# centreborelli/satnerf

Hardware: AMD Instinct MI355X
Metric: training rays/sec (64 samples/ray) (higher is better)
Workload: dtype bf16; 1 GPU; BASELINE configs[1] sat-nerf 256/tau4, 1024 rays x 64 samples/GPU, mlp_mode=bf16, saved state 8-bit, noise_std=0 sc_lambda=0 n_importance=0, stratified jitter drawn in-kernel (Philox-4x32-10); rays_per_gpu=1024, global_batch=1024, n_samples=64, parallelism=dp1

## Files before the change

include/satrender.h:

```cpp
#ifndef SATRENDER_H
#define SATRENDER_H

#include <stdint.h>

#ifdef __cplusplus
extern "C" {
#endif

#define SR_VERSION 100

#define SR_MODE_BF16 1
#define SR_MODE_BF16X3 3
#define SR_MODE_F16 2

#define SR_FMT16 16
#define SR_FMT8 8

int sr_version(void);
const char* sr_last_error(void);

int64_t sr_fwd_stream_elems(int feat, int tau);
int64_t sr_bwd_stream_elems(int feat, int tau);
int64_t sr_act_elems_per_tile(int feat, int fmt);
int64_t sr_dpre_elems_per_tile(int feat, int fmt);
int64_t sr_workspace_tiles(int64_t n_points);
int64_t sr_dpre_workspace_elems(int64_t n_points, int feat, int fmt);

int sr_pack_stream(const float* src, const int32_t* idx, const float* scale, int64_t n,
                   uint16_t* out_hi, uint16_t* out_lo, int64_t n_f16, void* stream);
int sr_pack_all(const float* src, const int32_t* idx, const float* scale, int64_t n, uint16_t* out_hi, uint16_t* out_lo,
                const int32_t* f32_idx, const float* f32_scale, int64_t n_f32, float* out_f32, float* tick, int64_t n_f16,
                void* stream);

int sr_gather_scale_f32(const float* src, const int32_t* idx, const float* scale, int64_t n, float* out, void* stream);

int sr_unpack_grads(const float* partial, const int32_t* gidx, const float* gscale, int64_t n_params, const int32_t* blocks,
                    float* grad, int accumulate, void* stream);

int sr_ray_sample_fwd(const float* rays, int ray_stride, const float* u, int64_t n_rays, int n_samples,
                      float* z_vals, void* stream);

int sr_sky_fwd(const float* sun, int sun_stride, int64_t n, int hidden, const float* w1, const float* b1,
               const float* w2, const float* b2, float* sky, void* stream);

typedef struct sr_mlp_inputs {
  const float* org;
  int org_stride;
  const float* dir;
  int dir_stride;
  const float* sun;
  int sun_stride;
  const float* z;
  const float* temb;
  const int64_t* ts;
  int64_t n_points;
  int n_samples;
} sr_mlp_inputs;

int sr_satnerf_mlp_fwd(const sr_mlp_inputs* in, int feat, int tau, int mode, const uint16_t* stream_hi,
                       const uint16_t* stream_lo, const float* l0, float* albedo, float* sigma, float* sun_v,
                       float* beta, uint16_t* acts, int act_fmt, void* stream);

typedef struct sr_render_args {
  const float* rays;
  int ray_stride;
  const int64_t* ts;
  const float* temb;
  int64_t n_rays;
  int n_samples;
  const float* z_in;
  const float* u;
  uint64_t seed;
  float* step_counter;
  int tick;
  const float* noise;
  float noise_std;
  int sky_hidden;
  const float* sky_w1;
  const float* sky_b1;
  const float* sky_w2;
  const float* sky_b2;
  int64_t bank_chunks;
} sr_render_args;

typedef struct sr_render_outputs {
  float* z_vals;
  float* albedo;
  float* sigma;
  float* sun_v;
  float* beta;
  float* sky;
  float* weights;
  float* transparency;
  float* depth;
  float* rgb;
} sr_render_outputs;

int sr_satnerf_render_fwd(const sr_render_args* in, int feat, int tau, int mode, const uint16_t* stream_hi, const uint16_t* stream_lo,
                          const float* l0, const sr_render_outputs* out, void* stream);
int sr_render_points_per_block(int feat, int mode);

typedef struct sr_train_args {
  const float* target;
  const float* sched;
  float beta_min;
  float* loss_parts;
  float* rgb;
  float* d_sigma;
  float* d_albedo;
  float* d_sun_v;
  float* g_beta;
  float* d_sky;
  const int64_t* gather_idx;
  float* cursor;
  int64_t batches;
  float* out_rays;
  float* out_rgbs;
  int64_t* out_ts;
} sr_train_args;
int sr_satnerf_render_train(const sr_render_args* in, int feat, int tau, int mode, const uint16_t* stream_hi, const uint16_t* stream_lo,
                            const float* l0, const sr_render_outputs* out, const sr_train_args* train, uint16_t* acts, int act_fmt, void* stream);

int sr_satnerf_mlp_bwd(int feat, int tau, int64_t n_points, const uint16_t* bwd_stream, const uint16_t* acts,
                       const float* albedo, const float* sigma, const float* sun_v, const float* beta, const float* g_albedo,
                       const float* g_sigma, const float* g_sun_v, const float* g_beta, uint16_t* dpre, float* d_t, int fmt,
                       void* stream);
int sr_wgrad_plan(int32_t* blocks, int n_blocks, int64_t n_points, int n_wg, int fmt, int* n_slices);
int sr_satnerf_wgrad(int feat, int tau, int64_t n_points, const uint16_t* dpre, const uint16_t* acts, const int32_t* blocks,
                     int n_blocks, int n_slices, float* partial, void* stream);
int sr_satnerf_wgrad8(int feat, int tau, int64_t n_points, const uint16_t* dpre, int64_t dpre_elems, const uint16_t* acts,
                      const int32_t* blocks, const int32_t* loads, int n_blocks, int n_slices, int plan_span, float* partial, void* stream);
int sr_wgrad8_load_ints(void);

int sr_sky_bwd(const float* sun, int sun_stride, int64_t n, int hidden, const float* w1, const float* b1, const float* w2,
               const float* sky, const float* d_sky, float* g_w1, float* g_b1, float* g_w2, float* g_b2, void* stream);
int sr_embedding_bwd(const float* d_t, const int64_t* ts, int64_t n_rays, int n_samples, int tau, float* g_emb, void* stream);

int sr_sc_loss(const float* z_vals, const float* sigma, const float* noise, float noise_std, const float* sun_v, int64_t n_rays,
               int n_samples, float lambda_sc, float* loss_parts, float* d_sun_v, void* stream);
int sr_depth_loss(const float* depth, const float* depths, int depths_stride, int use_weights, int64_t n_rays, float lambda_ds,
                  float* loss_parts, float* g_depth, void* stream);
int sr_ray_setup(const float* rays, int ray_stride, const float* u, int64_t n_rays, int n_samples, int hidden, const float* w1,
                 const float* b1, const float* w2, const float* b2, float* z_vals, float* sky, void* stream);
int sr_ray_setup_rng(const float* rays, int ray_stride, uint64_t seed, float* step_counter, int tick, int64_t n_rays, int n_samples,
                     int hidden, const float* w1, const float* b1, const float* w2, const float* b2, float* z_vals, float* sky,
                     void* stream);
int sr_render_loss(const float* z_vals, const float* sigma, const float* noise, float noise_std, const float* albedo,
                   const float* sun_v, const float* beta, const float* sky, const float* target, int64_t n_rays, int n_samples,
                   float beta_min, const float* sched, float* loss_parts, float* rgb, float* d_sigma, float* d_albedo, float* d_sun_v,
                   float* g_beta, float* d_sky, void* stream);

int sr_grad_tail(const float* partial, const int32_t* gidx, const float* gscale, int64_t n_params, const int32_t* blocks, int n_blocks,
                 float* grad, int accumulate, const float* sun, int sun_stride, int64_t n_rays, int hidden,
                 const float* w1, const float* b1, const float* w2, const float* sky, const float* d_sky, float* g_w1, float* g_b1,
                 float* g_w2, float* g_b2, const float* d_t, const int64_t* ts, int n_samples, int tau, float* g_emb, void* stream);
typedef struct sr_pack_scatter {
  const int32_t* map;
  uint16_t* hi;
  uint16_t* lo;
  float* l0;
  int64_t n_f16;
  float scales[4];
} sr_pack_scatter;
int sr_grad_tail_adam(const float* partial, const int32_t* gidx, const float* gscale, int64_t n_params, const int32_t* blocks, int n_blocks,
                      float* grad,
                      int accumulate, const float* sun, int sun_stride, int64_t n_rays, int hidden, const float* w1, const float* b1,
                      const float* w2, const float* sky, const float* d_sky, float* g_w1, float* g_b1, float* g_w2, float* g_b2,
                      const float* d_t, const int64_t* ts, int n_samples, int tau, float* g_emb, float* params, float* exp_avg,
                      float* exp_avg_sq, const int32_t* late_idx, int n_late, float* state, float lr, float beta1, float beta2, float eps,
                      float grad_scale, const sr_pack_scatter* pack, void* stream);
int sr_adam_step_graph(float* params, float* grads, float* exp_avg, float* exp_avg_sq, int64_t n, float lr, float beta1,
                       float beta2, float eps, float grad_scale, float* state, int zero_grad, void* stream);
int sr_adam_step_pack(float* params, float* grads, float* exp_avg, float* exp_avg_sq, int64_t n, float lr, float beta1, float beta2,
                      float eps, float grad_scale, float* state, int zero_grad, int64_t n_packed, const sr_pack_scatter* pack,
                      void* stream);

enum { SR_ACT_NONE = 0, SR_ACT_SIN = 1, SR_ACT_RELU = 2 };
enum { SR_OUT_NONE = 0, SR_OUT_SOFTPLUS = 1, SR_OUT_SIGMOID = 2, SR_OUT_SIGMOID_RGB = 3 };
typedef struct sr_linear_src {
  const float* x;
  int ld;
  int k;
  int act;
  float w0;
  int row_div;
} sr_linear_src;
int sr_linear_fwd(const sr_linear_src* src, int n_src, const float* weight, const float* bias, int64_t n_points, int n_out,
                  int out_act, float* y, int ldy, void* stream);
int sr_linear_bwd_input(const float* gy, int ldg, const float* y, int ldy, int out_act, const float* weight, int k_total, int col0,
                        const sr_linear_src* target, int64_t n_points, int n_out, float* d_src, int ldd, void* stream);
int sr_linear_bwd_weight(const float* gy, int ldg, const float* y, int ldy, int out_act, const sr_linear_src* src, int n_src,
                         int64_t n_points, int n_out, float* d_weight, float* d_bias, void* stream);
int sr_points_along(const float* rays, int ray_stride, int dir_col, const float* z_vals, int64_t n_rays, int n_samples, float* xyz,
                    void* stream);
int sr_positional_map(const float* x, int ld, int dim, int64_t rows, int n_freqs, float* out, void* stream);

int sr_composite_image(const float* z_vals, const float* sigma, const float* noise, float noise_std, const float* albedo,
                       const float* sun_v, const float* beta, const float* sky, int64_t n_rays, int n_samples, float* image,
                       void* stream);
int sr_latlonalt_from_depth(const float* rays, int ray_stride, const float* depth, int64_t n_rays, const double* center,
                            double range, double* lat, double* lon, double* alt, void* stream);

int sr_rpc_rays(const double* rpc, int width, int height, double min_alt, double max_alt, const double* center, double range,
                double sun_elevation_deg, double sun_azimuth_deg, float* rays11, float* rays8, void* stream);

int sr_rpc_rays_at(const double* rpc, const double* colrow, int64_t n, double min_alt, double max_alt, const double* center, double range,
                   double sun_elevation_deg, double sun_azimuth_deg, float* rays11, void* stream);
int sr_reprojection_errors(const double* rpc, const double* colrow, const int64_t* pts3d_idx, int64_t n, const double* pts3d,
                           int64_t n_pts, float* err, void* stream);
int sr_keypoint_weights_scratch(int64_t n_pts, int n_cams, int64_t* bytes);
int sr_keypoint_weights(const int64_t* pts3d_idx, const int64_t* cam, const float* err, int64_t n, int64_t n_pts, int n_cams,
                        void* scratch, int64_t scratch_bytes, float* e, float* w, float* e_mean, void* stream);
int sr_tie_point_depths(const float* rays11, const double* pts3d, const int64_t* pts3d_idx, int64_t n, int64_t n_pts,
                        const double* center, double range, const float* w, float* depths, void* stream);

int sr_idw_grid_scratch(int64_t k, int n_neighbors, int64_t* bytes);
int sr_idw_interpolate(const double* pts2d, const float* z, int64_t k, const double* query, int64_t n_query, int height, int width,
                       int n_neighbors, void* scratch, int64_t scratch_bytes, double* out, int* nn_idx, int* visited, void* stream);
int sr_gaussian_filter_f64(const double* in, int h, int w, const double* taps0, int radius0, const double* taps1, int radius1,
                           double* tmp, double* out, void* stream);

int sr_utm_zone(double lat, double lon, int* zone, int* letter);
int sr_utm_from_latlon(const double* lat, const double* lon, int64_t n, int zone, double* east, double* north, void* stream);
int sr_depth_to_utm(const float* rays, int ray_stride, const float* depth, int64_t n_rays, const double* center, double range,
                    int zone, double* east, double* north, double* alt, int* zone_out, void* stream);
int sr_dsm_bounds(const double* east, const double* north, const double* alt, int64_t n, double* bounds, void* stream);
int sr_dsm_rasterize(const double* east, const double* north, const double* alt, int64_t n, double xoff, double yoff,
                     double resolution, int xsize, int ysize, int radius, double sigma, uint64_t* acc, float* dsm, float* weight,
                     void* stream);

int sr_dsm_register_scratch(int hu, int wu, int hv, int wv, int irange, int64_t* bytes, int* levels);
int sr_dsm_downsample2x(const double* in, int h, int w, double* out, void* stream);
int sr_dsm_compute_shift(const double* u, int hu, int wu, const double* v, int hv, int wv, int irange, int scaling, void* scratch,
                         int64_t scratch_bytes, int* shift, double* coef, double* ncc_levels, int* start_levels, void* stream);
int sr_dsm_apply_shift(const double* v, int hv, int wv, const int* shift, const double* coef, float* out, void* stream);

int sr_image_metrics_scratch(int64_t n, int64_t planes, int h, int w, int64_t* bytes);
int sr_image_sse(const float* pred, const float* gt, int64_t n, const uint8_t* mask, int64_t mask_div, void* scratch,
                 int64_t scratch_bytes, double* out, void* stream);
int sr_ssim_sum(const float* img1, const float* img2, int64_t planes, int h, int w, void* scratch, int64_t scratch_bytes, double* out,
                void* stream);

int sr_satnerf_loss(const float* rgb, const float* weights, const float* beta, const float* target, int64_t n_rays,
                    int n_samples, float beta_min, float grad_scale, const float* sched, float* loss_parts, float* g_rgb,
                    float* g_weights, float* g_beta, void* stream);
int sr_gather_batch(const float* rays, const float* rgbs, const int64_t* ts, const int64_t* idx, int64_t n, float* out_rays,
                    float* out_rgbs, int64_t* out_ts, float* cursor, int64_t batches, void* stream);
int sr_gather_setup(const float* rays, const float* rgbs, const int64_t* ts, const int64_t* idx, int64_t n, float* out_rays,
                    float* out_rgbs, int64_t* out_ts, float* cursor, int64_t batches, int n_samples, int hidden, const float* w1,
                    const float* b1, const float* w2, const float* b2, float* z_vals, float* sky, uint64_t seed,
                    const float* step_counter, int step_offset, void* stream);
int sr_adam_step(float* params, float* grads, float* exp_avg, float* exp_avg_sq, int64_t n, float lr, float beta1,
                 float beta2, float eps, float grad_scale, int64_t step, int zero_grad, void* stream);

int sr_composite_fwd(const float* z_vals, const float* sigma, const float* noise, float noise_std,
                     const float* albedo, const float* sun_v, const float* sky, int64_t n_rays, int n_samples,
                     int clamp_rgb, float* weights, float* transparency, float* depth, float* rgb, void* stream);

int sr_composite_bwd(const float* z_vals, const float* sigma, const float* noise, float noise_std,
                     const float* albedo, const float* sun_v, const float* sky, const float* weights,
                     const float* transparency, const float* rgb_unclamped_or_null, int64_t n_rays, int n_samples,
                     int clamp_rgb, const float* g_rgb, const float* g_depth, const float* g_weights,
                     const float* g_transparency, float* d_sigma, float* d_albedo, float* d_sun_v, float* d_sky,
                     void* stream);

int sr_sample_pdf_merge(const float* z_coarse, const float* weights_coarse, const float* u, int64_t n_rays,
                        int n_samples, int n_importance, float eps, float* z_fine, void* stream);
int sr_sample_pdf(const float* bins, const float* weights, const float* u, int64_t n_rays, int n_bins, int n_importance,
                  float eps, float* samples, void* stream);

#ifdef __cplusplus
}
#endif
#endif
// ... 1 lines not shown
```

satnerf_amd/_lib.py:

```python
from __future__ import annotations

import ctypes as C
import os

_HERE = os.path.dirname(os.path.abspath(__file__))
LIB_PATH = os.environ.get("SATRENDER_LIB") or os.path.join(_HERE, "csrc", "libsatrender.so")

MODE_BF16 = 1
MODE_F16 = 2
MODE_BF16X3 = 3
FMT16, FMT8 = 16, 8

_vp, _i, _i64, _f, _d = C.c_void_p, C.c_int, C.c_int64, C.c_float, C.c_double


class MlpInputs(C.Structure):
    _fields_ = [("org", _vp), ("org_stride", _i), ("dir", _vp), ("dir_stride", _i), ("sun", _vp), ("sun_stride", _i),
                ("z", _vp), ("temb", _vp), ("ts", _vp), ("n_points", _i64), ("n_samples", _i)]


class RenderArgs(C.Structure):
    _fields_ = [("rays", _vp), ("ray_stride", _i), ("ts", _vp), ("temb", _vp), ("n_rays", _i64), ("n_samples", _i), ("z_in", _vp), ("u", _vp),
                ("seed", C.c_uint64), ("step_counter", _vp), ("tick", _i), ("noise", _vp), ("noise_std", _f), ("sky_hidden", _i),
                ("sky_w1", _vp), ("sky_b1", _vp), ("sky_w2", _vp), ("sky_b2", _vp), ("bank_chunks", _i64)]


class RenderOutputs(C.Structure):
    _fields_ = [(k, _vp) for k in ("z_vals", "albedo", "sigma", "sun_v", "beta", "sky", "weights", "transparency", "depth", "rgb")]


class TrainArgs(C.Structure):
    _fields_ = [("target", _vp), ("sched", _vp), ("beta_min", _f), ("loss_parts", _vp), ("rgb", _vp), ("d_sigma", _vp), ("d_albedo", _vp),
                ("d_sun_v", _vp), ("g_beta", _vp), ("d_sky", _vp), ("gather_idx", _vp), ("cursor", _vp), ("batches", _i64), ("out_rays", _vp),
                ("out_rgbs", _vp), ("out_ts", _vp)]


class PackScatter(C.Structure):
    _fields_ = [("map", _vp), ("hi", _vp), ("lo", _vp), ("l0", _vp), ("n_f16", _i64), ("scales", _f * 4)]


class LinearSrc(C.Structure):
    _fields_ = [("x", _vp), ("ld", _i), ("k", _i), ("act", _i), ("w0", _f), ("row_div", _i)]


ACT_NONE, ACT_SIN, ACT_RELU = 0, 1, 2
OUT_NONE, OUT_SOFTPLUS, OUT_SIGMOID, OUT_SIGMOID_RGB = 0, 1, 2, 3

SIGNATURES = {
    "sr_version": (_i, []),
    "sr_last_error": (C.c_char_p, []),
    "sr_fwd_stream_elems": (_i64, [_i, _i]),
    "sr_bwd_stream_elems": (_i64, [_i, _i]),
    "sr_act_elems_per_tile": (_i64, [_i, _i]),
    "sr_satnerf_render_fwd": (_i, [_vp, _i, _i, _i, _vp, _vp, _vp, _vp, _vp]),
    "sr_render_points_per_block": (_i, [_i, _i]),
    "sr_satnerf_render_train": (_i, [_vp, _i, _i, _i, _vp, _vp, _vp, _vp, _vp, _vp, _i, _vp]),
    "sr_pack_stream": (_i, [_vp, _vp, _vp, _i64, _vp, _vp, _i64, _vp]),
    "sr_dpre_elems_per_tile": (_i64, [_i, _i]),
    "sr_workspace_tiles": (_i64, [_i64]),
    "sr_dpre_workspace_elems": (_i64, [_i64, _i, _i]),
    "sr_unpack_grads": (_i, [_vp, _vp, _vp, _i64, _vp, _vp, _i, _vp]),
    "sr_composite_image": (_i, [_vp, _vp, _vp, _f, _vp, _vp, _vp, _vp, _i64, _i, _vp, _vp]),
    "sr_latlonalt_from_depth": (_i, [_vp, _i, _vp, _i64, _vp, _d, _vp, _vp, _vp, _vp]),
    "sr_linear_fwd": (_i, [C.POINTER(LinearSrc), _i, _vp, _vp, _i64, _i, _i, _vp, _i, _vp]),
    "sr_linear_bwd_input": (_i, [_vp, _i, _vp, _i, _i, _vp, _i, _i, C.POINTER(LinearSrc), _i64, _i, _vp, _i, _vp]),
    "sr_linear_bwd_weight": (_i, [_vp, _i, _vp, _i, _i, C.POINTER(LinearSrc), _i, _i64, _i, _vp, _vp, _vp]),
    "sr_positional_map": (_i, [_vp, _i, _i, _i64, _i, _vp, _vp]),
    "sr_points_along": (_i, [_vp, _i, _i, _vp, _i64, _i, _vp, _vp]),
    "sr_wgrad_plan": (_i, [_vp, _i, _i64, _i, _i, _vp]),
    "sr_satnerf_mlp_bwd": (_i, [_i, _i, _i64, _vp, _vp, _vp, _vp, _vp, _vp, _vp, _vp, _vp, _vp, _vp, _vp, _i, _vp]),
    "sr_satnerf_wgrad": (_i, [_i, _i, _i64, _vp, _vp, _vp, _i, _i, _vp, _vp]),
    "sr_satnerf_wgrad8": (_i, [_i, _i, _i64, _vp, _i64, _vp, _vp, _vp, _i, _i, _i, _vp, _vp]),
    "sr_wgrad8_load_ints": (_i, []),
    "sr_sky_bwd": (_i, [_vp, _i, _i64, _i, _vp, _vp, _vp, _vp, _vp, _vp, _vp, _vp, _vp, _vp]),
    "sr_embedding_bwd": (_i, [_vp, _vp, _i64, _i, _i, _vp, _vp]),
    "sr_ray_setup": (_i, [_vp, _i, _vp, _i64, _i, _i, _vp, _vp, _vp, _vp, _vp, _vp, _vp]),
    "sr_sc_loss": (_i, [_vp, _vp, _vp, _f, _vp, _i64, _i, _f, _vp, _vp, _vp]),
    "sr_depth_loss": (_i, [_vp, _vp, _i, _i, _i64, _f, _vp, _vp, _vp]),
    "sr_ray_setup_rng": (_i, [_vp, _i, C.c_uint64, _vp, _i, _i64, _i, _i, _vp, _vp, _vp, _vp, _vp, _vp, _vp]),
    "sr_render_loss": (_i, [_vp, _vp, _vp, _f, _vp, _vp, _vp, _vp, _vp, _i64, _i, _f, _vp, _vp, _vp, _vp, _vp, _vp, _vp, _vp, _vp]),
    "sr_satnerf_loss": (_i, [_vp, _vp, _vp, _vp, _i64, _i, _f, _f, _vp, _vp, _vp, _vp, _vp, _vp]),
    "sr_adam_step": (_i, [_vp, _vp, _vp, _vp, _i64, _f, _f, _f, _f, _f, _i64, _i, _vp]),
    "sr_gather_setup": (_i, [_vp, _vp, _vp, _vp, _i64, _vp, _vp, _vp, _vp, _i64, _i, _i, _vp, _vp, _vp, _vp, _vp, _vp, C.c_uint64, _vp, _i, _vp]),
    "sr_gather_batch": (_i, [_vp, _vp, _vp, _vp, _i64, _vp, _vp, _vp, _vp, _i64, _vp]),
    "sr_grad_tail": (_i, [_vp, _vp, _vp, _i64, _vp, _i, _vp, _i, _vp, _i, _i64, _i, _vp, _vp, _vp, _vp, _vp, _vp, _vp, _vp, _vp, _vp, _vp, _i, _i,
                          _vp, _vp]),
    "sr_grad_tail_adam": (_i, [_vp, _vp, _vp, _i64, _vp, _i, _vp, _i, _vp, _i, _i64, _i, _vp, _vp, _vp, _vp, _vp, _vp, _vp, _vp, _vp, _vp, _vp, _i, _i,
                               _vp, _vp, _vp, _vp, _vp, _i, _vp, _f, _f, _f, _f, _f, _vp, _vp]),
    "sr_adam_step_graph": (_i, [_vp, _vp, _vp, _vp, _i64, _f, _f, _f, _f, _f, _vp, _i, _vp]),
    "sr_adam_step_pack": (_i, [_vp, _vp, _vp, _vp, _i64, _f, _f, _f, _f, _f, _vp, _i, _i64, _vp, _vp]),
    "sr_pack_all": (_i, [_vp, _vp, _vp, _i64, _vp, _vp, _vp, _vp, _i64, _vp, _vp, _i64, _vp]),
    "sr_gather_scale_f32": (_i, [_vp, _vp, _vp, _i64, _vp, _vp]),
    "sr_ray_sample_fwd": (_i, [_vp, _i, _vp, _i64, _i, _vp, _vp]),
    "sr_sky_fwd": (_i, [_vp, _i, _i64, _i, _vp, _vp, _vp, _vp, _vp, _vp]),
    "sr_satnerf_mlp_fwd": (_i, [C.POINTER(MlpInputs), _i, _i, _i, _vp, _vp, _vp, _vp, _vp, _vp, _vp, _vp, _i, _vp]),
    "sr_composite_fwd": (_i, [_vp, _vp, _vp, _f, _vp, _vp, _vp, _i64, _i, _i, _vp, _vp, _vp, _vp, _vp]),
    "sr_composite_bwd": (_i, [_vp, _vp, _vp, _f, _vp, _vp, _vp, _vp, _vp, _vp, _i64, _i, _i, _vp, _vp, _vp, _vp, _vp, _vp,
                              _vp, _vp, _vp]),
    "sr_sample_pdf_merge": (_i, [_vp, _vp, _vp, _i64, _i, _i, _f, _vp, _vp]),
    "sr_sample_pdf": (_i, [_vp, _vp, _vp, _i64, _i, _i, _f, _vp, _vp]),
    "sr_rpc_rays": (_i, [_vp, _i, _i, _d, _d, _vp, _d, _d, _d, _vp, _vp, _vp]),
    "sr_rpc_rays_at": (_i, [_vp, _vp, _i64, _d, _d, _vp, _d, _d, _d, _vp, _vp]),
    "sr_reprojection_errors": (_i, [_vp, _vp, _vp, _i64, _vp, _i64, _vp, _vp]),
    "sr_keypoint_weights_scratch": (_i, [_i64, _i, C.POINTER(_i64)]),
    "sr_keypoint_weights": (_i, [_vp, _vp, _vp, _i64, _i64, _i, _vp, _i64, _vp, _vp, _vp, _vp]),
    "sr_tie_point_depths": (_i, [_vp, _vp, _vp, _i64, _i64, _vp, _d, _vp, _vp, _vp]),
    "sr_idw_grid_scratch": (_i, [_i64, _i, C.POINTER(_i64)]),
    "sr_idw_interpolate": (_i, [_vp, _vp, _i64, _vp, _i64, _i, _i, _i, _vp, _i64, _vp, _vp, _vp, _vp]),
    "sr_gaussian_filter_f64": (_i, [_vp, _i, _i, _vp, _i, _vp, _i, _vp, _vp, _vp]),
    "sr_utm_zone": (_i, [_d, _d, C.POINTER(_i), C.POINTER(_i)]),
    "sr_utm_from_latlon": (_i, [_vp, _vp, _i64, _i, _vp, _vp, _vp]),
    "sr_depth_to_utm": (_i, [_vp, _i, _vp, _i64, _vp, _d, _i, _vp, _vp, _vp, _vp, _vp]),
    "sr_dsm_bounds": (_i, [_vp, _vp, _vp, _i64, _vp, _vp]),
    "sr_dsm_rasterize": (_i, [_vp, _vp, _vp, _i64, _d, _d, _d, _i, _i, _i, _d, _vp, _vp, _vp, _vp]),
    "sr_dsm_register_scratch": (_i, [_i, _i, _i, _i, _i, C.POINTER(_i64), C.POINTER(_i)]),
    "sr_dsm_downsample2x": (_i, [_vp, _i, _i, _vp, _vp]),
    "sr_dsm_compute_shift": (_i, [_vp, _i, _i, _vp, _i, _i, _i, _i, _vp, _i64, _vp, _vp, _vp, _vp, _vp]),
    "sr_dsm_apply_shift": (_i, [_vp, _i, _i, _vp, _vp, _vp, _vp]),
    "sr_image_metrics_scratch": (_i, [_i64, _i64, _i, _i, C.POINTER(_i64)]),
    "sr_image_sse": (_i, [_vp, _vp, _i64, _vp, _i64, _vp, _i64, _vp, _vp]),
    "sr_ssim_sum": (_i, [_vp, _vp, _i64, _i, _i, _vp, _i64, _vp, _vp]),
}

_lib = None


class SatRenderError(RuntimeError):
    pass


def lib():
    global _lib
    if _lib is None:
        if not os.path.exists(LIB_PATH):
            raise SatRenderError(
                f"{LIB_PATH} not found: build the HIP library first (python -c 'import __graft_entry__ as g; g.build()'). "
                "satnerf_amd has no CPU or PyTorch fallback.")
        handle = C.CDLL(LIB_PATH)
        for name, (res, args) in SIGNATURES.items():
            fn = getattr(handle, name)
            fn.restype, fn.argtypes = res, args
        _lib = handle
    return _lib


def call(name, *args):
    handle = lib()
    rc = getattr(handle, name)(*args)
    if rc != 0:
        raise SatRenderError(f"{name} failed (status {rc}): {handle.sr_last_error().decode(errors='replace')}")
```

satnerf_amd/csrc/mlp_api.hip:

```cpp
#include "common.h"
#include "mlp_layout.h"
#include "mlp_params.h"

namespace sr {
int launch_fwd_p1a1(const FwdParams&, int, hipStream_t);
int launch_fwd_p1a2(const FwdParams&, int, hipStream_t);
int launch_fwd_p3a1(const FwdParams&, int, hipStream_t);
int launch_fwd_p3a2(const FwdParams&, int, hipStream_t);
int launch_fwd_h1a1(const FwdParams&, int, hipStream_t);
int launch_fwd_h1a2(const FwdParams&, int, hipStream_t);
int launch_fwd512_p1a1(const FwdParams&, int, hipStream_t);
int launch_fwd512_p1a2(const FwdParams&, int, hipStream_t);
int launch_fwd512_h1a1(const FwdParams&, int, hipStream_t);
int launch_fwd512_h1a2(const FwdParams&, int, hipStream_t);
long fwd512_stream_pieces_a1();
long fwd512_stream_pieces_a2();
}
using namespace sr;
extern "C" int sr_satnerf_mlp_fwd(const sr_mlp_inputs* in, int feat, int tau, int mode, const uint16_t* stream_hi,
                                  const uint16_t* stream_lo, const float* l0, float* albedo, float* sigma, float* sun_v,
                                  float* beta, uint16_t* acts, int act_fmt, void* stream) {
  SR_REQUIRE(in != nullptr, "sr_satnerf_mlp_fwd: null inputs");
  SR_REQUIRE(feat == kFeat || feat == 512, "sr_satnerf_mlp_fwd: feat=%d unsupported (this build handles %d and 512)", feat, kFeat);
  SR_REQUIRE(mode == SR_MODE_BF16 || mode == SR_MODE_BF16X3 || mode == SR_MODE_F16, "sr_satnerf_mlp_fwd: bad mode %d", mode);
  SR_REQUIRE(feat == kFeat || ((mode == SR_MODE_BF16 || mode == SR_MODE_F16) && (acts == nullptr || act_fmt == SR_FMT8)),
             "sr_satnerf_mlp_fwd: feat=512 runs the fused kernel in SR_MODE_BF16 / SR_MODE_F16, saving activations in SR_FMT8 only (parity mode: layer by layer)");
  SR_REQUIRE(tau >= 1 && tau <= 24, "sr_satnerf_mlp_fwd: tau=%d unsupported (1..24)", tau);
  SR_REQUIRE(stream_hi && l0 && in->org && in->sun && in->temb, "sr_satnerf_mlp_fwd: null pointer argument");
  SR_REQUIRE(mode != SR_MODE_BF16X3 || stream_lo, "sr_satnerf_mlp_fwd: BF16X3 needs the lo plane");
  SR_REQUIRE(in->n_samples >= 1, "sr_satnerf_mlp_fwd: n_samples must be >= 1");
  SR_REQUIRE(acts == nullptr || act_fmt == SR_FMT16 || act_fmt == SR_FMT8, "sr_satnerf_mlp_fwd: act_fmt must be 16 or 8 (got %d)", act_fmt);
  if (in->n_points <= 0) return 0;
  FwdParams p;
  p.in = *in;
  p.rend = RenderParams{};
  p.train = TrainParams{};
  p.stream_hi = (const char*)stream_hi;
  p.stream_lo = (const char*)stream_lo;
  p.l0 = (const float4*)l0;
  p.albedo = albedo, p.sigma = sigma, p.sun_v = sun_v, p.beta = beta;
  p.acts = (uint4*)acts;
  p.tau = tau;
  hipStream_t st = (hipStream_t)stream;
  const int save = acts != nullptr ? act_fmt : 0;
  const int auxs = aux_steps(tau);
  if (feat == 512 && mode == SR_MODE_F16) return auxs == 1 ? launch_fwd512_h1a1(p, save, st) : launch_fwd512_h1a2(p, save, st);
  if (feat == 512) return auxs == 1 ? launch_fwd512_p1a1(p, save, st) : launch_fwd512_p1a2(p, save, st);
  if (mode == SR_MODE_BF16) return auxs == 1 ? launch_fwd_p1a1(p, save, st) : launch_fwd_p1a2(p, save, st);
  if (mode == SR_MODE_F16) return auxs == 1 ? launch_fwd_h1a1(p, save, st) : launch_fwd_h1a2(p, save, st);
  return auxs == 1 ? launch_fwd_p3a1(p, save, st) : launch_fwd_p3a2(p, save, st);
}

extern "C" int64_t sr_fwd_stream_elems(int feat, int tau) {
  if ((feat != kFeat && feat != 512) || tau < 1 || tau > 24) return -1;
  if (feat == 512) return (aux_steps(tau) == 1 ? fwd512_stream_pieces_a1() : fwd512_stream_pieces_a2()) * 512;
  return (aux_steps(tau) == 1 ? FwdStream<1>::total_pieces() : FwdStream<2>::total_pieces()) * 512;
}

extern "C" int sr_render_points_per_block(int feat, int mode) {
  if (mode != SR_MODE_BF16 && mode != SR_MODE_BF16X3 && mode != SR_MODE_F16) return -1;
  if (feat == kFeat) return mode == SR_MODE_BF16X3 ? 128 : 256;
  if (feat == 512 && (mode == SR_MODE_BF16 || mode == SR_MODE_F16)) return 128;
  return -1;
}

static int render_launch(const char* who, const sr_render_args* in, int feat, int tau, int mode, const uint16_t* stream_hi, const uint16_t* stream_lo,
                         const float* l0, const sr_render_outputs* out, const sr_train_args* tr, uint16_t* acts, int act_fmt, void* stream) {
  SR_REQUIRE(in != nullptr && out != nullptr, "%s: null argument block", who);
  const int per_block = sr_render_points_per_block(feat, mode);
  SR_REQUIRE(per_block > 0, "%s: no fused kernel for feat=%d mode=%d (256: every mode; 512: SR_MODE_BF16 / SR_MODE_F16)", who, feat, mode);
  SR_REQUIRE(tau >= 1 && tau <= 24, "%s: tau=%d unsupported (1..24)", who, tau);
  SR_REQUIRE(in->n_samples >= 2 && per_block % in->n_samples == 0, "%s: n_samples=%d must be >= 2 and divide %d (sr_render_points_per_block)", who,
             in->n_samples, per_block);
  SR_REQUIRE(in->rays && in->ts && in->temb && in->ray_stride >= 11, "%s: rays (stride >= 11), ts and temb are required", who);
  SR_REQUIRE(stream_hi && l0 && (mode != SR_MODE_BF16X3 || stream_lo), "%s: null weight stream", who);
  SR_REQUIRE(in->sky_w1 && in->sky_b1 && in->sky_w2 && in->sky_b2 && in->sky_hidden >= 1, "%s: the sky head's weights are required", who);
  SR_REQUIRE(tr != nullptr || (out->weights && out->transparency), "%s: weights and transparency outputs are required", who);
  SR_REQUIRE(!in->tick || in->step_counter, "%s: tick needs the 4-float step counter block", who);
  SR_REQUIRE(in->bank_chunks >= 0 && (in->bank_chunks == 0 || in->step_counter), "%s: bank_chunks needs the step counter", who);
  if (tr != nullptr) {
    SR_REQUIRE(mode == SR_MODE_BF16 || mode == SR_MODE_F16, "%s: the fused training forward exists for SR_MODE_BF16 / SR_MODE_F16 (8-bit saved state)", who);
    SR_REQUIRE(acts != nullptr && act_fmt == SR_FMT8, "%s: needs the SR_FMT8 activation workspace", who);
    SR_REQUIRE(in->n_samples <= 64, "%s: n_samples=%d unsupported (one wave per ray: <= 64); use the separate launches", who, in->n_samples);
    SR_REQUIRE(tr->target && tr->loss_parts && tr->d_sigma && tr->d_albedo && tr->d_sun_v && tr->g_beta && tr->d_sky && out->sky, "%s: null training output", who);
    SR_REQUIRE(out->albedo && out->sigma && out->sun_v && out->beta, "%s: the four per-point outputs are required (the dX pass reads them)", who);
    if (tr->gather_idx != nullptr) {
      SR_REQUIRE(tr->cursor && tr->batches >= 1 && tr->batches < (1 << 24), "%s: the in-launch sampler needs a cursor block and 1 <= batches < 2^24", who);
      SR_REQUIRE(tr->out_rays && tr->out_rgbs && tr->out_ts, "%s: the in-launch sampler needs out_rays / out_rgbs / out_ts", who);
      SR_REQUIRE(in->ray_stride == 11 && in->bank_chunks == 0 && in->z_in == nullptr && in->u == nullptr && in->noise == nullptr,
                 "%s: the in-launch sampler takes a bank of 11-float rows and draws its own jitter (no z_in / u / noise / bank_chunks)", who);
    }
  }
  SR_REQUIRE(in->tick != 2 || (tr != nullptr && in->bank_chunks == 0), "%s: tick == 2 (tick first) is a training-launch option", who);
  SR_REQUIRE(in->tick >= 0 && in->tick <= 2, "%s: tick must be 0, 1 or 2", who);
  if (in->n_rays <= 0) return 0;
  FwdParams p;
  p.in.org = in->rays, p.in.org_stride = in->ray_stride;
  p.in.dir = in->rays + 3, p.in.dir_stride = in->ray_stride;
  p.in.sun = in->rays + 8, p.in.sun_stride = in->ray_stride;
  p.in.z = nullptr, p.in.temb = in->temb, p.in.ts = in->ts;
  p.in.n_points = in->n_rays * in->n_samples, p.in.n_samples = in->n_samples;
  RenderParams& r = p.rend;
  r.rays = in->rays, r.ray_stride = in->ray_stride, r.z_in = in->z_in, r.u = in->u, r.seed = in->seed, r.step_counter = in->step_counter;
  r.tick = in->tick, r.noise = in->noise, r.noise_std = in->noise_std, r.sky_hidden = in->sky_hidden;
  r.w1 = in->sky_w1, r.b1 = in->sky_b1, r.w2 = in->sky_w2, r.b2 = in->sky_b2;
  r.z_out = out->z_vals, r.sky = out->sky, r.weights = out->weights, r.transp = out->transparency, r.depth = out->depth, r.rgb = out->rgb;
  r.n_rays = in->n_rays, r.bank_chunks = in->bank_chunks;
  p.train = TrainParams{};
  if (tr != nullptr) {
    TrainParams& t = p.train;
    t.target = tr->target, t.sched = tr->sched, t.beta_min = tr->beta_min, t.loss_parts = tr->loss_parts, t.rgb = tr->rgb;
    t.d_sigma = tr->d_sigma, t.d_albedo = tr->d_albedo, t.d_sun = tr->d_sun_v, t.g_beta = tr->g_beta, t.d_sky = tr->d_sky;
    t.gather_idx = (const long long*)tr->gather_idx, t.cursor = tr->cursor, t.batches = (unsigned)tr->batches;
    t.out_rays = tr->out_rays, t.out_rgbs = tr->out_rgbs, t.out_ts = (long long*)tr->out_ts;
  }
  p.stream_hi = (const char*)stream_hi, p.stream_lo = (const char*)stream_lo, p.l0 = (const float4*)l0;
  p.albedo = out->albedo, p.sigma = out->sigma, p.sun_v = out->sun_v, p.beta = out->beta;
  p.acts = (uint4*)acts, p.tau = tau;
  hipStream_t st = (hipStream_t)stream;
  const int save = acts != nullptr ? act_fmt : 0;
  const int auxs = aux_steps(tau);
  if (feat == 512 && mode == SR_MODE_F16) return auxs == 1 ? launch_fwd512_h1a1(p, save, st) : launch_fwd512_h1a2(p, save, st);
  if (feat == 512) return auxs == 1 ? launch_fwd512_p1a1(p, save, st) : launch_fwd512_p1a2(p, save, st);
  if (mode == SR_MODE_BF16) return auxs == 1 ? launch_fwd_p1a1(p, save, st) : launch_fwd_p1a2(p, save, st);
  if (mode == SR_MODE_F16) return auxs == 1 ? launch_fwd_h1a1(p, save, st) : launch_fwd_h1a2(p, save, st);
  return auxs == 1 ? launch_fwd_p3a1(p, save, st) : launch_fwd_p3a2(p, save, st);
}

extern "C" int sr_satnerf_render_fwd(const sr_render_args* in, int feat, int tau, int mode, const uint16_t* stream_hi, const uint16_t* stream_lo,
                                     const float* l0, const sr_render_outputs* out, void* stream) {
  return render_launch("sr_satnerf_render_fwd", in, feat, tau, mode, stream_hi, stream_lo, l0, out, nullptr, nullptr, 0, stream);
}

extern "C" int sr_satnerf_render_train(const sr_render_args* in, int feat, int tau, int mode, const uint16_t* stream_hi, const uint16_t* stream_lo,
                                       const float* l0, const sr_render_outputs* out, const sr_train_args* train, uint16_t* acts, int act_fmt,
                                       void* stream) {
  SR_REQUIRE(train != nullptr, "sr_satnerf_render_train: null training argument block");
  return render_launch("sr_satnerf_render_train", in, feat, tau, mode, stream_hi, stream_lo, l0, out, train, acts, act_fmt, stream);
}
```

satnerf_amd/csrc/mlp_bwd.hip:

```cpp
#ifndef SR_BWD_TILES
#define SR_BWD_TILES 1
#endif
#if SR_BWD_TILES == 2
#define SR_MODE1_NW 4
#endif
#include "mlp_bwd.inc"

namespace sr {
int launch_bwd512(const BwdParams& p, int fmt, hipStream_t st);
long bwd512_stream_pieces();
int dpre8_units_512();
int act8_units_512(int auxs);
}

using namespace sr;

extern "C" int sr_satnerf_mlp_bwd(int feat, int tau, int64_t n_points, const uint16_t* bwd_stream, const uint16_t* acts, const float* albedo,
                                  const float* sigma, const float* sun_v, const float* beta, const float* g_albedo, const float* g_sigma,
                                  const float* g_sun_v, const float* g_beta, uint16_t* dpre, float* d_t, int fmt, void* stream) {
  SR_REQUIRE(feat == kFeat || feat == 512, "sr_satnerf_mlp_bwd: feat=%d unsupported (this build handles %d and 512)", feat, kFeat);
  SR_REQUIRE(tau >= 1 && tau <= 24, "sr_satnerf_mlp_bwd: tau=%d unsupported (1..24)", tau);
  SR_REQUIRE(fmt == SR_FMT16 || fmt == SR_FMT8, "sr_satnerf_mlp_bwd: workspace format must be 16 or 8 (got %d)", fmt);
  SR_REQUIRE(feat == kFeat || fmt == SR_FMT8, "sr_satnerf_mlp_bwd: feat=512 trains on the 8-bit workspaces only");
  SR_REQUIRE(bwd_stream && acts && dpre && albedo && sigma && sun_v && beta, "sr_satnerf_mlp_bwd: null pointer argument");
  if (n_points <= 0) return 0;
  BwdParams p;
  p.g_albedo = g_albedo, p.g_sigma = g_sigma, p.g_sun = g_sun_v, p.g_beta = g_beta;
  p.albedo = albedo, p.sigma = sigma, p.sun_v = sun_v, p.beta = beta;
  p.acts = (const uint4*)acts, p.dpre = (uint4*)dpre, p.d_t = d_t;
  p.stream = (const char*)bwd_stream;
  p.n_points = n_points, p.tau = tau, p.auxs = aux_steps(tau);
  p.emax = fmt == SR_FMT8 ? (uint4*)(dpre + sr_workspace_tiles(n_points) * sr_dpre_elems_per_tile(feat, fmt)) : nullptr;
  if (feat == 512) return launch_bwd512(p, fmt, (hipStream_t)stream);
  return fmt == SR_FMT8 ? launch_bwd_fmt<SR_FMT8>(p, (hipStream_t)stream) : launch_bwd_fmt<SR_FMT16>(p, (hipStream_t)stream);
}

extern "C" int64_t sr_bwd_stream_elems(int feat, int tau) {
  if ((feat != kFeat && feat != 512) || tau < 1 || tau > 24) return -1;
  return (feat == 512 ? bwd512_stream_pieces() : BwdStream::total_pieces()) * 512;
}

extern "C" int64_t sr_workspace_tiles(int64_t n_points) { return n_points < 0 ? -1 : sr::ws_tiles(n_points); }

extern "C" int64_t sr_dpre_elems_per_tile(int feat, int fmt) {
  if (fmt != SR_FMT16 && fmt != SR_FMT8) return -1;
  if (feat == 512) return fmt == SR_FMT8 ? (int64_t)dpre8_units_512() * 64 * 8 : -1;
  if (feat != kFeat) return -1;
  return (int64_t)(fmt == SR_FMT8 ? kD8Units : kDpFrags) * 64 * 8;
}

extern "C" int64_t sr_dpre_workspace_elems(int64_t n_points, int feat, int fmt) {
  const int64_t per_tile = sr_dpre_elems_per_tile(feat, fmt);
  if (per_tile < 0 || n_points < 0) return -1;
  return sr::ws_tiles(n_points) * per_tile + (fmt == SR_FMT8 ? sr::ws_emax_bytes(n_points) / 2 : 0);
}

extern "C" int64_t sr_act_elems_per_tile(int feat, int fmt) {
  if (fmt != SR_FMT16 && fmt != SR_FMT8) return -1;
  if (feat == 512) return fmt == SR_FMT8 ? (int64_t)act8_units_512(2) * 64 * 8 : -1;
  if (feat != kFeat) return -1;
  return (int64_t)(fmt == SR_FMT8 ? act8_units(2) : act_ksteps(2)) * 64 * 8;
}
```

satnerf_amd/csrc/mlp_bwd.inc:

```
#pragma once
#include "mlp_device.h"
#include "mlp_params.h"
#include "codec8.h"

namespace sr {
inline namespace SR_FEAT_NS {

using BS = BwdStream;
constexpr int kBSlot = BS::SLOTP * 1024;
#ifndef SR_BWD_TILES
#define SR_BWD_TILES 1
#endif
constexpr int kBT = SR_BWD_TILES;

template <int G, int LIMIT>
__device__ __forceinline__ void bchunk_enter(char* ring, const char* stream, int wave, int lane) {
  constexpr int later = [] {
    int n = 0;
    for (int c = 1; c < kD; ++c) n += G + c < LIMIT ? min_loads<1>(BS::np(G + c)) : 0;
    return n;
  }();
  wait_then_barrier<later>();
  if constexpr (G + kD < LIMIT) {
    constexpr long off = BS::offset_pieces(G + kD) * 1024L;
    constexpr int slot = (G + kD) % kNSLOT;
    issue_chunk<1, BS::np(G + kD)>(stream, nullptr, off, ring + slot * kBSlot, wave, lane);
  }
}

__device__ __forceinline__ float phase_cos(uint32_t w, int half) {
  const uint32_t u = half ? (w >> 16) : (w & 0xffffu);
  return __builtin_amdgcn_cosf((float)u * (1.0f / 65535.0f));
}

template <int FMT>
struct Phase {
  uint4 p0, p1;
  __device__ __forceinline__ void load(const uint4* acts_tile, int auxs, int frag) {
    if constexpr (FMT == SR_FMT8) p0 = ws_load(acts_tile + (auxs + (frag >> 1)) * 64);
    else p0 = ws_load(acts_tile + (auxs + frag) * 64), p1 = ws_load(acts_tile + (auxs + frag + 1) * 64);
  }
  __device__ __forceinline__ void from_lds(const char* slot, int lane) {
    p0 = *reinterpret_cast<const uint4*>(slot + lane * 16);
    if constexpr (FMT != SR_FMT8) p1 = *reinterpret_cast<const uint4*>(slot + 1024 + lane * 16);
  }
  __device__ __forceinline__ float cos(int g) const {
    if constexpr (FMT == SR_FMT8) {
      const uint32_t pw[4] = {p0.x, p0.y, p0.z, p0.w};
      return __builtin_amdgcn_cosf(phase8_rev(pw[g >> 2], g & 3));
    } else {
      const uint32_t pw[8] = {p0.x, p0.y, p0.z, p0.w, p1.x, p1.y, p1.z, p1.w};
      return phase_cos(pw[g >> 1], g & 1);
    }
  }
};

template <bool COS, int FMT>
__device__ __forceinline__ uint32_t bpack(const f32x16& acc, const Phase<FMT>& ph, uint4& o0, uint4& o1, uint4* dpre_tile, int frag) {
  float v[16];
#pragma unroll
  for (int g = 0; g < 16; ++g) v[g] = COS ? acc[g] * ph.cos(g) : acc[g];
  o0 = make_uint4(pack_bf16x2(v[0], v[1]), pack_bf16x2(v[2], v[3]), pack_bf16x2(v[4], v[5]), pack_bf16x2(v[6], v[7]));
  o1 = make_uint4(pack_bf16x2(v[8], v[9]), pack_bf16x2(v[10], v[11]), pack_bf16x2(v[12], v[13]), pack_bf16x2(v[14], v[15]));
  if constexpr (FMT == SR_FMT8) {
    const uint32_t e = mx8_exponent(v, o0.x);
    ws_store(dpre_tile + dp8_unit(frag) * 64, mx8_encode(v, e));
    return e;
  } else {
    ws_store(dpre_tile + frag * 64, o0);
    ws_store(dpre_tile + (frag + 1) * 64, o1);
    return 0u;
  }
}
template <int NT>
__device__ __forceinline__ uint32_t max_byte(const uint32_t (&eb)[4]) {
  uint32_t m = 0;
#pragma unroll
  for (int w = 0; w < (NT + 3) / 4; ++w) {
    const uint32_t a = eb[w] & 0xffu, b = (eb[w] >> 8) & 0xffu, c = (eb[w] >> 16) & 0xffu, d = eb[w] >> 24;
    const uint32_t ab = a > b ? a : b, cd = c > d ? c : d;
    m = m > ab ? m : ab, m = m > cd ? m : cd;
  }
  return m;
}
template <int CTRL, int ROW_MASK>
__device__ __forceinline__ uint32_t dpp_max_step(uint32_t v) {
  const uint32_t o = (uint32_t)__builtin_amdgcn_update_dpp(0, (int)v, CTRL, ROW_MASK, 0xf, false);
  return v > o ? v : o;
}
__device__ __forceinline__ uint32_t wave_max_u32(uint32_t v) {
  v = dpp_max_step<0x111, 0xf>(v);
  v = dpp_max_step<0x112, 0xf>(v);
  v = dpp_max_step<0x114, 0xf>(v);
  v = dpp_max_step<0x118, 0xf>(v);
  v = dpp_max_step<0x142, 0xa>(v);
  v = dpp_max_step<0x143, 0xc>(v);
  return (uint32_t)__builtin_amdgcn_readlane((int)v, 63);
}
__device__ __forceinline__ void note_emax(uint32_t* emax, int group, uint32_t lane_max, int lane) {
  const uint32_t m = wave_max_u32(lane_max);
  if (lane == 0) emax[group] = m;
}
template <int FMT, int NT>
__device__ __forceinline__ void store_scales(uint4* dpre_tile, int group, const uint32_t (&eb)[4], uint32_t* emax) {
  if constexpr (FMT == SR_FMT8) {
    note_emax(emax, group, max_byte<NT>(eb), (int)(threadIdx.x & 63));
    char* p = reinterpret_cast<char*>(dpre_tile + (kD8Scale + group / kD8GroupsPerUnit) * 64) + (group % kD8GroupsPerUnit) * kMT;
    if constexpr (NT > 8) *reinterpret_cast<uint4*>(p) = make_uint4(eb[0], eb[1], eb[2], eb[3]);
    else if constexpr (NT > 4) *reinterpret_cast<uint2*>(p) = make_uint2(eb[0], eb[1]);
    else *reinterpret_cast<uint32_t*>(p) = eb[0];
  }
}

template <int KIN>
__device__ __forceinline__ void btile(const char* slot, int p0, const uint4 (&in)[kBT][KIN], f32x16 (&acc)[kBT], int lane) {
#pragma unroll
  for (int j = 0; j < kBT; ++j) acc[j] = f32x16{0};
  uint4 a = {};
#pragma unroll
  for (int i = 0; i < KIN; ++i) {
#ifdef SR_ABL_HALF_LDS
    if (i % 2 == 0)
#endif
    a = *reinterpret_cast<const uint4*>(slot + (p0 + i) * 1024 + lane * 16);
#pragma unroll
    for (int j = 0; j < kBT; ++j) acc[j] = mfma(a, in[j][i], acc[j]);
  }
}
template <int NP, int OFF, int KIN>
__device__ __forceinline__ void btile_part(const char* slot, const uint4 (&in)[kBT][KIN], f32x16 (&acc)[kBT], int lane) {
#pragma unroll
  for (int i = 0; i < NP; ++i) {
    const uint4 a = *reinterpret_cast<const uint4*>(slot + i * 1024 + lane * 16);
#pragma unroll
    for (int j = 0; j < kBT; ++j) acc[j] = mfma(a, in[j][OFF + i], acc[j]);
  }
}

template <int NP, int NS, int NSS>
struct TrunkSched {
  static constexpr int ND = 2 * kKS / Mode<1>::NW;
  static constexpr int tile_len(int t) { return (t % 2 == 0 ? ND : 0) + NP + (t > 0 ? NS : 0); }
  static constexpr int tile_start(int t) {
    int p = 0;
    for (int k = 0; k < t; ++k) p += tile_len(k);
    return p;
  }
  static constexpr int period() { return tile_start(kMT) + NS + NSS; }
  static constexpr int after_d(int t) { return tile_start(t) + ND; }
  static constexpr int after_p(int t) { return tile_start(t) + (t % 2 == 0 ? ND : 0) + NP; }
  static constexpr int at_store(int t) { return t < kMT - 1 ? after_p(t + 1) : tile_start(kMT); }
  static constexpr int wait_b(int t) {
    if (t >= 2) return at_store(t) - after_p(t - 2);
    const int steady = at_store(t) - (after_p(t + kMT - 2) - period());
    const int first = t == 0 ? NP + at_store(0) : at_store(1);
    return steady < first ? steady : first;
  }
  static constexpr int wait_a(int t) { return t >= 2 ? tile_start(t) - after_d(t - 2) : tile_start(0) - (after_d(kMT - 2) - period()); }
};

template <int N>
__device__ __forceinline__ void wait_vmcnt() {
  static_assert(N >= 0 && N < 64, "vmcnt is a 6-bit field");
  asm volatile("s_waitcnt vmcnt(%0)" ::"n"(N) : "memory");
}

struct PreSched {
  static constexpr int kTiles = 3 * kMTH + kMTH + kMTH + kMT;
  static constexpr int frag(int k) {
    if (k < 3 * kMTH) {
      const int part = k / kMTH, t = k % kMTH;
      return (part == 0 ? kActRgbh : part == 1 ? kActS3 : kActE1) + 2 * t;
    }
    k -= 3 * kMTH;
    if (k < kMTH) return kActS2 + 2 * k;
    k -= kMTH;
    if (k < kMTH) return kActS1 + 2 * k;
    return kActA0 + 7 * kKS + 2 * (k - kMTH);
  }
  static constexpr int chunk_of(int k) {
    if (k < 3 * kMTH) return BS::G_H;
    k -= 3 * kMTH;
    if (k < kMTH) return BS::G_S3 + k / 2;
    k -= kMTH;
    if (k < kMTH) return BS::G_S2 + k / 2;
    return BS::G_G1 + (k - kMTH);
  }
  static constexpr int kAhead = 4;
  static constexpr int wait(int k, int nph, int limit) {
    int n = 0;
    const int req_chunk = k >= kAhead ? chunk_of(k - kAhead) : -1;
    for (int g = req_chunk + 1; g <= chunk_of(k); ++g) n += g + kD < limit ? min_loads<1>(BS::np(g + kD)) : 0;
    const int later = kTiles - 1 - k < kAhead - 1 ? kTiles - 1 - k : kAhead - 1;
    n += nph * later;
    return n < 63 ? n : 63;
  }
};

template <int FMT, int LIMIT, int KIN, int TPC, int NCHUNK, int G0, bool COS, int NOUT, int PK0, int DF0, class Req>
__device__ __forceinline__ void bstage(const uint4 (&in)[kBT][KIN], uint4 (&out)[kBT][NOUT], char* ring, const char* stream, int wave, int lane,
                                       const char* stage, Req&& request, uint4* const (&dpre_tile)[kBT], uint32_t* const (&emax)[kBT]) {
  constexpr int NPH = FMT == SR_FMT8 ? 1 : 2;
  uint32_t eb[kBT][4] = {};
  static_for<NCHUNK>([&](auto cc) {
    constexpr int c = decltype(cc)::value, g = G0 + c;
    static_assert(BS::np(g) == TPC * KIN, "backward stream geometry mismatch");
    bchunk_enter<g, LIMIT>(ring, stream, wave, lane);
    const char* slot = ring + (g % kNSLOT) * kBSlot;
    static_for<TPC>([&](auto tc) {
      constexpr int tt = decltype(tc)::value, t = c * TPC + tt, o = 2 * t;
      Phase<FMT> ph[kBT] = {};
      f32x16 acc[kBT];
      btile<KIN>(slot, tt * KIN, in, acc, lane);
      if constexpr (COS) {
        constexpr int k = PK0 + t;
        wait_vmcnt<PreSched::wait(k, kBT * NPH, LIMIT)>();
#pragma unroll
        for (int j = 0; j < kBT; ++j) ph[j].from_lds(stage + ((k & 3) * kBT + j) * NPH * 1024, lane);
      }
#pragma unroll
      for (int j = 0; j < kBT; ++j)
        eb[j][t >> 2] |= bpack<COS, FMT>(acc[j], ph[j], out[j][o], out[j][o + 1], dpre_tile[j], DF0 + 2 * t) << (8 * (t & 3));
      if constexpr (COS && PK0 + t + PreSched::kAhead < PreSched::kTiles) request((PK0 + t + PreSched::kAhead) & 3, PreSched::frag(PK0 + t + PreSched::kAhead));
    });
  });
#pragma unroll
  for (int j = 0; j < kBT; ++j) store_scales<FMT, TPC * NCHUNK>(dpre_tile[j], dp8_group(DF0), eb[j], emax[j]);
}

typedef uint32_t u32x32w __attribute__((ext_vector_type(32)));
typedef uint32_t u32x4w __attribute__((ext_vector_type(4)));
template <int FMT, bool TRUNK_ASM = false>
__global__ void __launch_bounds__(Mode<1>::NW * 64) satnerf_bwd_kernel(const BwdParams prm) {
  constexpr int NW = Mode<1>::NW;
  constexpr bool kStreamG1 = false;
  constexpr int LIMIT = !TRUNK_ASM ? BS::NCH : kStreamG1 ? BS::G_G1 : BS::G_L;
  extern __shared__ __attribute__((aligned(16))) char smem[];
  char* ring = smem;
#ifdef SR_BWD_TIMING
  const uint64_t t_kernel0 = __builtin_amdgcn_s_memtime(), r_kernel0 = __builtin_amdgcn_s_memrealtime();
#endif
  const int tid = threadIdx.x, lane = tid & 63;
  const int wave = __builtin_amdgcn_readfirstlane(tid >> 6);
  const int h = lane >> 5, pl = lane & 31;
  const char* stream = prm.stream;
  const int A = prm.auxs, AK = FMT == SR_FMT8 ? act8_units(prm.auxs) : act_ksteps(prm.auxs);
  constexpr int DK = FMT == SR_FMT8 ? kD8Units : kDpFrags;

#pragma unroll
  for (int g = 0; g < kD; ++g) {
    if (g == 0) issue_chunk<1, BS::np(0)>(stream, nullptr, 0, ring, wave, lane);
    if (g == 1) issue_chunk<1, BS::np(1)>(stream, nullptr, BS::offset_pieces(1) * 1024L, ring + kBSlot, wave, lane);
    if (g == 2) issue_chunk<1, BS::np(2)>(stream, nullptr, BS::offset_pieces(2) * 1024L, ring + 2 * kBSlot, wave, lane);
  }

#ifdef SR_BWD_REVERSE
  const long tile0 = ((long)(gridDim.x - 1 - blockIdx.x) * NW + wave) * kBT;
#else
  const long tile0 = ((long)blockIdx.x * NW + wave) * kBT;
#endif
  long pt[kBT];
  bool valid[kBT];
  uint4* dpre[kBT];
#pragma unroll
  for (int j = 0; j < kBT; ++j) {
    pt[j] = (tile0 + j) * 32 + pl;
    valid[j] = pt[j] < prm.n_points;
    dpre[j] = prm.dpre + (tile0 + j) * DK * 64 + lane;
  }

  uint4 dhead[kBT][1], dsig[kBT];
  uint32_t e_feats[kBT] = {}, e_raw[kBT] = {};
#pragma unroll
  for (int j = 0; j < kBT; ++j) {
    float v[8] = {0.f, 0.f, 0.f, 0.f, 0.f, 0.f, 0.f, 0.f}, sg = 0.f;
    const long q = pt[j];
    uint4 fs = {};
    if constexpr (FMT == SR_FMT8)
      fs = prm.acts[((tile0 + j) * (long)act8_units(prm.auxs) + prm.auxs + kA8Scale) * 64 + lane];
    if (valid[j]) {
      if (h == 0) {
        if (prm.g_albedo) {
#pragma unroll
          for (int c = 0; c < 3; ++c) {
            const float s = (prm.albedo[q * 3 + c] + 0.001f) * (1.0f / 1.002f);
            v[c] = prm.g_albedo[q * 3 + c] * 1.002f * s * (1.0f - s);
          }
        }
        if (prm.g_sun) {
          const float s = prm.sun_v[q];
          v[3] = prm.g_sun[q] * s * (1.0f - s);
        }
        if (prm.g_sigma) sg = prm.g_sigma[q] * (1.0f - expf(-prm.sigma[q]));
      } else if (prm.g_beta) {
        v[0] = prm.g_beta[q] * (1.0f - expf(-prm.beta[q]));
      }
    }
    dhead[j][0] = make_uint4(pack_bf16x2(v[0], v[1]), pack_bf16x2(v[2], v[3]), pack_bf16x2(v[4], v[5]), pack_bf16x2(v[6], v[7]));
    dsig[j] = make_uint4(pack_bf16x2(sg, 0.f), 0u, 0u, 0u);
    dpre[j][(FMT == SR_FMT8 ? kD8Head : kDpHead) * 64] = dhead[j][0];
    dpre[j][(FMT == SR_FMT8 ? kD8Sigma : kDpSigma) * 64] = dsig[j];
    if constexpr (FMT == SR_FMT8) {
      const uint32_t w4[4] = {fs.x, fs.y, kMT > 8 ? fs.z : 0u, kMT > 8 ? fs.w : 0u};
      e_feats[j] = max_byte<kMT>(w4);
      const uint32_t hw[5] = {dhead[j][0].x, dhead[j][0].y, dhead[j][0].z, dhead[j][0].w, dsig[j].x};
      uint32_t m = 0;
#pragma unroll
      for (int k = 0; k < 5; ++k) {
        const uint32_t lo = (hw[k] & 0x7fffu) >> 7, hi = (hw[k] >> 23) & 0xffu;
        m = m > lo ? m : lo, m = m > hi ? m : hi;
      }
      e_raw[j] = m;
    }
  }

  constexpr int NPH = FMT == SR_FMT8 ? 1 : 2;
  constexpr int NPT = kBT * NPH;
  char* stage = smem + kNSLOT * kBSlot + wave * (4 * NPT * 1024);
  const uint32_t stage_addr = __builtin_amdgcn_readfirstlane(lds_addr_of(stage));
  auto stage_phase = [&](int slot, int frag) {
#ifdef SR_ABL_NO_PHASE_LOADS
    return;
#endif
#pragma unroll
    for (int j = 0; j < kBT; ++j) {
      const char* src = reinterpret_cast<const char*>(prm.acts + ((tile0 + j) * AK + A + (FMT == SR_FMT8 ? frag >> 1 : frag)) * 64);
#pragma unroll
      for (int k = 0; k < NPH; ++k) glds16_s(src + k * 1024, (uint32_t)lane * 16u, stage_addr + ((slot * kBT + j) * NPH + k) * 1024);
    }
  };
  auto phases_of = [&](int slot, Phase<FMT> (&ph)[kBT]) {
#pragma unroll
    for (int j = 0; j < kBT; ++j) ph[j].from_lds(stage + (slot * kBT + j) * NPH * 1024, lane);
  };
  static_assert(PreSched::kAhead == 4, "the wave's phase staging ring has four slots");
  stage_phase(0, PreSched::frag(0)), stage_phase(1, PreSched::frag(1)), stage_phase(2, PreSched::frag(2)), stage_phase(3, PreSched::frag(3));

  uint32_t* emax_cells = reinterpret_cast<uint32_t*>(smem + kNSLOT * kBSlot + NW * (4 * NPT * 1024));
  uint32_t* emax[kBT];
#pragma unroll
  for (int j = 0; j < kBT; ++j) emax[j] = emax_cells + (wave * kBT + j) * 16;
  if constexpr (FMT == SR_FMT8) {
#pragma unroll
    for (int j = 0; j < kBT; ++j) note_emax(emax[j], kEmaxFeats, e_feats[j], lane), note_emax(emax[j], kEmaxRaw, e_raw[j], lane);
  }

#ifdef SR_BWD_TIMING
  uint64_t t_stage[5];
  t_stage[0] = __builtin_amdgcn_s_memtime();
#endif
  uint4 d_rgbh[kBT][kHS], d_s3[kBT][kHS], d_e1[kBT][kHS];
  {
    bchunk_enter<BS::G_H, LIMIT>(ring, stream, wave, lane);
    const char* slot = ring + (BS::G_H % kNSLOT) * kBSlot;
    uint32_t eb[kBT][3][4] = {};
    static_for<3 * kMTH>([&](auto tc) {
      constexpr int T = decltype(tc)::value, part = T / kMTH, t = T % kMTH;
      constexpr int dp0 = part == 0 ? kDpRgbh : (part == 1 ? kDpS3 : kDpE1);
      f32x16 acc[kBT];
      btile<1>(slot, T, dhead, acc, lane);
      wait_vmcnt<PreSched::wait(T, NPT, LIMIT)>();
      Phase<FMT> ph[kBT];
      phases_of(T & 3, ph);
#pragma unroll
      for (int j = 0; j < kBT; ++j) {
        uint4 o0, o1;
        eb[j][part][t >> 2] |= bpack<true, FMT>(acc[j], ph[j], o0, o1, dpre[j], dp0 + 2 * t) << (8 * (t & 3));
        if constexpr (part == 0) d_rgbh[j][2 * t] = o0, d_rgbh[j][2 * t + 1] = o1;
        else if constexpr (part == 1) d_s3[j][2 * t] = o0, d_s3[j][2 * t + 1] = o1;
        else d_e1[j][2 * t] = o0, d_e1[j][2 * t + 1] = o1;
      }
      stage_phase((T + PreSched::kAhead) & 3, PreSched::frag(T + PreSched::kAhead));
    });
#pragma unroll
    for (int j = 0; j < kBT; ++j) {
      store_scales<FMT, kMTH>(dpre[j], dp8_group(kDpRgbh), eb[j][0], emax[j]);
      store_scales<FMT, kMTH>(dpre[j], dp8_group(kDpS3), eb[j][1], emax[j]);
      store_scales<FMT, kMTH>(dpre[j], dp8_group(kDpE1), eb[j][2], emax[j]);
    }
  }
#ifdef SR_BWD_TIMING
  t_stage[1] = __builtin_amdgcn_s_memtime();
#endif
  uint4 d_g2[kBT][3 * kHS];
  {
    uint4 d_s2[kBT][kHS], d_s1[kBT][kHS];
    bstage<FMT, LIMIT, kHS, 2, kMTH / 2, BS::G_S3, true, kHS, 3 * kMTH, kDpS2>(d_s3, d_s2, ring, stream, wave, lane, stage, stage_phase, dpre, emax);
    bstage<FMT, LIMIT, kHS, 2, kMTH / 2, BS::G_S2, true, kHS, 4 * kMTH, kDpS1>(d_s2, d_s1, ring, stream, wave, lane, stage, stage_phase, dpre, emax);
#pragma unroll
    for (int j = 0; j < kBT; ++j) {
#pragma unroll
      for (int i = 0; i < kHS; ++i) d_g2[j][i] = d_rgbh[j][i], d_g2[j][kHS + i] = d_s1[j][i], d_g2[j][2 * kHS + i] = d_e1[j][i];
    }
  }
#ifdef SR_BWD_TIMING
  t_stage[2] = __builtin_amdgcn_s_memtime();
#endif
  uint4 d_g1[kBT][kKS + 1];
  {
    uint4 d_feats[kBT][kKS];
    {
      uint32_t eb[kBT][4] = {};
      static_for<kMT>([&](auto tc) {
        constexpr int t = decltype(tc)::value;
        f32x16 acc[kBT];
#pragma unroll
        for (int j = 0; j < kBT; ++j) acc[j] = f32x16{0};
        static_for<BS::kG2Split>([&](auto sc) {
          constexpr int sp = decltype(sc)::value, g = BS::G_G2 + t * BS::kG2Split + sp;
          static_assert(BS::np(g) == BS::kG2Part, "backward stream geometry mismatch");
          bchunk_enter<g, LIMIT>(ring, stream, wave, lane);
          btile_part<BS::kG2Part, sp * BS::kG2Part>(ring + (g % kNSLOT) * kBSlot, d_g2, acc, lane);
        });
        Phase<FMT> none = {};
#pragma unroll
        for (int j = 0; j < kBT; ++j)
          eb[j][t >> 2] |= bpack<false, FMT>(acc[j], none, d_feats[j][2 * t], d_feats[j][2 * t + 1], dpre[j], kDpFeats + 2 * t) << (8 * (t & 3));
      });
#pragma unroll
      for (int j = 0; j < kBT; ++j) store_scales<FMT, kMT>(dpre[j], dp8_group(kDpFeats), eb[j], emax[j]);
    }
    bchunk_enter<BS::G_DT, LIMIT>(ring, stream, wave, lane);
    f32x16 acc[kBT];
    btile<kHS>(ring + (BS::G_DT % kNSLOT) * kBSlot, 0, d_e1, acc, lane);
#pragma unroll
    for (int j = 0; j < kBT; ++j) {
      if (valid[j] && prm.d_t) {
#pragma unroll
        for (int g = 0; g < 16; ++g) {
          const int row = (g & 3) + 8 * (g >> 2) + 4 * h;
          if (row < prm.tau) prm.d_t[pt[j] * prm.tau + row] = acc[j][g];
        }
      }
#pragma unroll
      for (int i = 0; i < kKS; ++i) d_g1[j][i] = d_feats[j][i];
      d_g1[j][kKS] = dsig[j];
    }
  }
#ifdef SR_BWD_TIMING
  t_stage[3] = __builtin_amdgcn_s_memtime();
#endif
  uint4 cur[kBT][kKS], nxt[kBT][kKS];
  if constexpr (!kStreamG1)
    bstage<FMT, LIMIT, kKS + 1, 1, kMT, BS::G_G1, true, kKS, 5 * kMTH, kDpL + 7 * kKS>(d_g1, cur, ring, stream, wave, lane, stage, stage_phase, dpre, emax);
  constexpr long offL = BS::offset_pieces(BS::G_L);
  using TS = TrunkSched<NPT, 0, 0>;
  wait_then_barrier<0>();
#ifdef SR_BWD_TIMING
  t_stage[4] = __builtin_amdgcn_s_memtime();
#endif
  if constexpr (TRUNK_ASM) {
    static_assert(FMT == SR_FMT8 && kBT == 1, "the generated trunk reads and writes the 8-bit workspaces, one tile per wave");
    static_assert((kFeat == 256 && NW == 8 && kNSLOT * kBSlot == 96 * 1024) || (kFeat == 512 && NW == 4 && kNSLOT * kBSlot >= 128 * 1024),
                  "the generated trunk's geometry (gen/bwd_core.py Geo)");
    u32x32w xq[kKS / 8];
    u32x4w xs = {0u, 0u, 0u, 0u};
#pragma unroll
    for (int i = 0; i < kKS; ++i) {
      const uint4 f = kStreamG1 ? d_g1[0][i] : cur[0][i];
      xq[i / 8][4 * (i % 8)] = f.x, xq[i / 8][4 * (i % 8) + 1] = f.y, xq[i / 8][4 * (i % 8) + 2] = f.z, xq[i / 8][4 * (i % 8) + 3] = f.w;
    }
    if constexpr (kStreamG1) xs = u32x4w{d_g1[0][kKS].x, d_g1[0][kKS].y, d_g1[0][kKS].z, d_g1[0][kKS].w};
    auto uni64 = [](uint64_t v) {
      return ((uint64_t)(uint32_t)__builtin_amdgcn_readfirstlane((int)(uint32_t)(v >> 32)) << 32) | (uint32_t)__builtin_amdgcn_readfirstlane((int)(uint32_t)v);
    };
    const uint32_t ring_addr = lds_addr_of(ring);
    const uint32_t vl0 = ring_addr + (uint32_t)lane * 16u, vl1 = vl0 + 65536u;
    uint32_t voff = (uint32_t)wave * 1024u + (uint32_t)lane * 16u;
    uint32_t poff = (uint32_t)((unsigned long)tile0 * AK * 1024ul) + (uint32_t)lane * 16u;
    uint32_t soff = (uint32_t)((unsigned long)tile0 * DK * 1024ul) + (uint32_t)lane * 16u;
    const uint32_t vcell = lds_addr_of(reinterpret_cast<const char*>(emax[0]));
    const uint32_t wb = (uint32_t)__builtin_amdgcn_readfirstlane((int)(ring_addr + (uint32_t)wave * 1024u));
    const uint64_t sb = uni64((uint64_t)(uintptr_t)(stream + (kStreamG1 ? BS::offset_pieces(BS::G_G1) : offL) * 1024L)), ab = uni64((uint64_t)(uintptr_t)prm.acts), db = uni64((uint64_t)(uintptr_t)prm.dpre);
    const float magic = 12583040.0f;
    const uint32_t k43 = 0x43000000u;
    uint32_t m0save;
#ifdef SR_BWD_TIMING
    const uint64_t t_trunk0 = __builtin_amdgcn_s_memtime(), r_trunk0 = __builtin_amdgcn_s_memrealtime();
#endif
#if SR_FEAT == 512
#define SR_TRUNK_OUTS "+{v[0:31]}"(xq[0]), "+{v[32:63]}"(xq[1]), "+{v[64:95]}"(xq[2]), "+{v[96:127]}"(xq[3]), "+{a[124:127]}"(xs), "+{v217}"(voff), "+{v218}"(poff), "+{v219}"(soff), [m0save] "=&s"(m0save)
#define SR_TRUNK_INS "{v212}"(magic), "{v214}"(k43), "{v215}"(vl0), "{v216}"(vl1), "{v220}"(vcell), [sb] "s"(sb), [wb] "s"(wb), [ab] "s"(ab), [db] "s"(db)
#define SR_TRUNK_A1_DEFAULT "mlp_bwd512_trunk_a1.inc"
#define SR_TRUNK_A2 "mlp_bwd512_trunk_a2.inc"
#define SR_TRUNK_CLOBBERS "mlp_bwd512_trunk_clobbers.inc"
#else
#define SR_TRUNK_OUTS "+{v[0:31]}"(xq[0]), "+{v[32:63]}"(xq[1]), "+{v223}"(voff), "+{v224}"(poff), "+{v225}"(soff), [m0save] "=&s"(m0save)
#define SR_TRUNK_INS "{v218}"(magic), "{v220}"(k43), "{v221}"(vl0), "{v222}"(vl1), "{v230}"(vcell), [sb] "s"(sb), [wb] "s"(wb), [ab] "s"(ab), [db] "s"(db)
#define SR_TRUNK_A1_DEFAULT "mlp_bwd_trunk_a1.inc"
#define SR_TRUNK_A2 "mlp_bwd_trunk_a2.inc"
#define SR_TRUNK_CLOBBERS "mlp_bwd_trunk_clobbers.inc"
#endif
#ifndef SR_TRUNK_A1
#define SR_TRUNK_A1 SR_TRUNK_A1_DEFAULT
#endif
    if (prm.auxs == 1) {
      asm volatile(
#include SR_TRUNK_A1
          : SR_TRUNK_OUTS
          : SR_TRUNK_INS
          :
#include SR_TRUNK_CLOBBERS
      );
    } else {
      asm volatile(
#include SR_TRUNK_A2
          : SR_TRUNK_OUTS
          : SR_TRUNK_INS
          :
#include SR_TRUNK_CLOBBERS
      );
    }
#undef SR_TRUNK_OUTS
#undef SR_TRUNK_INS
#ifdef SR_BWD_TIMING
    {
      const uint64_t t_trunk1 = __builtin_amdgcn_s_memtime(), r_trunk1 = __builtin_amdgcn_s_memrealtime();
      if (lane == 0 && prm.d_t) {
        prm.d_t[tile0 * 8 + 0] = (float)(t_trunk0 - t_kernel0), prm.d_t[tile0 * 8 + 1] = (float)(t_trunk1 - t_trunk0);
        prm.d_t[tile0 * 8 + 2] = (float)(r_trunk1 - r_trunk0), prm.d_t[tile0 * 8 + 3] = (float)(r_trunk0 - r_kernel0);
        prm.d_t[tile0 * 8 + 4] = (float)(t_stage[0] - t_kernel0), prm.d_t[tile0 * 8 + 5] = (float)(t_stage[1] - t_stage[0]);
        prm.d_t[tile0 * 8 + 6] = (float)(t_stage[2] - t_stage[1]), prm.d_t[tile0 * 8 + 7] = (float)(t_stage[3] - t_stage[2]);
      }
    }
#endif
  } else {
  stage_phase(0, kActA0 + 6 * kKS), stage_phase(1, kActA0 + 6 * kKS + 2);
#pragma unroll 1
  for (int l = 7; l >= 1; --l) {
    const long cbase = (long)(7 - l) * kMT;
    const int lfrag = (l - 1) * kKS;
    const int nfrag = l >= 2 ? lfrag - kKS : lfrag;
    f32x16 acc[2][kBT];
    uint32_t eb[kBT][4] = {};
    auto epilogue = [&](auto tc) {
      constexpr int t = decltype(tc)::value;
      Phase<FMT> ph[kBT];
      phases_of(t & 3, ph);
#pragma unroll
      for (int j = 0; j < kBT; ++j)
        eb[j][t >> 2] |= bpack<true, FMT>(acc[t & 1][j], ph[j], nxt[j][2 * t], nxt[j][2 * t + 1], dpre[j], kDpL + lfrag + 2 * t) << (8 * (t & 3));
    };
    static_for<kMT>([&](auto tc) {
      constexpr int t = decltype(tc)::value;
      if constexpr (t % 2 == 0) {
        wait_then_barrier<TS::wait_a(t)>();
#pragma unroll
        for (int k = 2; k < 4; ++k) {
          long c = cbase + t + k;
          c = c < kTrunkLayers * kMT ? c : kTrunkLayers * kMT - 1;
          issue_chunk<1, kKS>(stream, nullptr, (offL + c * kKS) * 1024L, ring + ((BS::G_L + t + k) % kNSLOT) * kBSlot, wave, lane);
        }
      }
      stage_phase((t + 2) & 3, kActA0 + (t + 2 < kMT ? lfrag : nfrag) + 2 * ((t + 2) % kMT));
      if constexpr (t > 0) wait_vmcnt<TS::wait_b(t - 1)>();
      btile<kKS>(ring + ((BS::G_L + t) % kNSLOT) * kBSlot, 0, cur, acc[t & 1], lane);
      if constexpr (t > 0) epilogue(std::integral_constant<int, t - 1>{});
#ifdef SR_BWD_INTERLEAVE
      if constexpr (t > 0) {
#pragma unroll
        for (int i = 0; i < kKS; ++i) {
          __builtin_amdgcn_sched_group_barrier(0x100, 1, 0);
          __builtin_amdgcn_sched_group_barrier(0x008, kBT, 0);
          __builtin_amdgcn_sched_group_barrier(0x002, SR_BWD_INTERLEAVE, 0);
        }
      }
#endif
    });
    wait_vmcnt<TS::wait_b(kMT - 1)>();
    epilogue(std::integral_constant<int, kMT - 1>{});
#pragma unroll
    for (int j = 0; j < kBT; ++j) {
      store_scales<FMT, kMT>(dpre[j], l - 1, eb[j], emax[j]);
#pragma unroll
      for (int i = 0; i < kKS; ++i) cur[j][i] = nxt[j][i];
    }
  }
#ifdef SR_BWD_TIMING
    if (lane == 0 && prm.d_t) {
      const uint64_t t_end = __builtin_amdgcn_s_memtime();
      prm.d_t[tile0 * 8 + 0] = (float)(t_stage[4] - t_kernel0), prm.d_t[tile0 * 8 + 1] = (float)(t_end - t_stage[4]);
      prm.d_t[tile0 * 8 + 2] = 1.f, prm.d_t[tile0 * 8 + 3] = 1.f;
      prm.d_t[tile0 * 8 + 4] = (float)(t_stage[0] - t_kernel0), prm.d_t[tile0 * 8 + 5] = (float)(t_stage[1] - t_stage[0]);
      prm.d_t[tile0 * 8 + 6] = (float)(t_stage[2] - t_stage[1]), prm.d_t[tile0 * 8 + 7] = (float)(t_stage[3] - t_stage[2]);
    }
#endif
  }
  if constexpr (FMT == SR_FMT8) {
    constexpr int kRows = NW * kBT, kEntries = (kRows + kEmaxTiles - 1) / kEmaxTiles;
    __syncthreads();
    if (tid < kEntries && prm.emax) {
      uint32_t w[4] = {0u, 0u, 0u, 0u};
#pragma unroll
      for (int g = 0; g < 16; ++g) {
        uint32_t m = 0;
#pragma unroll
        for (int r = 0; r < kEmaxTiles; ++r) {
          const int row = tid * kEmaxTiles + r;
          const uint32_t c = row < kRows ? emax_cells[row * 16 + g] : 0u;
          m = m > c ? m : c;
        }
        w[g >> 2] |= m << (8 * (g & 3));
      }
      prm.emax[(tile0 - (long)wave * kBT) / kEmaxTiles + tid] = make_uint4(w[0], w[1], w[2], w[3]);
    }
  }
}


template <int FMT, bool TRUNK_ASM>
int launch_bwd_kernel(const BwdParams& p, size_t lds, hipStream_t st) {
  constexpr int NW = Mode<1>::NW;
  if (!ensure_dynamic_lds((const void*)satnerf_bwd_kernel<FMT, TRUNK_ASM>, lds)) return 1;
  const long tiles = (p.n_points + 31) / 32;
  hipLaunchKernelGGL((satnerf_bwd_kernel<FMT, TRUNK_ASM>), dim3((unsigned)((tiles + NW * kBT - 1) / (NW * kBT))), dim3(NW * 64), lds, st, p);
  return check_launch("satnerf_bwd_kernel");
}

template <int FMT>
int launch_bwd_fmt(const BwdParams& p, hipStream_t st) {
  constexpr int NW = Mode<1>::NW;
  const size_t lds = (size_t)kNSLOT * kBSlot + NW * 4 * kBT * (FMT == SR_FMT8 ? 1 : 2) * 1024 + (FMT == SR_FMT8 ? NW * kBT * 64 : 0);
  if constexpr (FMT == SR_FMT8 && (kFeat == 256 || kFeat == 512) && kBT == 1) {
    const char* e = getenv("SATNERF_BWD_V1");
    const bool v1 = e && e[0] == '1';
    const unsigned long big = (unsigned long)ws_tiles(p.n_points) * (kD8Units > act8_units(2) ? kD8Units : act8_units(2)) * 1024ul;
    if (!v1 && big < (1ul << 32)) return launch_bwd_kernel<FMT, true>(p, lds, st);
  }
  return launch_bwd_kernel<FMT, false>(p, lds, st);
}

}
}
```

satnerf_amd/csrc/mlp_fwd_io.inc:

```
#pragma once
#include "mlp_fwd.inc"

namespace sr {
inline namespace SR_FEAT_NS {

constexpr int kRendFloats = 7;
template <bool REND, int NW>
__device__ __forceinline__ void write_outputs(const FwdParams& prm, const PointIn& in, const f32x16& acc, float sig, float* r_z, int wave, int lane) {
  constexpr int P = NW * 32;
  float *r_sigma = r_z + P, *r_sun = r_z + 2 * P, *r_albedo = r_z + 3 * P, *r_beta = r_z + 6 * P;
  const int h = lane >> 5, pl = lane & 31;
  const long pt = in.pt, r = in.r, rg = in.rg;
  const bool valid = in.valid;
  if constexpr (REND) {
    const float sg = softplus_f(sig);
    if (h == 0) {
      r_sigma[wave * 32 + pl] = sg;
      const float al0 = sigmoid_f(acc[0]) * 1.002f - 0.001f, al1 = sigmoid_f(acc[1]) * 1.002f - 0.001f, al2 = sigmoid_f(acc[2]) * 1.002f - 0.001f;
      const float sv = sigmoid_f(acc[3]);
      float* la = r_albedo + (wave * 32 + pl) * 3;
      la[0] = al0, la[1] = al1, la[2] = al2;
      r_sun[wave * 32 + pl] = sv;
      if (valid) {
        if (prm.sigma) prm.sigma[pt] = sg;
        if (prm.albedo) {
          float* a = prm.albedo + pt * 3;
          a[0] = al0, a[1] = al1, a[2] = al2;
        }
        if (prm.sun_v) prm.sun_v[pt] = sv;
      }
    } else {
      const float bt = softplus_f(acc[0]);
      r_beta[wave * 32 + pl] = bt;
      if (valid && prm.beta) prm.beta[pt] = bt;
    }
    __syncthreads();
    const int S = prm.in.n_samples;
    const int rays_here = P / S;
    const bool train = prm.train.target != nullptr;
    const bool warm = prm.train.sched != nullptr && prm.train.sched[2] != 0.f;
    float loss_part = 0.f;
    for (int lr = wave; lr < rays_here; lr += NW) {
      const long ray = (long)blockIdx.x * rays_here + lr;
      if (ray >= prm.rend.n_rays) break;
      const bool gathered = prm.train.gather_idx != nullptr;
      const long ray_g = gathered ? (long)prm.train.gather_idx[in.first + ray] : ray + (rg - r);
      const float* rr = prm.rend.rays + ray_g * prm.rend.ray_stride;
      if (gathered) {
        if (lane < 11) prm.train.out_rays[ray * 11 + lane] = rr[lane];
        else if (lane < 14) prm.train.out_rgbs[ray * 3 + (lane - 11)] = prm.train.target[ray_g * 3 + (lane - 11)];
        else if (lane == 14) prm.train.out_ts[ray] = prm.in.ts[ray_g];
      }
      float k0, k1, k2;
      sky_ray(rr[8], rr[9], rr[10], prm.rend.sky_hidden, prm.rend.w1, prm.rend.b1, prm.rend.w2, prm.rend.b2, lane, k0, k1, k2);
      if (lane == 0 && prm.rend.sky) prm.rend.sky[ray * 3] = k0, prm.rend.sky[ray * 3 + 1] = k1, prm.rend.sky[ray * 3 + 2] = k2;
      if (train) {
        loss_part += render_loss_ray(r_z + lr * S, r_sigma + lr * S, prm.rend.noise ? prm.rend.noise + ray * S : nullptr, prm.rend.noise_std,
                                     r_albedo + lr * S * 3, r_sun + lr * S, r_beta + lr * S, k0, k1, k2, prm.train.target + (gathered ? ray_g : ray) * 3, ray,
                                     prm.rend.n_rays, S, lane, prm.train.beta_min, warm, prm.train.rgb ? prm.train.rgb + ray * 3 : nullptr,
                                     prm.train.d_sigma + ray * S, prm.train.d_albedo + ray * S * 3, prm.train.d_sun + ray * S,
                                     prm.train.g_beta + ray * S, prm.train.d_sky + ray * 3);
        continue;
      }
      composite_ray(r_z + lr * S, r_sigma + lr * S, prm.rend.noise ? prm.rend.noise + ray * S : nullptr, prm.rend.noise_std,
                    r_albedo + lr * S * 3, r_sun + lr * S, k0, k1, k2, S, lane, 1, prm.rend.weights + ray * S, prm.rend.transp + ray * S,
                    prm.rend.depth ? prm.rend.depth + ray : nullptr, prm.rend.rgb ? prm.rend.rgb + ray * 3 : nullptr);
    }
    if (train) {
      __syncthreads();
      if (lane == 0) r_z[wave] = loss_part;
      __syncthreads();
      if (threadIdx.x == 0) {
        float sum = 0.f;
#pragma unroll
        for (int w = 0; w < NW; ++w) sum += r_z[w];
        prm.train.loss_parts[blockIdx.x] = sum;
        if (prm.rend.tick) tick_at_exit(prm.rend.step_counter, in.step_read);
        if (prm.train.gather_idx != nullptr) tick_at_exit(prm.train.cursor, in.cursor_read, prm.train.batches);
      }
    }
  } else if (valid) {
    if (h == 0) {
      if (prm.sigma) prm.sigma[pt] = softplus_f(sig);
      if (prm.albedo) {
        float* a = prm.albedo + pt * 3;
        a[0] = sigmoid_f(acc[0]) * 1.002f - 0.001f;
        a[1] = sigmoid_f(acc[1]) * 1.002f - 0.001f;
        a[2] = sigmoid_f(acc[2]) * 1.002f - 0.001f;
      }
      if (prm.sun_v) prm.sun_v[pt] = sigmoid_f(acc[3]);
    } else if (prm.beta) {
      prm.beta[pt] = softplus_f(acc[0]);
    }
  }
}

}
}
```

satnerf_amd/csrc/mlp_params.h:

```cpp
#pragma once
#include "common.h"

namespace sr {

struct RenderParams {
  const float* rays;
  int ray_stride;
  const float* z_in;
  const float* u;
  unsigned long long seed;
  float* step_counter;
  int tick;
  const float* noise;
  float noise_std;
  int sky_hidden;
  const float *w1, *b1, *w2, *b2;
  float* z_out;
  float* sky;
  float* weights;
  float* transp;
  float* depth;
  float* rgb;
  long n_rays;
  long bank_chunks;
};

struct TrainParams {
  const float* target;
  const float* sched;
  float beta_min;
  float* loss_parts;
  float* rgb;
  float* d_sigma;
  float* d_albedo;
  float* d_sun;
  float* g_beta;
  float* d_sky;
  const long long* gather_idx;
  float* cursor;
  unsigned batches;
  float* out_rays;
  float* out_rgbs;
  long long* out_ts;
};

struct FwdParams {
  sr_mlp_inputs in;
  RenderParams rend;
  TrainParams train;
  const char* stream_hi;
  const char* stream_lo;
  const float4* l0;
  float* albedo;
  float* sigma;
  float* sun_v;
  float* beta;
  uint4* acts;
  int tau;
};

struct BwdParams {
  const float* g_albedo;
  const float* g_sigma;
  const float* g_sun;
  const float* g_beta;
  const float* albedo;
  const float* sigma;
  const float* sun_v;
  const float* beta;
  const uint4* acts;
  uint4* dpre;
  uint4* emax;
  float* d_t;
  const char* stream;
  long n_points;
  int tau;
  int auxs;
};

}
```

satnerf_amd/csrc/ray_device.h:

```cpp
#pragma once
#include "common.h"

namespace sr {

__device__ __forceinline__ float wave_sum(float v) {
#pragma unroll
  for (int m = 32; m >= 1; m >>= 1) v += __shfl_xor(v, m, 64);
  return v;
}
__device__ __forceinline__ float wave_scan_mul(float v, int lane) {
#pragma unroll
  for (int d = 1; d < 64; d <<= 1) {
    const float o = __shfl_up(v, d, 64);
    if (lane >= d) v *= o;
  }
  return v;
}
__device__ __forceinline__ float wave_scan_add(float v, int lane) {
#pragma unroll
  for (int d = 1; d < 64; d <<= 1) {
    const float o = __shfl_up(v, d, 64);
    if (lane >= d) v += o;
  }
  return v;
}
__device__ __forceinline__ float wave_rscan_add(float v, int lane) {
#pragma unroll
  for (int d = 1; d < 64; d <<= 1) {
    const float o = __shfl_down(v, d, 64);
    if (lane + d < 64) v += o;
  }
  return v;
}

__device__ __forceinline__ float linspace01(int i, int n, float step) {
  return i < n / 2 ? (float)i * step : __builtin_fmaf(-step, (float)(n - 1 - i), 1.0f);
}
__device__ __forceinline__ float lerp_near_far(float near, float far, float s) {
#pragma clang fp contract(off)
  const float a = near * (1.0f - s), b = far * s;
  return a + b;
}
__device__ __forceinline__ float stratified_z(float near, float far, int j, int S, float u) {
#pragma clang fp contract(off)
  const float step = 1.0f / (float)(S - 1);
  const float zj = lerp_near_far(near, far, linspace01(j, S, step));
  float lower = zj, upper = zj;
  if (j > 0) lower = 0.5f * (lerp_near_far(near, far, linspace01(j - 1, S, step)) + zj);
  if (j < S - 1) upper = 0.5f * (zj + lerp_near_far(near, far, linspace01(j + 1, S, step)));
  const float span = upper - lower;
  const float jit = span * u;
  return lower + jit;
}

__device__ __forceinline__ void philox4x32(uint32_t k0, uint32_t k1, uint32_t c[4]) {
#pragma unroll
  for (int round = 0; round < 10; ++round) {
    const uint64_t p0 = (uint64_t)0xD2511F53u * c[0], p1 = (uint64_t)0xCD9E8D57u * c[2];
    const uint32_t n0 = (uint32_t)(p1 >> 32) ^ c[1] ^ k0, n2 = (uint32_t)(p0 >> 32) ^ c[3] ^ k1;
    c[0] = n0, c[1] = (uint32_t)p1, c[2] = n2, c[3] = (uint32_t)p0;
    k0 += 0x9E3779B9u, k1 += 0xBB67AE85u;
  }
}
__device__ __forceinline__ float philox_uniform(unsigned long long seed, long r, int j, uint32_t step) {
  uint32_t c[4] = {static_cast<uint32_t>(r), static_cast<uint32_t>(static_cast<unsigned long long>(r) >> 32), static_cast<uint32_t>(j >> 2), step};
  philox4x32((uint32_t)seed, (uint32_t)(seed >> 32), c);
  return (float)(c[j & 3] >> 8) * 5.9604644775390625e-8f;
}

__device__ __forceinline__ uint32_t next_step(uint32_t step, uint32_t keep_mod = 1u) {
  uint32_t next = step + 1u;
  if (next >= (1u << 24)) next = (1u << 23) + (next - (1u << 23)) % (keep_mod ? keep_mod : 1u);
  return next;
}
__device__ __forceinline__ void tick_when_all_read(float* counter, uint32_t step_read, uint32_t modulo = 0u, uint32_t keep_mod = 1u) {
  asm volatile("" ::"v"(step_read));
  __syncthreads();
  if (threadIdx.x == 0) {
    unsigned* arrive = reinterpret_cast<unsigned*>(counter + 3);
    __threadfence();
    if (atomicAdd(arrive, 1u) == gridDim.x - 1) {
      counter[0] = (float)(modulo != 0u ? (step_read + 1u >= modulo ? 0u : step_read + 1u) : next_step(step_read, keep_mod));
      atomicExch(arrive, 0u);
    }
  }
}
__device__ __forceinline__ void tick_at_exit(float* counter, uint32_t step_read, uint32_t modulo = 0u, uint32_t keep_mod = 1u) {
  unsigned* arrive = reinterpret_cast<unsigned*>(counter + 3);
  if (atomicAdd(arrive, 1u) == gridDim.x - 1) {
    counter[0] = (float)(modulo != 0u ? (step_read + 1u >= modulo ? 0u : step_read + 1u) : next_step(step_read, keep_mod));
    atomicExch(arrive, 0u);
  }
}

__device__ __forceinline__ void sky_ray(float sx, float sy, float sz, int hidden, const float* __restrict__ w1, const float* __restrict__ b1,
                                        const float* __restrict__ w2, const float* __restrict__ b2, int lane, float& k0, float& k1, float& k2) {
  float a0 = 0.f, a1 = 0.f, a2 = 0.f;
  for (int k = lane; k < hidden; k += 64) {
    float hk = __builtin_fmaf(w1[k * 3 + 2], sz, __builtin_fmaf(w1[k * 3 + 1], sy, __builtin_fmaf(w1[k * 3], sx, b1[k])));
    hk = hk > 0.f ? hk : 0.f;
    a0 = __builtin_fmaf(w2[k], hk, a0);
    a1 = __builtin_fmaf(w2[hidden + k], hk, a1);
    a2 = __builtin_fmaf(w2[2 * hidden + k], hk, a2);
  }
  a0 = wave_sum(a0), a1 = wave_sum(a1), a2 = wave_sum(a2);
  k0 = sigmoid_f(a0 + b2[0]), k1 = sigmoid_f(a1 + b2[1]), k2 = sigmoid_f(a2 + b2[2]);
}

__device__ __forceinline__ void alpha_at(const float* z, const float* sigma, const float* noise, float noise_std, int j, int S, float& delta,
                                         float& dens, float& alpha) {
#pragma clang fp contract(off)
  delta = (j < S - 1) ? (z[j + 1] - z[j]) : 1e10f;
  float s = sigma[j];
  if (noise) s = s + noise[j] * noise_std;
  dens = s;
  const float rl = s > 0.f ? s : 0.f;
  alpha = 1.0f - expf(-delta * rl);
}
__device__ __forceinline__ void alpha_of(const float* z, const float* sigma, const float* noise, float noise_std, long base, int j, int S,
                                         float& delta, float& dens, float& alpha) {
  alpha_at(z + base, sigma + base, noise ? noise + base : nullptr, noise_std, j, S, delta, dens, alpha);
}

__device__ __forceinline__ void composite_ray(const float* z, const float* sigma, const float* noise, float noise_std, const float* albedo,
                                              const float* sun_v, float k0, float k1, float k2, int S, int lane, int clamp_rgb,
                                              float* __restrict__ weights, float* __restrict__ transp, float* __restrict__ depth_r,
                                              float* __restrict__ rgb_r) {
  float carry = 1.f, dsum = 0.f, c0 = 0.f, c1 = 0.f, c2 = 0.f;
  for (int j0 = 0; j0 < S; j0 += 64) {
    const int j = j0 + lane;
    const bool on = j < S;
    float delta, dens, alpha = 0.f;
    if (on) alpha_at(z, sigma, noise, noise_std, j, S, delta, dens, alpha);
    float f;
    {
#pragma clang fp contract(off)
      f = on ? (1.0f - alpha) + 1e-10f : 1.f;
    }
    const float incl = wave_scan_mul(f, lane);
    float excl = __shfl_up(incl, 1, 64);
    if (lane == 0) excl = 1.f;
    const float T = carry * excl;
    carry = carry * __shfl(incl, 63, 64);
    if (on) {
      const float w = alpha * T;
      weights[j] = w;
      transp[j] = T;
      dsum += w * z[j];
      if (albedo) {
        const float* a = albedo + j * 3;
        float i0 = 1.f, i1 = 1.f, i2 = 1.f;
        if (sun_v) {
          const float sv = sun_v[j];
          i0 = sv + (1.f - sv) * k0, i1 = sv + (1.f - sv) * k1, i2 = sv + (1.f - sv) * k2;
        }
        c0 += w * a[0] * i0, c1 += w * a[1] * i1, c2 += w * a[2] * i2;
      }
    }
  }
  dsum = wave_sum(dsum), c0 = wave_sum(c0), c1 = wave_sum(c1), c2 = wave_sum(c2);
  if (lane == 0) {
    if (depth_r) *depth_r = dsum;
    if (rgb_r) {
      if (clamp_rgb) c0 = fminf(fmaxf(c0, 0.f), 1.f), c1 = fminf(fmaxf(c1, 0.f), 1.f), c2 = fminf(fmaxf(c2, 0.f), 1.f);
      rgb_r[0] = c0, rgb_r[1] = c1, rgb_r[2] = c2;
    }
  }
}

__device__ __forceinline__ float render_loss_ray(const float* z, const float* sigma, const float* noise, float noise_std, const float* albedo,
                                                 const float* sun_v, const float* beta, float k0, float k1, float k2, const float* target, long r,
                                                 long n_rays, int S, int lane, float beta_min, bool warm, float* __restrict__ rgb_out,
                                                 float* __restrict__ d_sigma, float* __restrict__ d_albedo, float* __restrict__ d_sun,
                                                 float* __restrict__ g_beta, float* __restrict__ d_sky) {
  const bool on = lane < S;
  const int i = lane < S ? lane : S - 1;
  float delta = 0.f, dens = 0.f, alpha = 0.f, a0 = 0.f, a1 = 0.f, a2 = 0.f, sv = 0.f, bj = 0.f;
  if (on) {
#pragma clang fp contract(off)
    const float zj = z[i];
    delta = lane < S - 1 ? z[i + 1] - zj : 1e10f;
    float s = sigma[i];
    if (noise) s = s + noise[i] * noise_std;
    dens = s;
    alpha = 1.0f - expf(-delta * (s > 0.f ? s : 0.f));
    a0 = albedo[i * 3], a1 = albedo[i * 3 + 1], a2 = albedo[i * 3 + 2];
    sv = sun_v[i], bj = beta[i];
  }
  float f;
  {
#pragma clang fp contract(off)
    f = on ? (1.0f - alpha) + 1e-10f : 1.f;
  }
  const float incl = wave_scan_mul(f, lane);
  float T = __shfl_up(incl, 1, 64);
  if (lane == 0) T = 1.f;
  const float w = on ? alpha * T : 0.f;
  const float i0 = sv + (1.f - sv) * k0, i1 = sv + (1.f - sv) * k1, i2 = sv + (1.f - sv) * k2;
  const float c0 = wave_sum(w * a0 * i0), c1 = wave_sum(w * a1 * i1), c2 = wave_sum(w * a2 * i2);
  const float b = wave_sum(w * bj) + beta_min;
  const float r0 = fminf(fmaxf(c0, 0.f), 1.f), r1 = fminf(fmaxf(c1, 0.f), 1.f), r2 = fminf(fmaxf(c2, 0.f), 1.f);
  const float inv_n = 1.0f / (float)n_rays;
  const float e0 = r0 - target[0], e1 = r1 - target[1], e2 = r2 - target[2];
  const float sq = e0 * e0 + e1 * e1 + e2 * e2;
  const float ib2 = warm ? 2.0f : 1.0f / (b * b);
  float contrib = sq * ib2 * (0.5f / 3.0f) * inv_n + (warm ? 0.f : 0.5f * logf(b) * inv_n);
  if (r == 0 && !warm) contrib += 1.5f;
  if (lane == 0 && rgb_out) rgb_out[0] = r0, rgb_out[1] = r1, rgb_out[2] = r2;
  const float kk = ib2 * (1.0f / 3.0f) * inv_n;
  const float gr0 = (c0 >= 0.f && c0 <= 1.f) ? e0 * kk : 0.f;
  const float gr1 = (c1 >= 0.f && c1 <= 1.f) ? e1 * kk : 0.f;
  const float gr2 = (c2 >= 0.f && c2 <= 1.f) ? e2 * kk : 0.f;
  const float db = warm ? 0.f : (-sq * ib2 / b * (1.0f / 3.0f) + 0.5f / b) * inv_n;
  const float G = db * bj + gr0 * a0 * i0 + gr1 * a1 * i1 + gr2 * a2 * i2;
  const float tail = on ? G * w : 0.f;
  const float suf = wave_rscan_add(tail, lane);
  const float after = suf - tail;
  const float q0 = w * gr0, q1 = w * gr1, q2 = w * gr2;
  const float di0 = q0 * a0, di1 = q1 * a1, di2 = q2 * a2;
  const float s0 = wave_sum(di0 * (1.f - sv)), s1 = wave_sum(di1 * (1.f - sv)), s2 = wave_sum(di2 * (1.f - sv));
  if (lane == 0) d_sky[0] = s0, d_sky[1] = s1, d_sky[2] = s2;
  if (on) {
    const float dalpha = G * T - after / f;
    d_sigma[i] = dens > 0.f ? dalpha * delta * expf(-delta * dens) : 0.f;
    d_albedo[i * 3] = q0 * i0, d_albedo[i * 3 + 1] = q1 * i1, d_albedo[i * 3 + 2] = q2 * i2;
    d_sun[i] = di0 * (1.f - k0) + di1 * (1.f - k1) + di2 * (1.f - k2);
    g_beta[i] = db * w;
  }
  return contrib;
}

}
```

satnerf_amd/ops.py:

```python
from __future__ import annotations

import ctypes as C
import os

import torch

from . import _lib

MODES = {"bf16": _lib.MODE_BF16, "f16": _lib.MODE_F16, "bf16x3": _lib.MODE_BF16X3}


class KernelTimer:

    def __init__(self):
        self.spans = []

    def span(self, name):
        e0, e1 = torch.cuda.Event(enable_timing=True), torch.cuda.Event(enable_timing=True)
        self.spans.append((name, e0, e1))
        return e0, e1

    def mean_ms(self, name):
        t = [a.elapsed_time(b) for n, a, b in self.spans if n == name]
        return sum(t) / len(t) if t else None


kernel_timer = None


def _stream():
    return C.c_void_p(torch.cuda.current_stream().cuda_stream)


def _p(t):
    return None if t is None else C.c_void_p(t.data_ptr())


def _chk(t, name, dtype=torch.float32, allow_none=False):
    if t is None:
        if allow_none:
            return None
        raise ValueError(f"{name} is required")
    if not t.is_cuda:
        raise ValueError(f"{name} must live on the GPU (got {t.device}); satnerf_amd has no CPU path")
    _same_device(t, name)
    if t.dtype != dtype:
        raise ValueError(f"{name} must be {dtype} (got {t.dtype})")
    if not t.is_contiguous():
        raise ValueError(f"{name} must be contiguous")
    return t


def _same_device(t, name):
    if t.device.index != torch.cuda.current_device():
        raise ValueError(f"{name} lives on {t.device} but the current device is cuda:{torch.cuda.current_device()} "
                         "(wrap the call in torch.cuda.device(...) or torch.cuda.set_device)")


def _rows(t, name, min_cols):
    if t.dim() != 2 or t.shape[1] < min_cols or t.dtype != torch.float32 or not t.is_cuda or t.stride(1) != 1:
        raise ValueError(f"{name} must be a GPU fp32 (N,>={min_cols}) tensor with unit inner stride")
    _same_device(t, name)
    return t, t.stride(0) if t.shape[0] > 1 else t.shape[1]


def pack_stream(flat, idx, scale, want_lo, f16=False):
    n = idx.numel()
    hi = torch.empty(n, dtype=torch.int16, device=flat.device)
    lo = torch.empty(n, dtype=torch.int16, device=flat.device) if want_lo else None
    _lib.call("sr_pack_stream", _p(_chk(flat, "flat")), _p(_chk(idx, "idx", torch.int32)), _p(_chk(scale, "scale")), n, _p(hi), _p(lo),
              n if f16 else 0, _stream())
    return hi, lo


def pack_stream_into(flat, idx, scale, hi, lo, f16=False):
    _lib.call("sr_pack_stream", _p(_chk(flat, "flat")), _p(_chk(idx, "idx", torch.int32)), _p(_chk(scale, "scale")), idx.numel(), _p(hi), _p(lo),
              idx.numel() if f16 else 0, _stream())


def gather_scale_into(flat, idx, scale, out):
    _lib.call("sr_gather_scale_f32", _p(_chk(flat, "flat")), _p(_chk(idx, "idx", torch.int32)), _p(_chk(scale, "scale")), idx.numel(), _p(out),
              _stream())


def gather_scale(flat, idx, scale):
    out = torch.empty(idx.numel(), dtype=torch.float32, device=flat.device)
    _lib.call("sr_gather_scale_f32", _p(_chk(flat, "flat")), _p(_chk(idx, "idx", torch.int32)), _p(_chk(scale, "scale")), idx.numel(), _p(out),
              _stream())
    return out


def ray_sample(rays, u, n_samples):
    rays, stride = _rows(rays, "rays", 8)
    n = rays.shape[0]
    _chk(u, "u")
    if tuple(u.shape) != (n, n_samples):
        raise ValueError(f"u must be ({n},{n_samples}), got {tuple(u.shape)}")
    z = torch.empty(n, n_samples, dtype=torch.float32, device=rays.device)
    _lib.call("sr_ray_sample_fwd", _p(rays), stride, _p(u), n, n_samples, _p(z), _stream())
    return z


def sky(sun, w1, b1, w2, b2):
    sun, stride = _rows(sun, "sun", 3)
    n, hidden = sun.shape[0], w1.shape[0]
    out = torch.empty(n, 3, dtype=torch.float32, device=sun.device)
    _lib.call("sr_sky_fwd", _p(sun), stride, n, hidden, _p(_chk(w1, "w1")), _p(_chk(b1, "b1")), _p(_chk(w2, "w2")), _p(_chk(b2, "b2")), _p(out),
              _stream())
    return out


def satnerf_mlp(org, direction, sun, z, temb, ts, n_points, n_samples, feat, tau, mode, stream_hi, stream_lo, l0, acts=None, fmt=16):
    org, so = _rows(org, "org", 3)
    sun, ss = _rows(sun, "sun", 3)
    sd = 0
    if direction is not None:
        direction, sd = _rows(direction, "dir", 3)
    if z is not None:
        _chk(z, "z")
    _chk(temb, "temb")
    if ts is not None:
        _chk(ts, "ts", torch.int64)
    dev = org.device
    albedo = torch.empty(n_points, 3, dtype=torch.float32, device=dev)
    sigma = torch.empty(n_points, dtype=torch.float32, device=dev)
    sun_v = torch.empty(n_points, dtype=torch.float32, device=dev)
    beta = torch.empty(n_points, dtype=torch.float32, device=dev)
    inp = _lib.MlpInputs(_p(org), so, _p(direction), sd, _p(sun), ss, _p(z), _p(temb), _p(ts), n_points, n_samples)
    ev = kernel_timer.span("mlp_fwd") if kernel_timer is not None else None
    if ev:
        ev[0].record()
    _lib.call("sr_satnerf_mlp_fwd", C.byref(inp), feat, tau, MODES[mode], _p(stream_hi), _p(stream_lo), _p(_chk(l0, "l0")), _p(albedo), _p(sigma),
              _p(sun_v), _p(beta), _p(acts), int(fmt), _stream())
    if ev:
        ev[1].record()
    return albedo, sigma, sun_v, beta


def render_fused_ok(feat, mode, n_samples):
    per_block = _lib.lib().sr_render_points_per_block(int(feat), MODES[mode])
    return per_block > 0 and n_samples >= 2 and per_block % n_samples == 0


def render_fwd(rays, ts, temb, n_samples, feat, tau, mode, stream_hi, stream_lo, l0, sky_w1, sky_b1, sky_w2, sky_b2, z=None, u=None, noise=None,
               noise_std=0.0, seed=0, step_counter=None, tick=False, want_z=True, bank_chunks=0):
    rays, stride = _rows(rays, "rays", 11)
    n, s, dev = rays.shape[0], int(n_samples), rays.device
    if bank_chunks:
        if rays.shape[0] % bank_chunks or ts.numel() != rays.shape[0] or step_counter is None:
            raise ValueError("bank mode: rays / ts must hold bank_chunks x N rows and step_counter is required")
        n = rays.shape[0] // bank_chunks
    _chk(ts, "ts", torch.int64), _chk(temb, "temb")
    for t, nm in ((z, "z"), (u, "u"), (noise, "noise")):
        if t is not None and tuple(_chk(t, nm).shape) != (n, s):
            raise ValueError(f"{nm} must be ({n},{s}), got {tuple(t.shape)}")
    if tick and (step_counter is None or step_counter.numel() < 4):
        raise ValueError("tick=True needs step_counter = a zero-initialised float32 block of 4")
    e = lambda *shape: torch.empty(*shape, dtype=torch.float32, device=dev)
    out = {"z": z if z is not None else (e(n, s) if want_z else None), "albedo": e(n, s, 3), "sun_v": e(n, s), "beta": e(n, s), "sky": e(n, 3),
           "weights": e(n, s), "transparency": e(n, s), "depth": e(n), "rgb": e(n, 3)}
    args = _lib.RenderArgs(_p(rays), stride, _p(ts), _p(temb), n, s, _p(z), _p(u), int(seed) & 0xFFFFFFFFFFFFFFFF,
                           _p(_chk(step_counter, "step_counter", allow_none=True)), int(bool(tick)), _p(noise), float(noise_std), sky_w1.shape[0],
                           _p(_chk(sky_w1, "w1")), _p(_chk(sky_b1, "b1")), _p(_chk(sky_w2, "w2")), _p(_chk(sky_b2, "b2")), int(bank_chunks))
    outs = _lib.RenderOutputs(_p(out["z"]) if z is None else None, _p(out["albedo"]), None, _p(out["sun_v"]), _p(out["beta"]), _p(out["sky"]),
                              _p(out["weights"]), _p(out["transparency"]), _p(out["depth"]), _p(out["rgb"]))
    ev = kernel_timer.span("mlp_fwd") if kernel_timer is not None else None
    if ev:
        ev[0].record()
    _lib.call("sr_satnerf_render_fwd", C.byref(args), feat, tau, MODES[mode], _p(stream_hi), _p(stream_lo), _p(_chk(l0, "l0")), C.byref(outs), _stream())
    if ev:
        ev[1].record()
    return out


def render_train(rays, ts, temb, n_samples, feat, tau, mode, stream_hi, stream_lo, l0, sky_w1, sky_b1, sky_w2, sky_b2, target, acts, u=None,
                 noise=None, noise_std=0.0, seed=0, step_counter=None, sched=None, beta_min=0.05, want_z=False, tick=0, gather=None):
    rays, stride = _rows(rays, "rays", 11)
    n, s, dev = rays.shape[0], int(n_samples), rays.device
    if gather is not None:
        o_rays, o_rgbs, o_ts = gather["out"]
        n = o_rays.shape[0]
        if (stride != 11 or tuple(_chk(o_rays, "out rays").shape) != (n, 11) or tuple(_chk(o_rgbs, "out rgbs").shape) != (n, 3)
                or tuple(_chk(o_ts, "out ts", torch.int64).shape) != (n,) or _chk(gather["idx"], "idx", torch.int64).numel() < int(gather["batches"]) * n
                or target.shape[0] != rays.shape[0] or ts.shape[0] != rays.shape[0] or u is not None or noise is not None):
            raise ValueError("gather: the bank (rays (R,11), ts (R), target (R,3)), idx (>= batches x N) and out = ((N,11), (N,3), (N,)) do not fit")
    _chk(ts, "ts", torch.int64), _chk(temb, "temb")
    for t, nm in ((u, "u"), (noise, "noise")):
        if t is not None and tuple(_chk(t, nm).shape) != (n, s):
            raise ValueError(f"{nm} must be ({n},{s}), got {tuple(t.shape)}")
    per_block = _lib.lib().sr_render_points_per_block(int(feat), MODES[mode])
    if per_block <= 0 or s > 64 or per_block % s:
        raise ValueError(f"no fused training forward for feat={feat}, mode={mode}, n_samples={s}")
    e = lambda *shape: torch.empty(*shape, dtype=torch.float32, device=dev)
    out = {"z": e(n, s) if want_z else None, "albedo": e(n, s, 3), "sigma": e(n, s), "sun_v": e(n, s), "beta": e(n, s), "sky": e(n, 3),
           "loss": e((n * s + per_block - 1) // per_block), "rgb": e(n, 3), "d_sigma": e(n, s), "d_albedo": e(n, s, 3), "d_sun": e(n, s),
           "g_beta": e(n, s), "d_sky": e(n, 3)}
    args = _lib.RenderArgs(_p(rays), stride, _p(ts), _p(temb), n, s, None, _p(u), int(seed) & 0xFFFFFFFFFFFFFFFF,
                           _p(_chk(step_counter, "step_counter", allow_none=True)), int(tick), _p(noise), float(noise_std), sky_w1.shape[0],
                           _p(_chk(sky_w1, "w1")), _p(_chk(sky_b1, "b1")), _p(_chk(sky_w2, "w2")), _p(_chk(sky_b2, "b2")), 0)
    outs = _lib.RenderOutputs(_p(out["z"]), _p(out["albedo"]), _p(out["sigma"]), _p(out["sun_v"]), _p(out["beta"]), _p(out["sky"]), None, None, None, None)
    g = gather or {}
    tr = _lib.TrainArgs(_p(_chk(target, "target")), _p(_chk(sched, "sched", allow_none=True)), float(beta_min), _p(out["loss"]), _p(out["rgb"]),
                        _p(out["d_sigma"]), _p(out["d_albedo"]), _p(out["d_sun"]), _p(out["g_beta"]), _p(out["d_sky"]),
                        _p(g.get("idx")), _p(_chk(g.get("cursor"), "cursor", allow_none=True)), int(g.get("batches", 0)),
                        *([_p(t) for t in g["out"]] if gather is not None else [None, None, None]))
    ev = kernel_timer.span("mlp_fwd") if kernel_timer is not None else None
    if ev:
        ev[0].record()
    _lib.call("sr_satnerf_render_train", C.byref(args), feat, tau, MODES[mode], _p(stream_hi), _p(stream_lo), _p(_chk(l0, "l0")), C.byref(outs),
              C.byref(tr), _p(acts), 8, _stream())
    if ev:
        ev[1].record()
    return out


def composite(z, sigma, noise, noise_std, albedo, sun_v, sky_rgb, clamp_rgb=True):
    n, s = z.shape
    dev = z.device
    _chk(z, "z"), _chk(sigma, "sigma")
    weights = torch.empty(n, s, dtype=torch.float32, device=dev)
    transp = torch.empty(n, s, dtype=torch.float32, device=dev)
    depth = torch.empty(n, dtype=torch.float32, device=dev)
    rgb = torch.empty(n, 3, dtype=torch.float32, device=dev)
    _lib.call("sr_composite_fwd", _p(z), _p(sigma), _p(_chk(noise, "noise", allow_none=True)), float(noise_std), _p(_chk(albedo, "albedo")),
              _p(_chk(sun_v, "sun_v", allow_none=True)), _p(_chk(sky_rgb, "sky", allow_none=True)), n, s, int(clamp_rgb), _p(weights), _p(transp),
              _p(depth), _p(rgb), _stream())
    return weights, transp, depth, rgb


def composite_bwd(z, sigma, noise, noise_std, albedo, sun_v, sky_rgb, weights, transp, g_rgb, g_depth, g_weights, g_transp, clamp_rgb=True):
    n, s = z.shape
    dev = z.device
    d_sigma = torch.empty(n, s, dtype=torch.float32, device=dev)
    d_albedo = torch.empty(n, s, 3, dtype=torch.float32, device=dev)
    d_sun = torch.empty(n, s, dtype=torch.float32, device=dev)
    d_sky = torch.empty(n, 3, dtype=torch.float32, device=dev)
    opt = lambda t, nm: _p(_chk(t, nm, allow_none=True))
    _lib.call("sr_composite_bwd", _p(z), _p(sigma), opt(noise, "noise"), float(noise_std), _p(albedo), opt(sun_v, "sun_v"), opt(sky_rgb, "sky"),
              _p(weights), _p(transp), None, n, s, int(clamp_rgb), opt(g_rgb, "g_rgb"), opt(g_depth, "g_depth"), opt(g_weights, "g_weights"),
              opt(g_transp, "g_transparency"), _p(d_sigma), _p(d_albedo), _p(d_sun), _p(d_sky), _stream())
    return d_sigma, d_albedo, d_sun, d_sky


ACTS = {None: _lib.ACT_NONE, "none": _lib.ACT_NONE, "sin": _lib.ACT_SIN, "relu": _lib.ACT_RELU}
OUT_ACTS = {None: _lib.OUT_NONE, "none": _lib.OUT_NONE, "softplus": _lib.OUT_SOFTPLUS, "sigmoid": _lib.OUT_SIGMOID, "sigmoid_rgb": _lib.OUT_SIGMOID_RGB}


def _linear_srcs(srcs, n_points):
    if not 1 <= len(srcs) <= 2:
        raise ValueError("a linear layer takes one or two concatenated sources")
    arr = (_lib.LinearSrc * len(srcs))()
    for a, (x, act, w0, row_div) in zip(arr, srcs):
        if act not in ACTS:
            raise ValueError(f"unknown activation {act!r} (one of {sorted(k for k in ACTS if k)})")
        x, ld = _rows(x, "linear source", 1)
        if x.shape[0] * row_div < n_points:
            raise ValueError(f"linear source has {x.shape[0]} rows x row_div {row_div} < {n_points} points")
        a.x, a.ld, a.k, a.act, a.w0, a.row_div = x.data_ptr(), ld, x.shape[1], ACTS[act], float(w0), int(row_div)
    return arr


def linear_fwd(srcs, weight, bias, n_points, out_act=None):
    if out_act not in OUT_ACTS:
        raise ValueError(f"unknown output activation {out_act!r} (one of {sorted(k for k in OUT_ACTS if k)})")
    arr = _linear_srcs(srcs, n_points)
    n_out = weight.shape[0]
    if weight.shape[1] != sum(x.shape[1] for x, *_ in srcs):
        raise ValueError(f"weight is {tuple(weight.shape)} but the sources have {sum(x.shape[1] for x, *_ in srcs)} columns")
    y = torch.empty(n_points, n_out, dtype=torch.float32, device=weight.device)
    _lib.call("sr_linear_fwd", arr, len(srcs), _p(_chk(weight, "weight")), _p(_chk(bias, "bias", allow_none=True)), n_points, n_out, OUT_ACTS[out_act],
              _p(y), n_out, _stream())
    return y


def linear_bwd_input(gy, y, out_act, weight, col0, target, n_points):
    arr = _linear_srcs([target], n_points if target[3] == 1 else target[0].shape[0] * target[3])
    k = target[0].shape[1]
    d = torch.empty(n_points, k, dtype=torch.float32, device=gy.device)
    _lib.call("sr_linear_bwd_input", _p(_chk(gy, "gy")), gy.shape[1], _p(_chk(y, "y", allow_none=True)), 0 if y is None else y.shape[1], OUT_ACTS[out_act],
              _p(_chk(weight, "weight")), weight.shape[1], col0, arr, n_points, weight.shape[0], _p(d), k, _stream())
    return d


def linear_bwd_weight(gy, y, out_act, srcs, n_points, n_out, want_bias=True):
    arr = _linear_srcs(srcs, n_points)
    k = sum(x.shape[1] for x, *_ in srcs)
    dw = torch.zeros(n_out, k, dtype=torch.float32, device=gy.device)
    db = torch.zeros(n_out, dtype=torch.float32, device=gy.device) if want_bias else None
    _lib.call("sr_linear_bwd_weight", _p(_chk(gy, "gy")), gy.shape[1], _p(_chk(y, "y", allow_none=True)), 0 if y is None else y.shape[1], OUT_ACTS[out_act],
              arr, len(srcs), n_points, n_out, _p(dw), _p(db), _stream())
    return dw, db


def positional_map(x, n_freqs):
    x, ld = _rows(x, "x", 1)
    out = torch.empty(x.shape[0], 2 * n_freqs * x.shape[1], dtype=torch.float32, device=x.device)
    _lib.call("sr_positional_map", _p(x), ld, x.shape[1], x.shape[0], n_freqs, _p(out), _stream())
    return out


def points_along(rays, dir_col, z):
    rays, stride = _rows(rays, "rays", dir_col + 3)
    n, s = z.shape
    xyz = torch.empty(n * s, 3, dtype=torch.float32, device=rays.device)
    _lib.call("sr_points_along", _p(rays), stride, dir_col, _p(_chk(z, "z")), n, s, _p(xyz), _stream())
    return xyz


IMAGE_COLUMNS = {"rgb": (0, 3), "depth": (3, 4), "acc": (4, 5), "sun": (5, 6), "albedo": (6, 9), "beta": (9, 10), "sky": (10, 13)}


def composite_image(z, sigma, noise, noise_std, albedo, sun_v, beta, sky_rgb):
    n, s = z.shape
    image = torch.empty(n, 13, dtype=torch.float32, device=z.device)
    _lib.call("sr_composite_image", _p(_chk(z, "z")), _p(_chk(sigma, "sigma")), _p(_chk(noise, "noise", allow_none=True)), float(noise_std),
              _p(_chk(albedo, "albedo")), _p(_chk(sun_v, "sun_v")), _p(_chk(beta, "beta")), _p(_chk(sky_rgb, "sky")), n, s, _p(image), _stream())
    return image


def latlonalt_from_depth(rays, depth, center, scene_range):
    import ctypes

    rays, stride = _rows(rays, "rays", 6)
    n = rays.shape[0]
    if depth.reshape(-1).shape[0] != n:
        raise ValueError("depth must have one value per ray")
    depth = _chk(depth.reshape(-1).contiguous().float(), "depth")
    c = (ctypes.c_double * 3)(*[float(v) for v in center])
    out = torch.empty(3, n, dtype=torch.float64, device=rays.device)
    _lib.call("sr_latlonalt_from_depth", _p(rays), stride, _p(depth), n, ctypes.addressof(c), float(scene_range), out[0].data_ptr(),
              out[1].data_ptr(), out[2].data_ptr(), _stream())
    return out[0], out[1], out[2]


RPC_KEYS = ("row_num", "row_den", "col_num", "col_den")
RPC_SCALARS = ("row_offset", "col_offset", "lat_offset", "lon_offset", "alt_offset", "row_scale", "col_scale", "lat_scale", "lon_scale", "alt_scale")


def rpc_rays(rpc, width, height, min_alt, max_alt, center, scene_range, sun_elevation_deg, sun_azimuth_deg, device, want_cache=False):
    import ctypes

    vals = []
    for k in RPC_KEYS:
        c = [float(v) for v in rpc[k]]
        if len(c) != 20:
            raise ValueError(f"rpc[{k!r}] must hold the 20 RPC00B coefficients, got {len(c)}")
        vals += c
    vals += [float(rpc[k]) for k in RPC_SCALARS]
    buf = (ctypes.c_double * 90)(*vals)
    ctr = (ctypes.c_double * 3)(*[float(v) for v in center])
    n = int(width) * int(height)
    dev = torch.device(device)
    with torch.cuda.device(dev):
        rays = torch.empty(n, 11, dtype=torch.float32, device=dev)
        cache = torch.empty(n, 8, dtype=torch.float32, device=dev) if want_cache else None
        _lib.call("sr_rpc_rays", ctypes.addressof(buf), int(width), int(height), float(min_alt), float(max_alt), ctypes.addressof(ctr),
                  float(scene_range), float(sun_elevation_deg), float(sun_azimuth_deg), _p(rays), _p(cache), _stream())
    return rays, cache


def rpc_buffer(rpc):
    vals = []
    for k in RPC_KEYS:
        c = [float(v) for v in rpc[k]]
        if len(c) != 20:
            raise ValueError(f"rpc[{k!r}] must hold the 20 RPC00B coefficients, got {len(c)}")
        vals += c
    vals += [float(rpc[k]) for k in RPC_SCALARS]
    return (C.c_double * 90)(*vals)


def _colrow(colrow):
    colrow = _chk(colrow, "colrow", torch.float64)
    if colrow.dim() != 2 or colrow.shape[1] != 2:
        raise ValueError(f"colrow must be (n, 2) = (col, row) pairs, got {tuple(colrow.shape)}")
    return colrow


def _pts3d(pts3d):
    pts3d = _chk(pts3d, "pts3d", torch.float64)
    if pts3d.dim() != 2 or pts3d.shape[1] != 3:
        raise ValueError(f"pts3d must be (n_pts, 3) ECEF points, got {tuple(pts3d.shape)}")
    return pts3d


def _index(idx, n, name="pts3d_idx"):
    idx = _chk(idx, name, torch.int64)
    if idx.dim() != 1 or idx.numel() != n:
        raise ValueError(f"{name} must be ({n},), got {tuple(idx.shape)}")
    return idx


def rpc_rays_at(rpc, colrow, min_alt, max_alt, center, scene_range, sun_elevation_deg, sun_azimuth_deg, out=None):
    colrow = _colrow(colrow)
    n = colrow.shape[0]
    out = torch.empty(n, 11, dtype=torch.float32, device=colrow.device) if out is None else _chk(out, "out")
    if tuple(out.shape) != (n, 11):
        raise ValueError(f"out must be ({n}, 11), got {tuple(out.shape)}")
    buf, ctr = rpc_buffer(rpc), (C.c_double * 3)(*[float(v) for v in center])
    _lib.call("sr_rpc_rays_at", C.addressof(buf), _p(colrow), n, float(min_alt), float(max_alt), C.addressof(ctr), float(scene_range),
              float(sun_elevation_deg), float(sun_azimuth_deg), _p(out), _stream())
    return out


def reprojection_errors(rpc, colrow, pts3d_idx, pts3d, out=None):
    colrow, pts3d = _colrow(colrow), _pts3d(pts3d)
    n = colrow.shape[0]
    pts3d_idx = _index(pts3d_idx, n)
    out = torch.empty(n, dtype=torch.float32, device=colrow.device) if out is None else _chk(out, "out")
    if out.numel() != n:
        raise ValueError(f"out must hold {n} floats")
    buf = rpc_buffer(rpc)
    _lib.call("sr_reprojection_errors", C.addressof(buf), _p(colrow), _p(pts3d_idx), n, _p(pts3d), pts3d.shape[0], _p(out), _stream())
    return out


def keypoint_weights_scratch(n_pts, n_cams):
    nbytes = C.c_int64(0)
    _lib.call("sr_keypoint_weights_scratch", int(n_pts), int(n_cams), C.byref(nbytes))
    return nbytes.value


def keypoint_weights(pts3d_idx, cam, err, n_pts, n_cams, scratch=None):
    err = _chk(err, "err")
    n = err.numel()
    pts3d_idx, cam = _index(pts3d_idx, n), _index(cam, n, "cam")
    dev = err.device
    scratch = _metric_scratch(scratch, keypoint_weights_scratch(n_pts, n_cams), dev)
    e = torch.empty(int(n_pts), dtype=torch.float32, device=dev)
    w = torch.empty_like(e)
    e_mean = torch.empty(1, dtype=torch.float32, device=dev)
    _lib.call("sr_keypoint_weights", _p(pts3d_idx), _p(cam), _p(err), n, int(n_pts), int(n_cams), _p(scratch),
              scratch.numel() * scratch.element_size(), _p(e), _p(w), _p(e_mean), _stream())
    return e, w, e_mean


def tie_point_depths(rays, pts3d, pts3d_idx, center, scene_range, w=None, out=None):
    rays, pts3d = _chk(rays, "rays"), _pts3d(pts3d)
    if rays.dim() != 2 or rays.shape[1] != 11:
        raise ValueError(f"rays must be (n, 11), got {tuple(rays.shape)}")
    n = rays.shape[0]
    pts3d_idx = _index(pts3d_idx, n)
    if w is not None and (_chk(w, "w").numel() != pts3d.shape[0]):
        raise ValueError(f"w must hold one weight per tie point ({pts3d.shape[0]})")
    out = torch.empty(n, 2, dtype=torch.float32, device=rays.device) if out is None else _chk(out, "out")
    if tuple(out.shape) != (n, 2):
        raise ValueError(f"out must be ({n}, 2), got {tuple(out.shape)}")
    ctr = (C.c_double * 3)(*[float(v) for v in center])
    _lib.call("sr_tie_point_depths", _p(rays), _p(pts3d), _p(pts3d_idx), n, pts3d.shape[0], C.addressof(ctr), float(scene_range), _p(w),
              _p(out), _stream())
    return out


def sample_pdf(bins, weights, u, eps=1e-5):
    n, nb = bins.shape
    _chk(bins, "bins"), _chk(weights, "weights"), _chk(u, "u")
    if tuple(weights.shape) != (n, nb - 1) or u.shape[0] != n:
        raise ValueError(f"sample_pdf: weights must be ({n},{nb - 1}) and u ({n},I)")
    out = torch.empty(n, u.shape[1], dtype=torch.float32, device=bins.device)
    _lib.call("sr_sample_pdf", _p(bins), _p(weights), _p(u), n, nb, u.shape[1], float(eps), _p(out), _stream())
    return out


def sample_pdf_merge(z_coarse, weights_coarse, u, eps=1e-5):
    n, s = z_coarse.shape
    i = u.shape[1]
    _chk(z_coarse, "z_coarse"), _chk(weights_coarse, "weights_coarse"), _chk(u, "u")
    if tuple(weights_coarse.shape) != (n, s) or u.shape[0] != n:
        raise ValueError("sample_pdf_merge: shape mismatch")
    z_fine = torch.empty(n, s + i, dtype=torch.float32, device=z_coarse.device)
    _lib.call("sr_sample_pdf_merge", _p(z_coarse), _p(weights_coarse), _p(u), n, s, i, float(eps), _p(z_fine), _stream())
    return z_fine


def graph_capture(graph):
    import torch.distributed as dist

    if dist.is_available() and dist.is_initialized():
        return torch.cuda.graph(graph, capture_error_mode="thread_local")
    return torch.cuda.graph(graph)


def default_fmt(mode):
    return 8 if mode in ("bf16", "f16") else 16


def _ws_empty(n, dtype, device, slot):
    pad = int(os.environ.get("SATNERF_WS_PAD", "0")) * slot
    if not pad:
        return torch.empty(n, dtype=dtype, device=device)
    item = torch.empty((), dtype=dtype).element_size()
    return torch.empty(n + pad // item, dtype=dtype, device=device)[pad // item:]


def acts_workspace(n_points, feat, device, fmt=16):
    per_tile = _lib.lib().sr_act_elems_per_tile(feat, int(fmt))
    if per_tile <= 0:
        raise ValueError(f"unsupported workspace (feat={feat}, fmt={fmt})")
    return _ws_empty(_lib.lib().sr_workspace_tiles(n_points) * per_tile, torch.int16, device, 1)


def satnerf_mlp_bwd(feat, tau, n_points, bwd_stream, acts, albedo, sigma, sun_v, beta, g_albedo, g_sigma, g_sun_v, g_beta, want_dt=True, fmt=16):
    dev = albedo.device
    n_elems = _lib.lib().sr_dpre_workspace_elems(n_points, feat, int(fmt))
    if n_elems <= 0:
        raise ValueError(f"unsupported workspace (feat={feat}, fmt={fmt})")
    dpre = _ws_empty(n_elems, torch.int16, dev, 2)
    d_t = torch.empty(n_points, tau, dtype=torch.float32, device=dev) if want_dt else None
    opt = lambda t, nm: _p(_chk(t, nm, allow_none=True))
    ev = kernel_timer.span("mlp_bwd") if kernel_timer is not None else None
    if ev:
        ev[0].record()
    _lib.call("sr_satnerf_mlp_bwd", feat, tau, n_points, _p(bwd_stream), _p(acts), _p(_chk(albedo, "albedo")), _p(_chk(sigma, "sigma")),
              _p(_chk(sun_v, "sun_v")), _p(_chk(beta, "beta")), opt(g_albedo, "g_albedo"), opt(g_sigma, "g_sigma"), opt(g_sun_v, "g_sun_v"),
              opt(g_beta, "g_beta"), _p(dpre), _p(d_t), int(fmt), _stream())
    if ev:
        ev[1].record()
    return dpre, d_t


_plan_cache = {}


def wgrad_plan(blocks, n_points, n_wg=0, fmt=16):
    key = (blocks.data_ptr(), int(n_points), int(n_wg), str(blocks.device), int(fmt))
    ent = _plan_cache.get(key)
    if ent is None:
        import ctypes

        host = _chk(blocks, "blocks", torch.int32).cpu().contiguous().clone()
        n_slices = ctypes.c_int(0)
        with torch.cuda.device(blocks.device):
            _lib.call("sr_wgrad_plan", host.data_ptr(), host.shape[0], n_points, n_wg, int(fmt), ctypes.addressof(n_slices))
        if len(_plan_cache) > 64:
            _plan_cache.clear()
        ent = _plan_cache[key] = (host.to(blocks.device), int(n_slices.value), blocks, int(host[0, 11]))
    return ent[0], ent[1], ent[3]


def wgrad_partials(feat, tau, n_points, dpre, acts, blocks, fmt=16, loads=None, n_wg=0):
    plan, n_slices, span = wgrad_plan(blocks, n_points, n_wg=n_wg, fmt=fmt)
    block_floats = 256 * 256 + 256 * 32
    partial = _ws_empty(n_slices * block_floats, torch.float32, dpre.device, 3)
    ev = kernel_timer.span("wgrad") if kernel_timer is not None else None
    if ev:
        ev[0].record()
    if int(fmt) == 8:
        _lib.call("sr_satnerf_wgrad8", feat, tau, n_points, _p(dpre), dpre.numel(), _p(acts), _p(plan), _p(_chk(loads, "loads", torch.int32)), plan.shape[0], n_slices,
                  span, _p(partial), _stream())
    else:
        _lib.call("sr_satnerf_wgrad", feat, tau, n_points, _p(dpre), _p(acts), _p(plan), plan.shape[0], n_slices, _p(partial), _stream())
    if ev:
        ev[1].record()
    return partial, plan


def satnerf_wgrad(feat, tau, n_points, dpre, acts, blocks, gidx, gscale, grad_flat, accumulate=True, fmt=16, loads=None):
    partial, plan = wgrad_partials(feat, tau, n_points, dpre, acts, blocks, fmt, loads)
    _lib.call("sr_unpack_grads", _p(partial), _p(_chk(gidx, "gidx", torch.int32)), _p(_chk(gscale, "gscale")), gidx.numel(), _p(plan),
              _p(_chk(grad_flat, "grad_flat")), int(accumulate), _stream())


def sky_bwd(sun, w1, b1, w2, sky_rgb, d_sky, g_w1, g_b1, g_w2, g_b2):
    sun, stride = _rows(sun, "sun", 3)
    _lib.call("sr_sky_bwd", _p(sun), stride, sun.shape[0], w1.shape[0], _p(w1), _p(b1), _p(w2), _p(_chk(sky_rgb, "sky")), _p(_chk(d_sky, "d_sky")),
              _p(g_w1), _p(g_b1), _p(g_w2), _p(g_b2), _stream())


def embedding_bwd(d_t, ts, n_rays, n_samples, tau, g_emb):
    _lib.call("sr_embedding_bwd", _p(_chk(d_t, "d_t")), _p(_chk(ts, "ts", torch.int64)), n_rays, n_samples, tau, _p(_chk(g_emb, "g_emb")), _stream())


def satnerf_loss(rgb, weights, beta, target, beta_min=0.05, grad_scale=1.0, sched=None):
    n, s = weights.shape
    dev = rgb.device
    loss = torch.empty((n + 3) // 4, dtype=torch.float32, device=dev)
    g_rgb = torch.empty(n, 3, dtype=torch.float32, device=dev)
    g_w = torch.empty(n, s, dtype=torch.float32, device=dev)
    g_b = torch.empty(n, s, dtype=torch.float32, device=dev)
    _lib.call("sr_satnerf_loss", _p(_chk(rgb, "rgb")), _p(_chk(weights, "weights")), _p(_chk(beta, "beta")), _p(_chk(target, "target")), n, s,
              float(beta_min), float(grad_scale), _p(_chk(sched, "sched", allow_none=True)), _p(loss), _p(g_rgb), _p(g_w), _p(g_b), _stream())
    return loss, g_rgb, g_w, g_b


def adam_step(params, grads, exp_avg, exp_avg_sq, step, lr=5e-4, betas=(0.9, 0.999), eps=1e-8, grad_scale=1.0, zero_grad=True):
    _lib.call("sr_adam_step", _p(_chk(params, "params")), _p(_chk(grads, "grads")), _p(_chk(exp_avg, "exp_avg")), _p(_chk(exp_avg_sq, "exp_avg_sq")),
              params.numel(), float(lr), float(betas[0]), float(betas[1]), float(eps), float(grad_scale), int(step), int(zero_grad), _stream())


def pack_all(flat, idx, scale, hi, lo, f32_idx, f32_scale, f32_out, tick=None, n_f16=0):
    _lib.call("sr_pack_all", _p(_chk(flat, "flat")), _p(_chk(idx, "idx", torch.int32)), _p(_chk(scale, "scale")), idx.numel(), _p(hi), _p(lo),
              _p(_chk(f32_idx, "f32_idx", torch.int32)), _p(_chk(f32_scale, "f32_scale")), f32_idx.numel(), _p(f32_out), _p(tick), int(n_f16),
              _stream())


def sc_loss(z, sigma, noise, noise_std, sun_v, lambda_sc):
    n, s = z.shape
    parts = torch.empty((n + 3) // 4, dtype=torch.float32, device=z.device)
    d_sun = torch.empty(n, s, dtype=torch.float32, device=z.device)
    _lib.call("sr_sc_loss", _p(_chk(z, "z")), _p(_chk(sigma, "sigma")), _p(_chk(noise, "noise", allow_none=True)), float(noise_std),
              _p(_chk(sun_v, "sun_v")), n, s, float(lambda_sc), _p(parts), _p(d_sun), _stream())
    return parts, d_sun


def depth_loss(depth, depths, lambda_ds, use_weights=True):
    depths, stride = _rows(depths, "depths", 2 if use_weights else 1)
    n = depth.shape[0]
    parts = torch.empty((n + 255) // 256, dtype=torch.float32, device=depth.device)
    g = torch.empty(n, dtype=torch.float32, device=depth.device)
    _lib.call("sr_depth_loss", _p(_chk(depth, "depth")), _p(depths), stride, int(use_weights), n, float(lambda_ds), _p(parts), _p(g), _stream())
    return parts, g


def ray_setup(rays, u, n_samples, w1, b1, w2, b2, seed=0, step_counter=None, tick=False):
    rays, stride = _rows(rays, "rays", 11)
    n = rays.shape[0]
    z = torch.empty(n, n_samples, dtype=torch.float32, device=rays.device)
    sky_rgb = torch.empty(n, 3, dtype=torch.float32, device=rays.device)
    w = (_p(_chk(w1, "w1")), _p(_chk(b1, "b1")), _p(_chk(w2, "w2")), _p(_chk(b2, "b2")))
    if u is None:
        if tick and (step_counter is None or step_counter.numel() < 4):
            raise ValueError("tick=True needs step_counter = a zero-initialised float32 block of 4")
        _lib.call("sr_ray_setup_rng", _p(rays), stride, int(seed) & 0xFFFFFFFFFFFFFFFF, _p(_chk(step_counter, "step_counter", allow_none=True)),
                  int(bool(tick)), n, n_samples, w1.shape[0], *w, _p(z), _p(sky_rgb), _stream())
    else:
        _lib.call("sr_ray_setup", _p(rays), stride, _p(_chk(u, "u")), n, n_samples, w1.shape[0], *w, _p(z), _p(sky_rgb), _stream())
    return z, sky_rgb


def render_loss(z, sigma, noise, noise_std, albedo, sun_v, beta, sky_rgb, target, beta_min=0.05, sched=None):
    n, s = z.shape
    dev = z.device
    e = lambda *shape: torch.empty(*shape, dtype=torch.float32, device=dev)
    loss, rgb, d_sigma, d_albedo, d_sun, g_beta, d_sky = e((n + 3) // 4), e(n, 3), e(n, s), e(n, s, 3), e(n, s), e(n, s), e(n, 3)
    _lib.call("sr_render_loss", _p(_chk(z, "z")), _p(_chk(sigma, "sigma")), _p(_chk(noise, "noise", allow_none=True)), float(noise_std),
              _p(_chk(albedo, "albedo")), _p(_chk(sun_v, "sun_v")), _p(_chk(beta, "beta")), _p(_chk(sky_rgb, "sky")), _p(_chk(target, "target")), n, s,
              float(beta_min), _p(_chk(sched, "sched", allow_none=True)), _p(loss), _p(rgb), _p(d_sigma), _p(d_albedo), _p(d_sun), _p(g_beta), _p(d_sky),
              _stream())
    return loss, rgb, d_sigma, d_albedo, d_sun, g_beta, d_sky


def gather_batch(rays, rgbs, ts, idx, out=None, cursor=None, batches=0):
    n = idx.numel()
    if cursor is not None:
        if batches < 1 or n % batches or cursor.numel() < 4:
            raise ValueError("cursor mode: idx must hold batches x B indices and cursor 4 floats")
        n //= batches
    if rays.shape[1] != 11 or rgbs.shape[1] != 3:
        raise ValueError("gather_batch expects (N,11) rays and (N,3) rgbs")
    if out is None:
        out = (torch.empty(n, 11, dtype=torch.float32, device=rays.device), torch.empty(n, dtype=torch.int64, device=rays.device),
               torch.empty(n, 3, dtype=torch.float32, device=rays.device))
    _lib.call("sr_gather_batch", _p(_chk(rays, "rays")), _p(_chk(rgbs, "rgbs")), _p(_chk(ts, "ts", torch.int64)), _p(_chk(idx, "idx", torch.int64)), n,
              _p(_chk(out[0], "out_rays")), _p(_chk(out[2], "out_rgbs")), _p(_chk(out[1], "out_ts", torch.int64)),
              _p(_chk(cursor, "cursor", allow_none=True)), int(batches), _stream())
    return out


def gather_setup(rays, rgbs, ts, idx, out, n_samples, w1, b1, w2, b2, z, sky_rgb, seed, step_counter, step_offset=1, cursor=None, batches=0):
    n = idx.numel()
    if cursor is not None:
        if batches < 1 or n % batches or cursor.numel() < 4:
            raise ValueError("cursor mode: idx must hold batches x B indices and cursor 4 floats")
        n //= batches
    if out[0].shape[0] != n or tuple(z.shape) != (n, n_samples) or tuple(sky_rgb.shape) != (n, 3):
        raise ValueError("gather_setup: output shapes do not match the batch")
    _lib.call("sr_gather_setup", _p(_chk(rays, "rays")), _p(_chk(rgbs, "rgbs")), _p(_chk(ts, "ts", torch.int64)), _p(_chk(idx, "idx", torch.int64)), n,
              _p(_chk(out[0], "out_rays")), _p(_chk(out[2], "out_rgbs")), _p(_chk(out[1], "out_ts", torch.int64)),
# ... 250 lines not shown
```

satnerf_amd/packing.py:

```python
from __future__ import annotations

import functools
import os
import math
from collections import OrderedDict

import numpy as np

INV_2PI = np.float32(1.0 / (2.0 * math.pi))
W0_FIRST = 30.0


def aux_steps(tau: int) -> int:
    return (8 + ((tau + 7) // 8) * 8 + 15) // 16


def slot_to_feat(sigma):
    sigma = np.asarray(sigma)
    s, h, j = sigma >> 4, (sigma >> 3) & 1, sigma & 7
    g = j + 8 * (s & 1)
    return 32 * (s >> 1) + (g & 3) + 8 * (g >> 2) + 4 * h


def satnerf_param_shapes(feat=256, tau=4, layers=8, skips=(4,)):
# ... 244 lines not shown
    for l in range(7, 0, -1):
        mats.append(transposed(feat, [(f"fc_net.{2 * l}.weight", feat, phi_f)], in_col0=3 if l == 4 else 0))
    parts = [_serialize(m) for m in mats]
    idx = np.concatenate([p[0] for p in parts]).astype(np.int32)
    scale = np.concatenate([p[1] for p in parts]).astype(np.float32)

    A = auxs
    a_frag = lambda l: A + KS * l
    ACT_FEATS = A + 8 * KS
    ACT_RGBH, ACT_S1, ACT_E1, ACT_S2, ACT_S3 = (ACT_FEATS + KS + k * HS for k in range(5))
    DP_FEATS, DP_SIGMA = 8 * KS, 9 * KS
    DP_RGBH = DP_SIGMA + 1
    DP_S1, DP_E1, DP_S2, DP_S3, DP_HEAD = (DP_RGBH + k * HS for k in range(1, 6))
    tab = _Blocks()
    todo = []
    if feat == 256:
        for l in range(1, 8):
            todo.append(([(16 * l, 16)], [(a_frag(l - 1), 16)], KIND_PHASE, None))
        todo.append(([(DP_FEATS, 16)], [(a_frag(7), 16)], KIND_PHASE, "a7"))
        todo.append(([(0, 8), (DP_SIGMA, 1)], [(a_frag(7), 16)], KIND_PHASE, "a7"))
        todo.append(([(DP_RGBH, 16)], [(ACT_FEATS, 16)], KIND_BF16, "feats"))
        todo.append(([(DP_RGBH + 16, 8), (8, 8)], [(ACT_FEATS, 16)], KIND_BF16, "feats"))
        todo.append(([(DP_S2, 8), (DP_S3, 8)], [(ACT_S1, 8), (ACT_S2, 8)], KIND_PHASE, None))
        todo.append(([(DP_HEAD, 1)], [(ACT_RGBH, 8), (ACT_S3, 8)], KIND_PHASE, None))
        todo.append(([(DP_HEAD, 1)], [(ACT_E1, 8)], KIND_PHASE, None))
    else:
        def tile_job(r0, nr, c0, nc, kind, key=None):
            for rb in range(0, nr, 16):
                for cb in range(0, max(nc, 1), 16):
                    todo.append(([(r0 + rb, min(16, nr - rb))], [(c0 + cb, min(16, nc - cb))] if nc else [], kind, key))
        for l in range(1, 8):
            tile_job(KS * l, KS, a_frag(l - 1), KS, KIND_PHASE, f"L{l}")
        tile_job(DP_FEATS, KS, a_frag(7), KS, KIND_PHASE, "G1")
        tile_job(DP_SIGMA, 1, a_frag(7), KS, KIND_PHASE)
        tile_job(0, KS, 0, 0, KIND_PHASE)
        tile_job(DP_RGBH, 3 * HS, ACT_FEATS, KS, KIND_BF16)
        tile_job(DP_S2, HS, ACT_S1, HS, KIND_PHASE)
        tile_job(DP_S3, HS, ACT_S2, HS, KIND_PHASE)
        for c0 in (ACT_RGBH, ACT_S3, ACT_E1):
            tile_job(DP_HEAD, 1, c0, HS, KIND_PHASE)
    groups = {}
    for i, t in enumerate(todo):
        if t[3] is not None:
            groups.setdefault(t[3], []).append(i)
    order = [None] * len(todo)
    free = lambda p: p < len(order) and order[p] is None
    for members in groups.values():
        p = next((p for p in range(len(order)) if all(free(p + 8 * j) for j in range(len(members)))), None)
        if p is None:
            continue
        for j, i in enumerate(members):
            order[p + 8 * j] = i
    rest = iter(i for i in range(len(todo)) if i not in order)
    order = [i if i is not None else next(rest) for i in order]
    assert sorted(order) == list(range(len(todo)))
    for i in order:
        tab.add(*todo[i][:3])
    jobs = {"L0": _Job(tab, 0, [])}
    for l in range(1, 8):
        jobs[f"L{l}"] = _Job(tab, KS * l, [a_frag(l - 1)])
    jobs["G1"] = _Job(tab, DP_FEATS, [a_frag(7)])
    jobs["G2"] = _Job(tab, DP_RGBH, [ACT_FEATS])
    jobs["S2"] = _Job(tab, DP_S2, [ACT_S1])
    jobs["S3"] = _Job(tab, DP_S3, [ACT_S2])
    jobs["H"] = _Job(tab, DP_HEAD, [ACT_RGBH, ACT_S3, ACT_E1])

    gidx = np.full(n_params, -1, np.int64)
    gscale = np.zeros(n_params, np.float32)
    inv_f, inv_h, inv16 = feat_to_slot(feat), feat_to_slot(half), feat_to_slot(32)[:16]

    def put(name, job, row_slots, seg, col_slots, scale_=1.0, cols=None):
        off, shp = offsets[name]
        row_slots, col_slots = np.asarray(row_slots), np.asarray(col_slots)
        where = (lambda r, c: job.pos_aux(r, c)) if seg == "aux" else (lambda r, c: job.pos(r, seg, c))
        if len(shp) == 1:
            gidx[off + np.arange(shp[0])] = where(row_slots, np.full_like(row_slots, int(col_slots)))
            gscale[off:off + shp[0]] = scale_
            return
        cols = np.arange(shp[1]) if cols is None else np.asarray(cols)
        r = np.arange(shp[0])[:, None]
        flat = off + r * shp[1] + cols[None, :]
        gidx[flat] = where(np.broadcast_to(row_slots[:, None], flat.shape), np.broadcast_to(col_slots[None, :], flat.shape))
        gscale[flat] = scale_

    AUXC = _Mat
    put("fc_net.0.weight", jobs["L0"], inv_f, "aux", AUXC.AUX_XYZ + np.arange(3), W0_FIRST)
    put("fc_net.0.bias", jobs["L0"], inv_f, "aux", AUXC.AUX_ONE, W0_FIRST)
    for l in range(1, 8):
        name, job = f"fc_net.{2 * l}", jobs[f"L{l}"]
        if l == 4:
            put(name + ".weight", job, inv_f, "aux", AUXC.AUX_XYZ + np.arange(3), cols=[0, 1, 2])
            put(name + ".weight", job, inv_f, 0, inv_f, cols=3 + np.arange(feat))
        else:
            put(name + ".weight", job, inv_f, 0, inv_f)
        put(name + ".bias", job, inv_f, "aux", AUXC.AUX_ONE)
    put("feats_from_xyz.weight", jobs["G1"], inv_f, 0, inv_f)
    put("feats_from_xyz.bias", jobs["G1"], inv_f, "aux", AUXC.AUX_ONE)
    put("sigma_from_xyz.0.weight", jobs["G1"], np.array([feat + inv16[0]]), 0, inv_f)
    put("sigma_from_xyz.0.bias", jobs["G1"], np.array([feat + inv16[0]]), "aux", AUXC.AUX_ONE)
    for k, (name, aux0) in enumerate((("rgb_from_xyzdir.0", None), ("sun_v_net.0", AUXC.AUX_SUN), ("beta_from_xyz.0", AUXC.AUX_T))):
        rows = half * k + inv_h
        put(name + ".weight", jobs["G2"], rows, 0, inv_f, cols=np.arange(feat))
        put(name + ".bias", jobs["G2"], rows, "aux", AUXC.AUX_ONE)
        if aux0 is not None:
            extra = offsets[name + ".weight"][1][1] - feat
            put(name + ".weight", jobs["G2"], rows, "aux", aux0 + np.arange(extra), cols=feat + np.arange(extra))
    put("sun_v_net.2.weight", jobs["S2"], inv_h, 0, inv_h)
    put("sun_v_net.2.bias", jobs["S2"], inv_h, "aux", AUXC.AUX_ONE)
    put("sun_v_net.4.weight", jobs["S3"], inv_h, 0, inv_h)
    put("sun_v_net.4.bias", jobs["S3"], inv_h, "aux", AUXC.AUX_ONE)
    put("rgb_from_xyzdir.2.weight", jobs["H"], inv16[[0, 1, 2]], 0, inv_h)
    put("rgb_from_xyzdir.2.bias", jobs["H"], inv16[[0, 1, 2]], "aux", AUXC.AUX_ONE)
    put("sun_v_net.6.weight", jobs["H"], inv16[[3]], 1, inv_h)
    put("sun_v_net.6.bias", jobs["H"], inv16[[3]], "aux", AUXC.AUX_ONE)
    put("beta_from_xyz.2.weight", jobs["H"], inv16[[4]], 2, inv_h)
    put("beta_from_xyz.2.bias", jobs["H"], inv16[[4]], "aux", AUXC.AUX_ONE)
    return dict(idx=idx, scale=scale, blocks=tab.table(), block_rows=tab.rows, block_cols=tab.cols, gidx=gidx.astype(np.int32), gscale=gscale,
                n_params=n_params, auxs=auxs, offsets=offsets, feat=feat)


SRC_DPRE, SRC_ACTS = 1, 2
RAW16, PHASE8, MX8 = 0, 1, 2
WG8_OLD_INTS = 20
WG9_DUTY_INTS = 4 * 5 * 4
WG9_SCAN_INTS = 8
EMAX_FEATS, EMAX_RAW = 14, 15
WG9_MASK_INTS = 1
WG9_VARIANT_INTS = 4
WG8_LOAD_INTS = WG8_OLD_INTS + WG9_DUTY_INTS + WG9_SCAN_INTS + WG9_MASK_INTS + WG9_VARIANT_INTS
WG9_THIN = ((1, True, "thin"), (3, False, "none"), (0, True, "thin"), (2, True, "none"), (2, False, "none"), (0, False, "none"))
WG9_DUMP_FRAG = 34
def fmt8_geometry(feat=256):
    KS, HS = feat // 16, feat // 32
    MT = KS // 2
    body = (9 * KS + 5 * HS) // 2
    gpu = 16 // MT
    d8_scale = body + 2
    return dict(KS=KS, HS=HS, MT=MT, MTH=HS // 2, D8_SIGMA=body, D8_HEAD=body + 1, D8_SCALE=d8_scale, GROUPS_PER_UNIT=gpu,
                D8_UNITS=d8_scale + (14 + gpu - 1) // gpu, A8_SCALE=body,
                DP_FEATS=8 * KS, DP_SIGMA=9 * KS, DP_RGBH=9 * KS + 1, DP_HEAD=9 * KS + 1 + 5 * HS, ACT_FEATS=8 * KS)


D8_SIGMA, D8_HEAD, D8_SCALE, D8_UNITS, A8_SCALE = (fmt8_geometry(256)[k] for k in ("D8_SIGMA", "D8_HEAD", "D8_SCALE", "D8_UNITS", "A8_SCALE"))


def act8_units(auxs, feat=256):
    return auxs + fmt8_geometry(feat)["A8_SCALE"] + 1


def dpre8_units(feat=256):
    return fmt8_geometry(feat)["D8_UNITS"]


def dpre8_source(f, feat=256):
    g8 = fmt8_geometry(feat)
    if f == g8["DP_SIGMA"]:
        return dict(unit=g8["D8_SIGMA"], codec=RAW16, half=0, group=EMAX_RAW)
    if f == g8["DP_HEAD"]:
        return dict(unit=g8["D8_HEAD"], codec=RAW16, half=0, group=EMAX_RAW)
    if f < g8["DP_SIGMA"]:
        u, half = f >> 1, f & 1
        g, k = u // g8["MT"], u % g8["MT"]
    else:
        u, half = (f - 1) >> 1, (f - 1) & 1
        h = u - 9 * g8["MT"]
        g, k = 9 + h // g8["MTH"], h % g8["MTH"]
    gpu = g8["GROUPS_PER_UNIT"]
    return dict(unit=u, codec=MX8, half=half, scale_unit=g8["D8_SCALE"] + g // gpu, scale_byte=(g % gpu) * g8["MT"] + k, group=g)


def act8_source(f, auxs, feat=256):
    g8 = fmt8_geometry(feat)
    a = f - auxs
    assert a >= 0, "aux fragments are fetched by the kernel itself"
    if g8["ACT_FEATS"] <= a < g8["ACT_FEATS"] + g8["KS"]:
        return dict(unit=auxs + (a >> 1), codec=MX8, half=a & 1, scale_unit=auxs + g8["A8_SCALE"], scale_byte=(a - g8["ACT_FEATS"]) >> 1)
    return dict(unit=auxs + (a >> 1), codec=PHASE8, half=a & 1)


@functools.lru_cache(maxsize=8)
def wgrad8_loads(feat=256, tau=4):
    bm = backward_maps(feat, tau)
    auxs = bm["auxs"]
    out = np.zeros((len(bm["block_rows"]), WG8_LOAD_INTS), np.int32)
    for b, (rows, cols) in enumerate(zip(bm["block_rows"], bm["block_cols"])):
        loads, areas = [], []

        def area_of(src, unit):
            if (src, unit) not in areas:
                areas.append((src, unit))
            return areas.index((src, unit))

        for base, frags, src, lookup in ((0, rows, SRC_DPRE, lambda f: dpre8_source(f, feat)), (16, cols, SRC_ACTS, lambda f: act8_source(f, auxs, feat))):
            pos = 0
            while pos < len(frags):
                d = lookup(frags[pos])
                desc = src | (d["codec"] << 2) | (d["unit"] << 4) | ((base + pos) << 12)
                if d["codec"] == RAW16:
                    pos += 1
                else:
                    assert d["half"] == 0 and pos + 1 < len(frags) and frags[pos + 1] == frags[pos] + 1, (b, frags, pos)
                    if d["codec"] == MX8:
                        desc |= (area_of(src, d["scale_unit"]) << 18) | (d["scale_byte"] << 20)
                    pos += 2
                loads.append(desc)
        assert len(loads) <= 16 and len(areas) <= 3, (b, len(loads), len(areas))
        order = list(range(5, 16)) + [4, 3, 2, 1, 0]
        for w, desc in zip(order, loads):
            out[b, w] = desc
        for k, (src, unit) in enumerate(areas):
            out[b, 16 + k] = src | (unit << 4)
    duties = wgrad9_duties(feat, tau)
    out[:, WG8_OLD_INTS:WG8_OLD_INTS + WG9_DUTY_INTS] = duties
    out[:, WG8_OLD_INTS + WG9_DUTY_INTS:WG8_OLD_INTS + WG9_DUTY_INTS + WG9_SCAN_INTS] = wgrad9_pair_groups(feat, tau)
    out[:, WG8_OLD_INTS + WG9_DUTY_INTS + WG9_SCAN_INTS + WG9_MASK_INTS:] = wgrad9_variants(feat, tau)
    g = bm["gidx"][bm["gidx"] >= 0].astype(np.int64)
    blk, w = g // WG_BLOCK_FLOATS, g % WG_BLOCK_FLOATS
    main = w < 256 * 256
    quad = 2 * ((w[main] // 256) // 128) + (w[main] % 256) // 128
    for b, q in zip(blk[main], quad):
        out[b, WG8_OLD_INTS + WG9_DUTY_INTS + WG9_SCAN_INTS] |= 1 << int(q)
    return out


@functools.lru_cache(maxsize=8)
def wgrad9_pair_groups(feat=256, tau=4):
    bm = backward_maps(feat, tau)
    out = np.full((len(bm["block_rows"]), WG9_SCAN_INTS), -1, np.int32)
    for b, rows in enumerate(bm["block_rows"]):
        pos = 0
        while pos < len(rows):
            d = dpre8_source(rows[pos], feat)
            assert pos % 2 == 0, (b, rows, "a row operand must start a 32-row pair")
            out[b, pos // 2] = d["group"]
            if d["codec"] == RAW16:
                assert pos + 1 == len(rows), (b, rows, "a raw row fragment must be the last of its block")
                pos += 1
            else:
                pos += 2
    return out


def wgrad9_thin_blocks(feat=256, tau=4):
    bm = backward_maps(feat, tau)
    out = {}
    if os.environ.get("SATNERF_WGRAD_THIN", "1") == "0" or bm["auxs"] != 1:
        return out
    for b, (rows, cols) in enumerate(zip(bm["block_rows"], bm["block_cols"])):
        if len(rows) == 1 and dpre8_source(rows[0], feat)["codec"] == RAW16 and bm["blocks"][b, 8] == KIND_PHASE and len(cols) in (8, 16):
            if all(act8_source(c, bm["auxs"], feat)["codec"] == PHASE8 for c in cols):
                out[b] = len(cols) // 2
    return out


@functools.lru_cache(maxsize=8)
def wgrad9_variants(feat=256, tau=4):
    thin = wgrad9_thin_blocks(feat, tau)
    out = np.zeros((len(backward_maps(feat, tau)["block_rows"]), WG9_VARIANT_INTS), np.int32)
    vid = lambda v: 1 + WG9_THIN.index(v)
    for b, n in thin.items():
        out[b] = ([vid((1, True, "thin")), vid((1, True, "thin")), vid((3, False, "none")), vid((3, False, "none"))] if n == 8 else
                  [vid((0, True, "thin")), vid((2, True, "none")), vid((2, False, "none")), vid((0, False, "none"))])
    return out


@functools.lru_cache(maxsize=8)
def wgrad9_duties(feat=256, tau=4):
    bm = backward_maps(feat, tau)
    auxs = bm["auxs"]
    out = np.zeros((len(bm["block_rows"]), 4, 5, 4), np.int32)
    thin = wgrad9_thin_blocks(feat, tau)
    for b, (rows, cols) in enumerate(zip(bm["block_rows"], bm["block_cols"])):
        out[b, :, 0:2] = [SRC_DPRE, 0, WG9_DUMP_FRAG, 0]
        out[b, :, 2:4] = [SRC_ACTS, auxs, WG9_DUMP_FRAG, 16 * auxs]
        out[b, :, 4] = [SRC_ACTS, 0, WG9_DUMP_FRAG, 0]
        raw_wave = 0
        for a in range(auxs):
            out[b, 1 + a, 4] = [SRC_ACTS, a, 32 + a, 0]
        if b in thin:
            d = dpre8_source(rows[0], feat)
            out[b, 0, 4] = [SRC_DPRE, d["unit"], 0, 0]
            share = ([1, 1, 3, 3] if thin[b] == 8 else [0, 2, 2, 0])
            j = 0
            for w, k in enumerate(share):
                for slot in range(k):
                    c = act8_source(cols[2 * j], auxs, feat)
                    assert c["codec"] == PHASE8 and c["half"] == 0 and cols[2 * j + 1] == cols[2 * j] + 1
                    out[b, w, slot] = [SRC_ACTS, c["unit"], 16 + 2 * j, 16 * auxs]
                    j += 1
            assert j == thin[b]
            continue
        for base, frags, src, lookup, d0 in ((0, rows, SRC_DPRE, lambda f: dpre8_source(f, feat), 0),
                                             (16, cols, SRC_ACTS, lambda f: act8_source(f, auxs, feat), 2)):
            pos, n_df = 0, 0
            while pos < len(frags):
                d = lookup(frags[pos])
                if d["codec"] == RAW16:
                    assert src == SRC_DPRE and raw_wave == 0, (b, frags)
                    out[b, 0, 4] = [src, d["unit"], base + pos, 0]
                    raw_wave = 1
                    pos += 1
                    continue
                assert d["half"] == 0 and pos + 1 < len(frags) and frags[pos + 1] == frags[pos] + 1, (b, frags, pos)
                assert (d["codec"] == MX8) == (src == SRC_DPRE or bm["blocks"][b, 8] == KIND_BF16), (b, frags, pos)
                assert n_df < 8, (b, frags)
                scale = 16 * d["scale_unit"] + d["scale_byte"] if d["codec"] == MX8 else 16 * auxs
# ... 37 lines not shown
```

satnerf_amd/train.py:

```python
from __future__ import annotations

import os

import torch
import torch.distributed as dist


_VOTES = 0


def _fmt_of(args):
    from . import ops
    from .rendering import _mode_of

    fmt = getattr(args, "bwd_fmt", None)
    fmt = ops.default_fmt(_mode_of(args)) if fmt is None else int(fmt)
    if fmt not in (8, 16, 32):
        raise ValueError(f"bwd_fmt must be 8, 16 or 32, got {fmt}")
    if fmt == 32 and _mode_of(args) != "bf16x3":
        raise ValueError("bwd_fmt=32 (parity-grade backward) belongs to mlp_mode='bf16x3'")
    if fmt == 8 and _mode_of(args) not in ("bf16", "f16"):
        raise ValueError("the 8-bit workspace format belongs to mlp_mode='bf16' / 'f16'")
    return fmt

# ... 41 lines not shown
    return loss


class FlatState:

    def __init__(self, modules):
        self.modules = list(modules)
        sizes = [sum(p.numel() for p in m.parameters()) for m in self.modules]
        dev = next(self.modules[0].parameters()).device
        self.params = torch.empty(sum(sizes), dtype=torch.float32, device=dev)
        self.grads = torch.zeros_like(self.params)
        off = 0
        for m, n in zip(self.modules, sizes):
            pslice, gslice = self.params[off:off + n], self.grads[off:off + n]
            if hasattr(m, "_flatten"):
                m._flatten(buffer=_filled(pslice, m))
                m.flat_grads(buffer=gslice)
            else:
                o = 0
                for p in m.parameters():
                    k = p.numel()
                    pslice[o:o + k].copy_(p.data.reshape(-1))
                    p.data = pslice[o:o + k].view(p.shape)
                    p.grad = gslice[o:o + k].view(p.shape)
                    o += k
            off += n

    def zero_grad(self):
        self.grads.zero_()

    def allreduce_mean_(self, world_size):
        if world_size > 1:
            dist.all_reduce(self.grads, op=dist.ReduceOp.SUM)
            self.grads.mul_(1.0 / world_size)


def _filled(dst, module):
    flat = torch.cat([p.data.reshape(-1) for p in module.parameters()])
    dst.copy_(flat)
    return dst


def shard_rays(n_total, rank, world_size):
    base, rem = divmod(n_total, world_size)
    start = rank * base + min(rank, rem)
    return start, start + base + (1 if rank < rem else 0)


class _LazyLoss:

    def __init__(self, parts):
        self.parts = parts

    def item(self):
        return float(self.parts.sum().item())

    def detach(self):
        return self.parts.sum()

    def __float__(self):
        return self.item()


class Trainer:

    def __init__(self, models, args, world_size=1, lr=5e-4, loss_fn=None, use_graph=True, steps_per_epoch=None, lr_gamma=0.9,
                 warmup_epochs=2, lr_steps_per_epoch=None):
        self._snerf = args.model == "s-nerf"
        self._caller_args = args
        if args.model == "sat-nerf" and steps_per_epoch is None:
            import warnings

            warnings.warn("Trainer(steps_per_epoch=None): constant learning rate and SatNerfLoss from the first step; main.py decays the rate "
                          "by 0.9 per epoch and trains sat-nerf with SNerfLoss for 2 epochs -- pass steps_per_epoch = len(dataset) // batch_size",
                          stacklevel=2)
        if self._snerf:
            from .rendering import _as_satnerf

            models, args = _as_satnerf(models, args)
        self.models, self.args, self.world, self.lr = models, args, world_size, lr
        self._collective = world_size > 1 or (os.environ.get("SATNERF_FORCE_ALLREDUCE", "0") == "1" and dist.is_available() and dist.is_initialized())
        self.lr0, self.lr_gamma, self.steps_per_epoch, self.warmup_epochs = lr, lr_gamma, steps_per_epoch, warmup_epochs
        self.lr_steps_per_epoch = lr_steps_per_epoch if lr_steps_per_epoch else steps_per_epoch
        if args.model == "sat-nerf" and args.n_importance > 0 and loss_fn is None:
            raise NotImplementedError("sat-nerf with n_importance > 0 has no trainable reference loss (metrics.py:22 shape error): pass loss_fn")
        mods = [models["coarse"]] + ([models["fine"]] if "fine" in models else []) + ([models["t"]] if "t" in models else [])
        self.state = FlatState(mods)
        p = self.state.params
        self.exp_avg, self.exp_avg_sq = torch.zeros_like(p), torch.zeros_like(p)
        self.n_steps = 0
        self.adam_state = torch.zeros(4, dtype=torch.float32, device=p.device)
        self.sched = self.adam_state
        self._sched_host = None
        self._apply_schedule()
        self._kernel_rng = False
        self._seed = int(torch.initial_seed()) & 0x7FFFFFFFFFFFFFFF
        self._adam_in_graph = False
        self.loss_fn = loss_fn
        from .rendering import _mode_of

        self.direct = (loss_fn is None and p.is_cuda and args.n_importance == 0 and args.model == "sat-nerf"
                       and hasattr(models["coarse"], "fused_training") and models["coarse"].fused_training(_mode_of(args), _fmt_of(args)))
        self.use_graph = use_graph and self.direct
        self._late_idx = None
        if self.direct and mods[0] is models["coarse"] and len(mods) == 2 and mods[1] is models.get("t"):
            import numpy as np

            from . import packing

            gidx = packing.backward_maps(models["coarse"].feat, models["coarse"].t_embedding_dims)["gidx"]
            late = np.concatenate([np.nonzero(gidx < 0)[0], np.arange(gidx.size, p.numel())])
            self._late_idx = torch.from_numpy(late.astype(np.int32)).to(p.device)
        self._graph, self._static, self._graph_banks = None, None, None
        self._pre_setup, self._pre_bufs = None, None
        self._pack_in_tail, self._gather_in_fwd, self._packed_version = False, None, None
        self.max_inflight = int(os.environ.get("SATNERF_MAX_INFLIGHT", "0"))
        self.pace_every = max(1, int(os.environ.get("SATNERF_PACE_EVERY", "1")))
        self.last_rgb = None
        self.last_loss = None
        self.jitter = lambda n, s, device: torch.rand(n, s, device=device)

    def _forward_backward(self, rays, ts, rgbs, depth=None):
        from . import ops
        from .rendering import _mode_of

        if self._snerf:
            ts = self._zero_ts(ts)
            if depth is not None:
                depth = (depth[0], self._zero_ts(depth[1]), depth[2])
        model, emb = self.models["coarse"], self.models["t"]
        args = self.args
        n, s = rays.shape[0], args.n_samples
        mode = _mode_of(args)
        feat, tau = model.feat, model.t_embedding_dims
        ticking = self._kernel_rng or self._adam_in_graph
        pit = self._pack_in_tail and ticking
        if pit:
            hi, lo, l0, bstream, maps = model.packed_static(mode)
        else:
            model.repack(mode, backward=True, tick=self.adam_state if ticking else None)
            hi, lo, l0 = model.packed(mode)
            bstream, maps = model.packed_backward()
        sk = model.sky_color
        u = None if self._kernel_rng else self.jitter(n, s, rays.device)
        noise_std = float(args.noise_std)
        nz = torch.randn(n, s, device=rays.device) if noise_std != 0 else None
        fmt = _fmt_of(args)
        acts = ops.acts_workspace(n * s, feat, rays.device, fmt)
        sc_on = float(getattr(args, "sc_lambda", 0.0)) > 0
        fused = self._pre_setup is None and self._fused_forward()
        gather, self._gather_in_fwd = self._gather_in_fwd, None
        if pit and not fused:
            raise RuntimeError("pack-in-tail steps need the one-launch training forward (it ticks the step counter)")
        if fused:
            src = (gather["bank"].rays, gather["bank"].ts, gather["bank"].rgbs) if gather is not None else (rays, ts, rgbs)
            r = ops.render_train(src[0], src[1], emb.weight.data, s, feat, tau, mode, hi, lo, l0, sk[0].weight.data, sk[0].bias.data, sk[2].weight.data,
                                 sk[2].bias.data, src[2], acts, u=u, noise=nz, noise_std=noise_std, seed=self._seed, step_counter=self.adam_state,
                                 sched=self.sched, want_z=sc_on, tick=2 if pit else 0,
                                 gather=None if gather is None else dict(idx=gather["idx"], cursor=gather["cursor"], batches=gather["batches"],
                                                                         out=(rays, rgbs, ts)))
            z, sky, loss, self.last_rgb = r["z"], r["sky"], r["loss"], r["rgb"]
            albedo, sigma, sun_v, beta = r["albedo"].view(-1, 3), r["sigma"].view(-1), r["sun_v"].view(-1), r["beta"].view(-1)
            d_sigma, d_albedo, d_sun, g_beta, d_sky = r["d_sigma"], r["d_albedo"], r["d_sun"], r["g_beta"], r["d_sky"]
        else:
            if self._pre_setup is not None:
                (z, sky), self._pre_setup = self._pre_setup, None
            else:
                z, sky = ops.ray_setup(rays, u, s, sk[0].weight.data, sk[0].bias.data, sk[2].weight.data, sk[2].bias.data, seed=self._seed,
                                       step_counter=self.adam_state)
            albedo, sigma, sun_v, beta = ops.satnerf_mlp(rays[:, 0:3], rays[:, 3:6], rays[:, 8:11], z, emb.weight.data, ts, n * s, s, feat, tau, mode,
                                                         hi, lo, l0, acts=acts, fmt=fmt)
            if s <= 64:
                loss, self.last_rgb, d_sigma, d_albedo, d_sun, g_beta, d_sky = ops.render_loss(z, sigma.view(n, s), nz, noise_std, albedo.view(n, s, 3),
                                                                                               sun_v.view(n, s), beta.view(n, s), sky, rgbs,
                                                                                               sched=self.sched)
            else:
                weights, transp, _, rgb = ops.composite(z, sigma.view(n, s), nz, noise_std, albedo.view(n, s, 3), sun_v.view(n, s), sky)
                loss, g_rgb, g_w, g_beta = ops.satnerf_loss(rgb, weights, beta.view(n, s), rgbs, sched=self.sched)
                d_sigma, d_albedo, d_sun, d_sky = ops.composite_bwd(z, sigma.view(n, s), nz, noise_std, albedo.view(n, s, 3), sun_v.view(n, s), sky,
                                                                   weights, transp, g_rgb, None, g_w, None)
                self.last_rgb = rgb
        dpre, d_t = ops.satnerf_mlp_bwd(feat, tau, n * s, bstream, acts, albedo, sigma, sun_v, beta, d_albedo, d_sigma, d_sun, g_beta.view(-1), fmt=fmt)
        partial, plan = ops.wgrad_partials(feat, tau, n * s, dpre, acts, maps["blocks"], fmt, maps["loads8"])
        if sc_on:
            loss = torch.cat([loss.view(-1), self._sc_pass(rays, ts, z, noise_std).view(-1)])
        if depth is not None:
            loss = torch.cat([loss.view(-1), self._depth_pass(*depth, noise_std * 0.9).view(-1)])
        tail = (partial, plan, maps["gidx"], maps["gscale"], model.flat_grads(), rays[:, 8:11], sk[0].weight.data, sk[0].bias.data,
                sk[2].weight.data, sky, d_sky, sk[0].weight.grad, sk[0].bias.grad, sk[2].weight.grad, sk[2].bias.grad, d_t, ts, n, s, tau,
                emb.weight.grad)
        if self._adam_in_graph and not self._collective and self._late_idx is not None and os.environ.get("SATNERF_TAIL_ADAM", "1") != "0":
            ops.grad_tail_adam(*tail, self.state.params, self.exp_avg, self.exp_avg_sq, self._late_idx, self.adam_state, lr=-1.0,
                               grad_scale=1.0 / self.world, pack=model.pack_scatter(mode) if pit else None)
            return loss
        if pit and not self._collective:
            raise RuntimeError("single-GPU pack-in-tail steps end in sr_grad_tail_adam")
        ops.grad_tail(*tail)
        if self._adam_in_graph:
            if self._collective:
                dist.all_reduce(self.state.grads, op=dist.ReduceOp.SUM)
            if pit:
                self._update_and_pack()
            else:
                ops.adam_step_graph(self.state.params, self.state.grads, self.exp_avg, self.exp_avg_sq, self.adam_state, lr=-1.0,
                                    grad_scale=1.0 / self.world, zero_grad=True)
        return loss

    def _update_and_pack(self):
        from . import ops
        from .rendering import _mode_of

        ops.adam_step_pack(self.state.params, self.state.grads, self.exp_avg, self.exp_avg_sq, self.adam_state,
                           pack=self.models["coarse"].pack_scatter(_mode_of(self.args)), lr=-1.0, grad_scale=1.0 / self.world, zero_grad=True)

    def _fused_forward(self):
        from . import ops
        from .rendering import _mode_of

        s, mode = self.args.n_samples, _mode_of(self.args)
        return (_fmt_of(self.args) == 8 and s <= 64 and ops.render_fused_ok(self.models["coarse"].feat, mode, s)
                and os.environ.get("SATNERF_TRAIN_FUSED", "1") != "0" and os.environ.get("SATNERF_FWD_V1", "0") != "1")

    def _sc_pass(self, rays, ts, z, noise_std):
        from . import ops
        from .rendering import _mode_of

        model, emb, args = self.models["coarse"], self.models["t"], self.args
        n, s = z.shape
        mode = _mode_of(args)
        feat, tau = model.feat, model.t_embedding_dims
        hi, lo, l0 = model.packed(mode)
        bstream, maps = model.packed_backward()
        nz = torch.randn(n, s, device=rays.device) if noise_std != 0 else None
        fmt = _fmt_of(args)
        acts = ops.acts_workspace(n * s, feat, rays.device, fmt)
        albedo, sigma, sun_v, beta = ops.satnerf_mlp(rays[:, 0:3], rays[:, 8:11], rays[:, 8:11], z, emb.weight.data, ts, n * s, s, feat, tau, mode,
                                                     hi, lo, l0, acts=acts, fmt=fmt)
        loss, d_sun = ops.sc_loss(z, sigma.view(n, s), nz, noise_std, sun_v.view(n, s), float(args.sc_lambda))
        dpre, _ = ops.satnerf_mlp_bwd(feat, tau, n * s, bstream, acts, albedo, sigma, sun_v, beta, None, None, d_sun, None, want_dt=False, fmt=fmt)
        ops.satnerf_wgrad(feat, tau, n * s, dpre, acts, maps["blocks"], maps["gidx"], maps["gscale"], model.flat_grads(), accumulate=True, fmt=fmt,
                          loads=maps["loads8"])
        return loss

    def _depth_pass(self, rays, ts, depths, noise_std):
        from . import ops
        from .rendering import _mode_of

        model, emb, args = self.models["coarse"], self.models["t"], self.args
        n, s = rays.shape[0], args.n_samples
        mode = _mode_of(args)
        feat, tau = model.feat, model.t_embedding_dims
        hi, lo, l0 = model.packed(mode)
        bstream, maps = model.packed_backward()
        sk = model.sky_color
        u = None if self._kernel_rng else self.jitter(n, s, rays.device)
        nz = torch.randn(n, s, device=rays.device) if noise_std != 0 else None
        z, sky = ops.ray_setup(rays, u, s, sk[0].weight.data, sk[0].bias.data, sk[2].weight.data, sk[2].bias.data, seed=self._seed + 1,
                               step_counter=self.adam_state)
        fmt = _fmt_of(args)
        acts = ops.acts_workspace(n * s, feat, rays.device, fmt)
        albedo, sigma, sun_v, beta = ops.satnerf_mlp(rays[:, 0:3], rays[:, 3:6], rays[:, 8:11], z, emb.weight.data, ts, n * s, s, feat, tau, mode,
                                                     hi, lo, l0, acts=acts, fmt=fmt)
        weights, transp, depth, _ = ops.composite(z, sigma.view(n, s), nz, noise_std, albedo.view(n, s, 3), sun_v.view(n, s), sky)
        loss, g_depth = ops.depth_loss(depth, depths, float(args.ds_lambda), use_weights=not getattr(args, "ds_noweights", False))
        d_sigma, _, _, _ = ops.composite_bwd(z, sigma.view(n, s), nz, noise_std, albedo.view(n, s, 3), sun_v.view(n, s), sky, weights, transp,
                                             None, g_depth, None, None)
        dpre, _ = ops.satnerf_mlp_bwd(feat, tau, n * s, bstream, acts, albedo, sigma, sun_v, beta, None, d_sigma, None, None, want_dt=False, fmt=fmt)
        ops.satnerf_wgrad(feat, tau, n * s, dpre, acts, maps["blocks"], maps["gidx"], maps["gscale"], model.flat_grads(), accumulate=True, fmt=fmt,
                          loads=maps["loads8"])
        return loss

    def current_epoch(self):
        return 0 if not self.steps_per_epoch else (self.n_steps + 1) // int(self.steps_per_epoch)

    def _pace(self):
        every = self.pace_every
        k = self.max_inflight // every
        if k <= 0 or self.n_steps % every:
            return
        ring = self.__dict__.get("_pace_ring")
        if ring is None:
            ring = self._pace_ring = [torch.cuda.Event() for _ in range(k)]
            for ev in ring:
                ev.record()
        ev = ring[(self.n_steps // every) % k]
        ev.synchronize()
        ev.record()

    def _zero_ts(self, ts):
        n = ts.shape[0]
        cache = self.__dict__.setdefault("_zero_ts_cache", {})
        if n not in cache:
            cache[n] = torch.zeros(n, dtype=torch.int64, device=self.state.params.device)
        return cache[n]

    def warming_up(self):
        if self._snerf:
            return True
        return bool(self.steps_per_epoch) and self.args.model == "sat-nerf" and self.current_epoch() < self.warmup_epochs

    def _apply_schedule(self):
        if self.steps_per_epoch:
            self.lr = self.lr0 * self.lr_gamma ** (self.n_steps // int(self.lr_steps_per_epoch))
        host = (float(self.lr), 1.0 if self.warming_up() else 0.0)
        if host != self._sched_host:
            self.adam_state[1:3].copy_(torch.tensor(host, dtype=torch.float32))
            self._sched_host = host

    def set_lr(self, lr):
        self.lr0 = self.lr = float(lr)
        self._apply_schedule()

    def save_ckpt(self, path):
        sd = {}
        for prefix, key in (("nerf_coarse.", "coarse"), ("nerf_fine.", "fine"), ("embedding_t.", "t")):
            if key in self.models and not (self._snerf and key == "t"):
                sd.update({prefix + k: v.detach().cpu().clone() for k, v in self.models[key].state_dict().items()})
        torch.save({"state_dict": sd, "global_step": self.n_steps, "epoch": self.current_epoch(),
                    "optimizer": {"exp_avg": self.exp_avg.cpu(), "exp_avg_sq": self.exp_avg_sq.cpu(), "lr": self.lr, "step": self.n_steps,
                                  "lr0": self.lr0, "device_step": float(self.adam_state[0].item()), "noise_std": float(self.args.noise_std),
                                  "jitter_seed": int(self._seed)}}, path)

    def load_ckpt(self, path):
        ck = torch.load(path, map_location="cpu", weights_only=False)
        sd = ck["state_dict"]
        for prefix, key in (("nerf_coarse.", "coarse"), ("nerf_fine.", "fine"), ("embedding_t.", "t")):
            if key in self.models and not (self._snerf and key == "t"):
                part = {k[len(prefix):]: v for k, v in sd.items() if k.startswith(prefix)}
                if not part:
                    raise KeyError(f"checkpoint holds no '{prefix}*' entries")
                self.models[key].load_state_dict(part)
        self.state.zero_grad()
        self.n_steps = int(ck.get("global_step", 0))
        opt = ck.get("optimizer")
        if opt is not None and "exp_avg" in opt:
# ... 254 lines not shown
```

Baseline: 2.785 million rays/s.

## Hand off head gradients from fused training forward directly into dpre workspace

The fused render-train kernel now computes the head pre-activation gradients (albedo, sun, sigma, beta) and writes them straight into the dpre workspace, and can skip writing the per-point fp32 gradient arrays. The MLP backward kernel gets a HEADS variant that reads those slots from dpre instead of recomputing them from albedo/sigma/sun/beta and their gradients. This removes several fp32 per-point global-memory write and read round trips between the two kernels. In exchange it adds a new dpre workspace allocation per step and couples the two kernels' layouts. The path is on by default behind an environment flag.

```diff
diff --git a/include/satrender.h b/include/satrender.h
--- a/include/satrender.h
+++ b/include/satrender.h
@@ -120,6 +120,11 @@
 } sr_train_args;
 int sr_satnerf_render_train(const sr_render_args* in, int feat, int tau, int mode, const uint16_t* stream_hi, const uint16_t* stream_lo,
                             const float* l0, const sr_render_outputs* out, const sr_train_args* train, uint16_t* acts, int act_fmt, void* stream);
+int sr_satnerf_render_train_handoff(const sr_render_args* in, int feat, int tau, int mode, const uint16_t* stream_hi, const uint16_t* stream_lo,
+                                    const float* l0, const sr_render_outputs* out, const sr_train_args* train, uint16_t* acts, int act_fmt,
+                                    uint16_t* dpre, int64_t dpre_elems, int dpre_fmt, int skip_point_grads, void* stream);
+int sr_satnerf_mlp_bwd_handoff(int feat, int tau, int64_t n_points, const uint16_t* bwd_stream, const uint16_t* acts, uint16_t* dpre, float* d_t,
+                               int fmt, void* stream);
 
 int sr_satnerf_mlp_bwd(int feat, int tau, int64_t n_points, const uint16_t* bwd_stream, const uint16_t* acts,
                        const float* albedo, const float* sigma, const float* sun_v, const float* beta, const float* g_albedo,
diff --git a/satnerf_amd/_lib.py b/satnerf_amd/_lib.py
--- a/satnerf_amd/_lib.py
+++ b/satnerf_amd/_lib.py
@@ -55,6 +55,8 @@
     "sr_satnerf_render_fwd": (_i, [_vp, _i, _i, _i, _vp, _vp, _vp, _vp, _vp]),
     "sr_render_points_per_block": (_i, [_i, _i]),
     "sr_satnerf_render_train": (_i, [_vp, _i, _i, _i, _vp, _vp, _vp, _vp, _vp, _vp, _i, _vp]),
+    "sr_satnerf_render_train_handoff": (_i, [_vp, _i, _i, _i, _vp, _vp, _vp, _vp, _vp, _vp, _i, _vp, _i64, _i, _i, _vp]),
+    "sr_satnerf_mlp_bwd_handoff": (_i, [_i, _i, _i64, _vp, _vp, _vp, _vp, _i, _vp]),
     "sr_pack_stream": (_i, [_vp, _vp, _vp, _i64, _vp, _vp, _i64, _vp]),
     "sr_dpre_elems_per_tile": (_i64, [_i, _i]),
     "sr_workspace_tiles": (_i64, [_i64]),
diff --git a/satnerf_amd/csrc/head_grads.h b/satnerf_amd/csrc/head_grads.h
--- /dev/null
+++ b/satnerf_amd/csrc/head_grads.h
@@ -0,0 +1,22 @@
+#pragma once
+#include "common.h"
+
+namespace sr {
+
+__device__ __forceinline__ float head_d_albedo(float g, float albedo, int c) {
+#pragma clang fp contract(off)
+  const float t = albedo + 0.001f, k = 1.0f / 1.002f;
+  const float s = t * k;
+  const float one_minus_s = c > 0 ? __builtin_fmaf(-t, k, 1.0f) : 1.0f - s;
+  return g * 1.002f * s * one_minus_s;
+}
+__device__ __forceinline__ float head_d_sigmoid(float g, float s) {
+#pragma clang fp contract(off)
+  return g * s * (1.0f - s);
+}
+__device__ __forceinline__ float head_d_softplus(float g, float y) {
+#pragma clang fp contract(off)
+  return g * (1.0f - expf(-y));
+}
+
+}
diff --git a/satnerf_amd/csrc/mlp_api.hip b/satnerf_amd/csrc/mlp_api.hip
--- a/satnerf_amd/csrc/mlp_api.hip
+++ b/satnerf_amd/csrc/mlp_api.hip
@@ -65,7 +65,8 @@
 }
 
 static int render_launch(const char* who, const sr_render_args* in, int feat, int tau, int mode, const uint16_t* stream_hi, const uint16_t* stream_lo,
-                         const float* l0, const sr_render_outputs* out, const sr_train_args* tr, uint16_t* acts, int act_fmt, void* stream) {
+                         const float* l0, const sr_render_outputs* out, const sr_train_args* tr, uint16_t* acts, int act_fmt, uint16_t* dpre,
+                         int64_t dpre_elems, int dpre_fmt, int skip_point_grads, void* stream) {
   SR_REQUIRE(in != nullptr && out != nullptr, "%s: null argument block", who);
   const int per_block = sr_render_points_per_block(feat, mode);
   SR_REQUIRE(per_block > 0, "%s: no fused kernel for feat=%d mode=%d (256: every mode; 512: SR_MODE_BF16 / SR_MODE_F16)", who, feat, mode);
@@ -82,7 +83,15 @@
     SR_REQUIRE(mode == SR_MODE_BF16 || mode == SR_MODE_F16, "%s: the fused training forward exists for SR_MODE_BF16 / SR_MODE_F16 (8-bit saved state)", who);
     SR_REQUIRE(acts != nullptr && act_fmt == SR_FMT8, "%s: needs the SR_FMT8 activation workspace", who);
     SR_REQUIRE(in->n_samples <= 64, "%s: n_samples=%d unsupported (one wave per ray: <= 64); use the separate launches", who, in->n_samples);
-    SR_REQUIRE(tr->target && tr->loss_parts && tr->d_sigma && tr->d_albedo && tr->d_sun_v && tr->g_beta && tr->d_sky && out->sky, "%s: null training output", who);
+    SR_REQUIRE(tr->target && tr->loss_parts && tr->d_sky && out->sky, "%s: null training output", who);
+    SR_REQUIRE(skip_point_grads || (tr->d_sigma && tr->d_albedo && tr->d_sun_v && tr->g_beta), "%s: null training output", who);
+    if (dpre != nullptr) {
+      SR_REQUIRE(dpre_fmt == SR_FMT8 || (dpre_fmt == SR_FMT16 && feat == kFeat), "%s: dpre_fmt must be 8, or 16 at width %d (got %d)", who, kFeat, dpre_fmt);
+      SR_REQUIRE(dpre_elems >= sr_dpre_workspace_elems(in->n_rays * in->n_samples, feat, dpre_fmt),
+                 "%s: the dpre workspace holds %lld elements, sr_dpre_workspace_elems asks for %lld", who, (long long)dpre_elems,
+                 (long long)sr_dpre_workspace_elems(in->n_rays * in->n_samples, feat, dpre_fmt));
+    }
+    SR_REQUIRE(!skip_point_grads || dpre != nullptr, "%s: skip_point_grads needs the dpre workspace (nothing else carries the gradients)", who);
     SR_REQUIRE(out->albedo && out->sigma && out->sun_v && out->beta, "%s: the four per-point outputs are required (the dX pass reads them)", who);
     if (tr->gather_idx != nullptr) {
       SR_REQUIRE(tr->cursor && tr->batches >= 1 && tr->batches < (1 << 24), "%s: the in-launch sampler needs a cursor block and 1 <= batches < 2^24", who);
@@ -113,6 +122,7 @@
     t.d_sigma = tr->d_sigma, t.d_albedo = tr->d_albedo, t.d_sun = tr->d_sun_v, t.g_beta = tr->g_beta, t.d_sky = tr->d_sky;
     t.gather_idx = (const long long*)tr->gather_idx, t.cursor = tr->cursor, t.batches = (unsigned)tr->batches;
     t.out_rays = tr->out_rays, t.out_rgbs = tr->out_rgbs, t.out_ts = (long long*)tr->out_ts;
+    t.dpre = (uint4*)dpre, t.dpre_fmt = dpre_fmt, t.skip_point_grads = skip_point_grads;
   }
   p.stream_hi = (const char*)stream_hi, p.stream_lo = (const char*)stream_lo, p.l0 = (const float4*)l0;
   p.albedo = out->albedo, p.sigma = out->sigma, p.sun_v = out->sun_v, p.beta = out->beta;
@@ -129,12 +139,21 @@
 
 extern "C" int sr_satnerf_render_fwd(const sr_render_args* in, int feat, int tau, int mode, const uint16_t* stream_hi, const uint16_t* stream_lo,
                                      const float* l0, const sr_render_outputs* out, void* stream) {
-  return render_launch("sr_satnerf_render_fwd", in, feat, tau, mode, stream_hi, stream_lo, l0, out, nullptr, nullptr, 0, stream);
+  return render_launch("sr_satnerf_render_fwd", in, feat, tau, mode, stream_hi, stream_lo, l0, out, nullptr, nullptr, 0, nullptr, 0, 0, 0, stream);
 }
 
 extern "C" int sr_satnerf_render_train(const sr_render_args* in, int feat, int tau, int mode, const uint16_t* stream_hi, const uint16_t* stream_lo,
                                        const float* l0, const sr_render_outputs* out, const sr_train_args* train, uint16_t* acts, int act_fmt,
                                        void* stream) {
   SR_REQUIRE(train != nullptr, "sr_satnerf_render_train: null training argument block");
-  return render_launch("sr_satnerf_render_train", in, feat, tau, mode, stream_hi, stream_lo, l0, out, train, acts, act_fmt, stream);
+  return render_launch("sr_satnerf_render_train", in, feat, tau, mode, stream_hi, stream_lo, l0, out, train, acts, act_fmt, nullptr, 0, 0, 0, stream);
 }
+
+extern "C" int sr_satnerf_render_train_handoff(const sr_render_args* in, int feat, int tau, int mode, const uint16_t* stream_hi,
+                                               const uint16_t* stream_lo, const float* l0, const sr_render_outputs* out, const sr_train_args* train,
+                                               uint16_t* acts, int act_fmt, uint16_t* dpre, int64_t dpre_elems, int dpre_fmt, int skip_point_grads,
+                                               void* stream) {
+  SR_REQUIRE(train != nullptr && dpre != nullptr, "sr_satnerf_render_train_handoff: null training argument block or dpre workspace");
+  return render_launch("sr_satnerf_render_train_handoff", in, feat, tau, mode, stream_hi, stream_lo, l0, out, train, acts, act_fmt, dpre, dpre_elems,
+                       dpre_fmt, skip_point_grads != 0, stream);
+}
diff --git a/satnerf_amd/csrc/mlp_bwd.hip b/satnerf_amd/csrc/mlp_bwd.hip
--- a/satnerf_amd/csrc/mlp_bwd.hip
+++ b/satnerf_amd/csrc/mlp_bwd.hip
@@ -15,14 +15,14 @@
 
 using namespace sr;
 
-extern "C" int sr_satnerf_mlp_bwd(int feat, int tau, int64_t n_points, const uint16_t* bwd_stream, const uint16_t* acts, const float* albedo,
-                                  const float* sigma, const float* sun_v, const float* beta, const float* g_albedo, const float* g_sigma,
-                                  const float* g_sun_v, const float* g_beta, uint16_t* dpre, float* d_t, int fmt, void* stream) {
-  SR_REQUIRE(feat == kFeat || feat == 512, "sr_satnerf_mlp_bwd: feat=%d unsupported (this build handles %d and 512)", feat, kFeat);
-  SR_REQUIRE(tau >= 1 && tau <= 24, "sr_satnerf_mlp_bwd: tau=%d unsupported (1..24)", tau);
-  SR_REQUIRE(fmt == SR_FMT16 || fmt == SR_FMT8, "sr_satnerf_mlp_bwd: workspace format must be 16 or 8 (got %d)", fmt);
-  SR_REQUIRE(feat == kFeat || fmt == SR_FMT8, "sr_satnerf_mlp_bwd: feat=512 trains on the 8-bit workspaces only");
-  SR_REQUIRE(bwd_stream && acts && dpre && albedo && sigma && sun_v && beta, "sr_satnerf_mlp_bwd: null pointer argument");
+static int bwd_launch(const char* who, int feat, int tau, int64_t n_points, const uint16_t* bwd_stream, const uint16_t* acts, const float* albedo,
+                      const float* sigma, const float* sun_v, const float* beta, const float* g_albedo, const float* g_sigma, const float* g_sun_v,
+                      const float* g_beta, uint16_t* dpre, float* d_t, int fmt, int heads_ready, void* stream) {
+  SR_REQUIRE(feat == kFeat || feat == 512, "%s: feat=%d unsupported (this build handles %d and 512)", who, feat, kFeat);
+  SR_REQUIRE(tau >= 1 && tau <= 24, "%s: tau=%d unsupported (1..24)", who, tau);
+  SR_REQUIRE(fmt == SR_FMT16 || fmt == SR_FMT8, "%s: workspace format must be 16 or 8 (got %d)", who, fmt);
+  SR_REQUIRE(feat == kFeat || fmt == SR_FMT8, "%s: feat=512 trains on the 8-bit workspaces only", who);
+  SR_REQUIRE(bwd_stream && acts && dpre && (heads_ready || (albedo && sigma && sun_v && beta)), "%s: null pointer argument", who);
   if (n_points <= 0) return 0;
   BwdParams p;
   p.g_albedo = g_albedo, p.g_sigma = g_sigma, p.g_sun = g_sun_v, p.g_beta = g_beta;
@@ -30,9 +30,23 @@
   p.acts = (const uint4*)acts, p.dpre = (uint4*)dpre, p.d_t = d_t;
   p.stream = (const char*)bwd_stream;
   p.n_points = n_points, p.tau = tau, p.auxs = aux_steps(tau);
+  p.heads_ready = heads_ready;
   p.emax = fmt == SR_FMT8 ? (uint4*)(dpre + sr_workspace_tiles(n_points) * sr_dpre_elems_per_tile(feat, fmt)) : nullptr;
   if (feat == 512) return launch_bwd512(p, fmt, (hipStream_t)stream);
   return fmt == SR_FMT8 ? launch_bwd_fmt<SR_FMT8>(p, (hipStream_t)stream) : launch_bwd_fmt<SR_FMT16>(p, (hipStream_t)stream);
+}
+
+extern "C" int sr_satnerf_mlp_bwd(int feat, int tau, int64_t n_points, const uint16_t* bwd_stream, const uint16_t* acts, const float* albedo,
+                                  const float* sigma, const float* sun_v, const float* beta, const float* g_albedo, const float* g_sigma,
+                                  const float* g_sun_v, const float* g_beta, uint16_t* dpre, float* d_t, int fmt, void* stream) {
+  return bwd_launch("sr_satnerf_mlp_bwd", feat, tau, n_points, bwd_stream, acts, albedo, sigma, sun_v, beta, g_albedo, g_sigma, g_sun_v, g_beta, dpre,
+                    d_t, fmt, 0, stream);
+}
+
+extern "C" int sr_satnerf_mlp_bwd_handoff(int feat, int tau, int64_t n_points, const uint16_t* bwd_stream, const uint16_t* acts, uint16_t* dpre,
+                                          float* d_t, int fmt, void* stream) {
+  return bwd_launch("sr_satnerf_mlp_bwd_handoff", feat, tau, n_points, bwd_stream, acts, nullptr, nullptr, nullptr, nullptr, nullptr, nullptr,
+                    nullptr, nullptr, dpre, d_t, fmt, 1, stream);
 }
 
 extern "C" int64_t sr_bwd_stream_elems(int feat, int tau) {
diff --git a/satnerf_amd/csrc/mlp_bwd.inc b/satnerf_amd/csrc/mlp_bwd.inc
--- a/satnerf_amd/csrc/mlp_bwd.inc
+++ b/satnerf_amd/csrc/mlp_bwd.inc
@@ -2,6 +2,7 @@
 #include "mlp_device.h"
 #include "mlp_params.h"
 #include "codec8.h"
+#include "head_grads.h"
 
 namespace sr {
 inline namespace SR_FEAT_NS {
@@ -230,7 +231,7 @@
 
 typedef uint32_t u32x32w __attribute__((ext_vector_type(32)));
 typedef uint32_t u32x4w __attribute__((ext_vector_type(4)));
-template <int FMT, bool TRUNK_ASM = false>
+template <int FMT, bool TRUNK_ASM = false, bool HEADS = false>
 __global__ void __launch_bounds__(Mode<1>::NW * 64) satnerf_bwd_kernel(const BwdParams prm) {
   constexpr int NW = Mode<1>::NW;
   constexpr bool kStreamG1 = false;
@@ -267,51 +268,6 @@
     pt[j] = (tile0 + j) * 32 + pl;
     valid[j] = pt[j] < prm.n_points;
     dpre[j] = prm.dpre + (tile0 + j) * DK * 64 + lane;
-  }
-
-  uint4 dhead[kBT][1], dsig[kBT];
-  uint32_t e_feats[kBT] = {}, e_raw[kBT] = {};
-#pragma unroll
-  for (int j = 0; j < kBT; ++j) {
-    float v[8] = {0.f, 0.f, 0.f, 0.f, 0.f, 0.f, 0.f, 0.f}, sg = 0.f;
-    const long q = pt[j];
-    uint4 fs = {};
-    if constexpr (FMT == SR_FMT8)
-      fs = prm.acts[((tile0 + j) * (long)act8_units(prm.auxs) + prm.auxs + kA8Scale) * 64 + lane];
-    if (valid[j]) {
-      if (h == 0) {
-        if (prm.g_albedo) {
-#pragma unroll
-          for (int c = 0; c < 3; ++c) {
-            const float s = (prm.albedo[q * 3 + c] + 0.001f) * (1.0f / 1.002f);
-            v[c] = prm.g_albedo[q * 3 + c] * 1.002f * s * (1.0f - s);
-          }
-        }
-        if (prm.g_sun) {
-          const float s = prm.sun_v[q];
-          v[3] = prm.g_sun[q] * s * (1.0f - s);
-        }
-        if (prm.g_sigma) sg = prm.g_sigma[q] * (1.0f - expf(-prm.sigma[q]));
-      } else if (prm.g_beta) {
-        v[0] = prm.g_beta[q] * (1.0f - expf(-prm.beta[q]));
-      }
-    }
-    dhead[j][0] = make_uint4(pack_bf16x2(v[0], v[1]), pack_bf16x2(v[2], v[3]), pack_bf16x2(v[4], v[5]), pack_bf16x2(v[6], v[7]));
-    dsig[j] = make_uint4(pack_bf16x2(sg, 0.f), 0u, 0u, 0u);
-    dpre[j][(FMT == SR_FMT8 ? kD8Head : kDpHead) * 64] = dhead[j][0];
-    dpre[j][(FMT == SR_FMT8 ? kD8Sigma : kDpSigma) * 64] = dsig[j];
-    if constexpr (FMT == SR_FMT8) {
-      const uint32_t w4[4] = {fs.x, fs.y, kMT > 8 ? fs.z : 0u, kMT > 8 ? fs.w : 0u};
-      e_feats[j] = max_byte<kMT>(w4);
-      const uint32_t hw[5] = {dhead[j][0].x, dhead[j][0].y, dhead[j][0].z, dhead[j][0].w, dsig[j].x};
-      uint32_t m = 0;
-#pragma unroll
-      for (int k = 0; k < 5; ++k) {
-        const uint32_t lo = (hw[k] & 0x7fffu) >> 7, hi = (hw[k] >> 23) & 0xffu;
-        m = m > lo ? m : lo, m = m > hi ? m : hi;
-      }
-      e_raw[j] = m;
-    }
   }
 
   constexpr int NPH = FMT == SR_FMT8 ? 1 : 2;
@@ -335,6 +291,50 @@
   };
   static_assert(PreSched::kAhead == 4, "the wave's phase staging ring has four slots");
   stage_phase(0, PreSched::frag(0)), stage_phase(1, PreSched::frag(1)), stage_phase(2, PreSched::frag(2)), stage_phase(3, PreSched::frag(3));
+
+  uint4 dhead[kBT][1], dsig[kBT];
+  uint32_t e_feats[kBT] = {}, e_raw[kBT] = {};
+#pragma unroll
+  for (int j = 0; j < kBT; ++j) {
+    float v[8] = {0.f, 0.f, 0.f, 0.f, 0.f, 0.f, 0.f, 0.f}, sg = 0.f;
+    const long q = pt[j];
+    uint4 fs = {};
+    if constexpr (FMT == SR_FMT8)
+      fs = prm.acts[((tile0 + j) * (long)act8_units(prm.auxs) + prm.auxs + kA8Scale) * 64 + lane];
+    if constexpr (HEADS) {
+      dhead[j][0] = dpre[j][(FMT == SR_FMT8 ? kD8Head : kDpHead) * 64];
+      dsig[j] = dpre[j][(FMT == SR_FMT8 ? kD8Sigma : kDpSigma) * 64];
+    } else {
+    if (valid[j]) {
+      if (h == 0) {
+        if (prm.g_albedo) {
+#pragma unroll
+          for (int c = 0; c < 3; ++c) v[c] = head_d_albedo(prm.g_albedo[q * 3 + c], prm.albedo[q * 3 + c], c);
+        }
+        if (prm.g_sun) v[3] = head_d_sigmoid(prm.g_sun[q], prm.sun_v[q]);
+        if (prm.g_sigma) sg = head_d_softplus(prm.g_sigma[q], prm.sigma[q]);
+      } else if (prm.g_beta) {
+        v[0] = head_d_softplus(prm.g_beta[q], prm.beta[q]);
+      }
+    }
+    dhead[j][0] = make_uint4(pack_bf16x2(v[0], v[1]), pack_bf16x2(v[2], v[3]), pack_bf16x2(v[4], v[5]), pack_bf16x2(v[6], v[7]));
+    dsig[j] = make_uint4(pack_bf16x2(sg, 0.f), 0u, 0u, 0u);
+    dpre[j][(FMT == SR_FMT8 ? kD8Head : kDpHead) * 64] = dhead[j][0];
+    dpre[j][(FMT == SR_FMT8 ? kD8Sigma : kDpSigma) * 64] = dsig[j];
+    }
+    if constexpr (FMT == SR_FMT8) {
+      const uint32_t w4[4] = {fs.x, fs.y, kMT > 8 ? fs.z : 0u, kMT > 8 ? fs.w : 0u};
+      e_feats[j] = max_byte<kMT>(w4);
+      const uint32_t hw[5] = {dhead[j][0].x, dhead[j][0].y, dhead[j][0].z, dhead[j][0].w, dsig[j].x};
+      uint32_t m = 0;
+#pragma unroll
+      for (int k = 0; k < 5; ++k) {
+        const uint32_t lo = (hw[k] & 0x7fffu) >> 7, hi = (hw[k] >> 23) & 0xffu;
+        m = m > lo ? m : lo, m = m > hi ? m : hi;
+      }
+      e_raw[j] = m;
+    }
+  }
 
   uint32_t* emax_cells = reinterpret_cast<uint32_t*>(smem + kNSLOT * kBSlot + NW * (4 * NPT * 1024));
   uint32_t* emax[kBT];
@@ -608,13 +608,17 @@
 }
 
 
+template <int FMT, bool TRUNK_ASM, bool HEADS>
+int launch_bwd_heads(const BwdParams& p, size_t lds, hipStream_t st) {
+  constexpr int NW = Mode<1>::NW;
+  if (!ensure_dynamic_lds((const void*)satnerf_bwd_kernel<FMT, TRUNK_ASM, HEADS>, lds)) return 1;
+  const long tiles = (p.n_points + 31) / 32;
+  hipLaunchKernelGGL((satnerf_bwd_kernel<FMT, TRUNK_ASM, HEADS>), dim3((unsigned)((tiles + NW * kBT - 1) / (NW * kBT))), dim3(NW * 64), lds, st, p);
+  return check_launch("satnerf_bwd_kernel");
+}
 template <int FMT, bool TRUNK_ASM>
 int launch_bwd_kernel(const BwdParams& p, size_t lds, hipStream_t st) {
-  constexpr int NW = Mode<1>::NW;
-  if (!ensure_dynamic_lds((const void*)satnerf_bwd_kernel<FMT, TRUNK_ASM>, lds)) return 1;
-  const long tiles = (p.n_points + 31) / 32;
-  hipLaunchKernelGGL((satnerf_bwd_kernel<FMT, TRUNK_ASM>), dim3((unsigned)((tiles + NW * kBT - 1) / (NW * kBT))), dim3(NW * 64), lds, st, p);
-  return check_launch("satnerf_bwd_kernel");
+  return p.heads_ready ? launch_bwd_heads<FMT, TRUNK_ASM, true>(p, lds, st) : launch_bwd_heads<FMT, TRUNK_ASM, false>(p, lds, st);
 }
 
 template <int FMT>
diff --git a/satnerf_amd/csrc/mlp_fwd_io.inc b/satnerf_amd/csrc/mlp_fwd_io.inc
--- a/satnerf_amd/csrc/mlp_fwd_io.inc
+++ b/satnerf_amd/csrc/mlp_fwd_io.inc
@@ -5,6 +5,17 @@
 inline namespace SR_FEAT_NS {
 
 constexpr int kRendFloats = 7;
+
+__device__ __forceinline__ void store_head_rows(uint4* dpre, int fmt, long pt, const float (&v)[6]) {
+  const int dk = fmt == SR_FMT8 ? kD8Units : kDpFrags, u_head = fmt == SR_FMT8 ? kD8Head : kDpHead, u_sigma = fmt == SR_FMT8 ? kD8Sigma : kDpSigma;
+  uint4* tile = dpre + (pt >> 5) * dk * 64 + (pt & 31);
+  const uint32_t z = pack_bf16x2(0.f, 0.f);
+  tile[u_head * 64] = make_uint4(pack_bf16x2(v[0], v[1]), pack_bf16x2(v[2], v[3]), z, z);
+  tile[u_head * 64 + 32] = make_uint4(pack_bf16x2(v[4], 0.f), z, z, z);
+  tile[u_sigma * 64] = make_uint4(pack_bf16x2(v[5], 0.f), 0u, 0u, 0u);
+  tile[u_sigma * 64 + 32] = make_uint4(z, 0u, 0u, 0u);
+}
+
 template <bool REND, int NW>
 __device__ __forceinline__ void write_outputs(const FwdParams& prm, const PointIn& in, const f32x16& acc, float sig, float* r_z, int wave, int lane) {
   constexpr int P = NW * 32;
@@ -39,10 +50,16 @@
     const int rays_here = P / S;
     const bool train = prm.train.target != nullptr;
     const bool warm = prm.train.sched != nullptr && prm.train.sched[2] != 0.f;
+    const bool handoff = train && prm.train.dpre != nullptr;
     float loss_part = 0.f;
     for (int lr = wave; lr < rays_here; lr += NW) {
       const long ray = (long)blockIdx.x * rays_here + lr;
-      if (ray >= prm.rend.n_rays) break;
+      if (ray >= prm.rend.n_rays) {
+        if (!handoff) break;
+        const float none[6] = {0.f, 0.f, 0.f, 0.f, 0.f, 0.f};
+        if (lane < S) store_head_rows(prm.train.dpre, prm.train.dpre_fmt, ray * S + lane, none);
+        continue;
+      }
       const bool gathered = prm.train.gather_idx != nullptr;
       const long ray_g = gathered ? (long)prm.train.gather_idx[in.first + ray] : ray + (rg - r);
       const float* rr = prm.rend.rays + ray_g * prm.rend.ray_stride;
@@ -55,11 +72,18 @@
       sky_ray(rr[8], rr[9], rr[10], prm.rend.sky_hidden, prm.rend.w1, prm.rend.b1, prm.rend.w2, prm.rend.b2, lane, k0, k1, k2);
       if (lane == 0 && prm.rend.sky) prm.rend.sky[ray * 3] = k0, prm.rend.sky[ray * 3 + 1] = k1, prm.rend.sky[ray * 3 + 2] = k2;
       if (train) {
+        HeadGrads hg;
         loss_part += render_loss_ray(r_z + lr * S, r_sigma + lr * S, prm.rend.noise ? prm.rend.noise + ray * S : nullptr, prm.rend.noise_std,
                                      r_albedo + lr * S * 3, r_sun + lr * S, r_beta + lr * S, k0, k1, k2, prm.train.target + (gathered ? ray_g : ray) * 3, ray,
                                      prm.rend.n_rays, S, lane, prm.train.beta_min, warm, prm.train.rgb ? prm.train.rgb + ray * 3 : nullptr,
                                      prm.train.d_sigma + ray * S, prm.train.d_albedo + ray * S * 3, prm.train.d_sun + ray * S,
-                                     prm.train.g_beta + ray * S, prm.train.d_sky + ray * 3);
+                                     prm.train.g_beta + ray * S, prm.train.d_sky + ray * 3, handoff ? &hg : nullptr, !prm.train.skip_point_grads);
+        if (handoff && lane < S) {
+          const int j = lr * S + lane;
+          float v[6];
+          head_pre_grads(hg, r_albedo[j * 3], r_albedo[j * 3 + 1], r_albedo[j * 3 + 2], r_sun[j], r_sigma[j], r_beta[j], v);
+          store_head_rows(prm.train.dpre, prm.train.dpre_fmt, ray * S + lane, v);
+        }
         continue;
       }
       composite_ray(r_z + lr * S, r_sigma + lr * S, prm.rend.noise ? prm.rend.noise + ray * S : nullptr, prm.rend.noise_std,
diff --git a/satnerf_amd/csrc/mlp_params.h b/satnerf_amd/csrc/mlp_params.h
--- a/satnerf_amd/csrc/mlp_params.h
+++ b/satnerf_amd/csrc/mlp_params.h
@@ -42,6 +42,9 @@
   float* out_rays;
   float* out_rgbs;
   long long* out_ts;
+  uint4* dpre;
+  int dpre_fmt;
+  int skip_point_grads;
 };
 
 struct FwdParams {
@@ -76,6 +79,7 @@
   long n_points;
   int tau;
   int auxs;
+  int heads_ready;
 };
 
 }
diff --git a/satnerf_amd/csrc/ray_device.h b/satnerf_amd/csrc/ray_device.h
--- a/satnerf_amd/csrc/ray_device.h
+++ b/satnerf_amd/csrc/ray_device.h
@@ -1,5 +1,6 @@
 #pragma once
 #include "common.h"
+#include "head_grads.h"
 
 namespace sr {
 
@@ -168,11 +169,15 @@
   }
 }
 
+struct HeadGrads {
+  float d_sigma, d_alb0, d_alb1, d_alb2, d_sun, g_beta;
+};
 __device__ __forceinline__ float render_loss_ray(const float* z, const float* sigma, const float* noise, float noise_std, const float* albedo,
                                                  const float* sun_v, const float* beta, float k0, float k1, float k2, const float* target, long r,
                                                  long n_rays, int S, int lane, float beta_min, bool warm, float* __restrict__ rgb_out,
                                                  float* __restrict__ d_sigma, float* __restrict__ d_albedo, float* __restrict__ d_sun,
-                                                 float* __restrict__ g_beta, float* __restrict__ d_sky) {
+                                                 float* __restrict__ g_beta, float* __restrict__ d_sky, HeadGrads* hg = nullptr,
+                                                 bool store = true) {
   const bool on = lane < S;
   const int i = lane < S ? lane : S - 1;
   float delta = 0.f, dens = 0.f, alpha = 0.f, a0 = 0.f, a1 = 0.f, a2 = 0.f, sv = 0.f, bj = 0.f;
@@ -220,14 +225,30 @@
   const float di0 = q0 * a0, di1 = q1 * a1, di2 = q2 * a2;
   const float s0 = wave_sum(di0 * (1.f - sv)), s1 = wave_sum(di1 * (1.f - sv)), s2 = wave_sum(di2 * (1.f - sv));
   if (lane == 0) d_sky[0] = s0, d_sky[1] = s1, d_sky[2] = s2;
+  HeadGrads g = {0.f, 0.f, 0.f, 0.f, 0.f, 0.f};
   if (on) {
     const float dalpha = G * T - after / f;
-    d_sigma[i] = dens > 0.f ? dalpha * delta * expf(-delta * dens) : 0.f;
-    d_albedo[i * 3] = q0 * i0, d_albedo[i * 3 + 1] = q1 * i1, d_albedo[i * 3 + 2] = q2 * i2;
-    d_sun[i] = di0 * (1.f - k0) + di1 * (1.f - k1) + di2 * (1.f - k2);
-    g_beta[i] = db * w;
-  }
+    g.d_sigma = dens > 0.f ? dalpha * delta * expf(-delta * dens) : 0.f;
+    g.d_alb0 = q0 * i0, g.d_alb1 = q1 * i1, g.d_alb2 = q2 * i2;
+    g.d_sun = di0 * (1.f - k0) + di1 * (1.f - k1) + di2 * (1.f - k2);
+    g.g_beta = db * w;
+    if (store) {
+      d_sigma[i] = g.d_sigma;
+      d_albedo[i * 3] = g.d_alb0, d_albedo[i * 3 + 1] = g.d_alb1, d_albedo[i * 3 + 2] = g.d_alb2;
+      d_sun[i] = g.d_sun;
+      g_beta[i] = g.g_beta;
+    }
+  }
+  if (hg) *hg = g;
   return contrib;
 }
 
-}
+__device__ __forceinline__ void head_pre_grads(const HeadGrads& g, float alb0, float alb1, float alb2, float sun_v, float sigma, float beta,
+                                               float (&v)[6]) {
+  v[0] = head_d_albedo(g.d_alb0, alb0, 0), v[1] = head_d_albedo(g.d_alb1, alb1, 1), v[2] = head_d_albedo(g.d_alb2, alb2, 2);
+  v[3] = head_d_sigmoid(g.d_sun, sun_v);
+  v[4] = head_d_softplus(g.g_beta, beta);
+  v[5] = head_d_softplus(g.d_sigma, sigma);
+}
+
+}
diff --git a/satnerf_amd/ops.py b/satnerf_amd/ops.py
--- a/satnerf_amd/ops.py
+++ b/satnerf_amd/ops.py
@@ -174,7 +174,8 @@
 
 
 def render_train(rays, ts, temb, n_samples, feat, tau, mode, stream_hi, stream_lo, l0, sky_w1, sky_b1, sky_w2, sky_b2, target, acts, u=None,
-                 noise=None, noise_std=0.0, seed=0, step_counter=None, sched=None, beta_min=0.05, want_z=False, tick=0, gather=None):
+                 noise=None, noise_std=0.0, seed=0, step_counter=None, sched=None, beta_min=0.05, want_z=False, tick=0, gather=None, dpre=None,
+                 dpre_fmt=8, skip_point_grads=False):
     rays, stride = _rows(rays, "rays", 11)
     n, s, dev = rays.shape[0], int(n_samples), rays.device
     if gather is not None:
@@ -193,8 +194,11 @@
         raise ValueError(f"no fused training forward for feat={feat}, mode={mode}, n_samples={s}")
     e = lambda *shape: torch.empty(*shape, dtype=torch.float32, device=dev)
     out = {"z": e(n, s) if want_z else None, "albedo": e(n, s, 3), "sigma": e(n, s), "sun_v": e(n, s), "beta": e(n, s), "sky": e(n, 3),
-           "loss": e((n * s + per_block - 1) // per_block), "rgb": e(n, 3), "d_sigma": e(n, s), "d_albedo": e(n, s, 3), "d_sun": e(n, s),
-           "g_beta": e(n, s), "d_sky": e(n, 3)}
+           "loss": e((n * s + per_block - 1) // per_block), "rgb": e(n, 3), "d_sky": e(n, 3)}
+    if skip_point_grads and dpre is None:
+        raise ValueError("skip_point_grads needs the dpre workspace of the head hand-off")
+    for k, shape in (("d_sigma", (n, s)), ("d_albedo", (n, s, 3)), ("d_sun", (n, s)), ("g_beta", (n, s))):
+        out[k] = None if skip_point_grads else e(*shape)
     args = _lib.RenderArgs(_p(rays), stride, _p(ts), _p(temb), n, s, None, _p(u), int(seed) & 0xFFFFFFFFFFFFFFFF,
                            _p(_chk(step_counter, "step_counter", allow_none=True)), int(tick), _p(noise), float(noise_std), sky_w1.shape[0],
                            _p(_chk(sky_w1, "w1")), _p(_chk(sky_b1, "b1")), _p(_chk(sky_w2, "w2")), _p(_chk(sky_b2, "b2")), 0)
@@ -207,8 +211,13 @@
     ev = kernel_timer.span("mlp_fwd") if kernel_timer is not None else None
     if ev:
         ev[0].record()
-    _lib.call("sr_satnerf_render_train", C.byref(args), feat, tau, MODES[mode], _p(stream_hi), _p(stream_lo), _p(_chk(l0, "l0")), C.byref(outs),
-              C.byref(tr), _p(acts), 8, _stream())
+    if dpre is None:
+        _lib.call("sr_satnerf_render_train", C.byref(args), feat, tau, MODES[mode], _p(stream_hi), _p(stream_lo), _p(_chk(l0, "l0")), C.byref(outs),
+                  C.byref(tr), _p(acts), 8, _stream())
+    else:
+        _lib.call("sr_satnerf_render_train_handoff", C.byref(args), feat, tau, MODES[mode], _p(stream_hi), _p(stream_lo), _p(_chk(l0, "l0")),
+                  C.byref(outs), C.byref(tr), _p(acts), 8, _p(_chk(dpre, "dpre", torch.int16)), dpre.numel(), int(dpre_fmt), int(bool(skip_point_grads)),
+                  _stream())
     if ev:
         ev[1].record()
     return out
@@ -500,20 +509,37 @@
     return _ws_empty(_lib.lib().sr_workspace_tiles(n_points) * per_tile, torch.int16, device, 1)
 
 
-def satnerf_mlp_bwd(feat, tau, n_points, bwd_stream, acts, albedo, sigma, sun_v, beta, g_albedo, g_sigma, g_sun_v, g_beta, want_dt=True, fmt=16):
-    dev = albedo.device
+def dpre_workspace(n_points, feat, device, fmt=16):
     n_elems = _lib.lib().sr_dpre_workspace_elems(n_points, feat, int(fmt))
     if n_elems <= 0:
         raise ValueError(f"unsupported workspace (feat={feat}, fmt={fmt})")
-    dpre = _ws_empty(n_elems, torch.int16, dev, 2)
+    return _ws_empty(n_elems, torch.int16, device, 2)
+
+
+def head_handoff_enabled():
+    return os.environ.get("SATNERF_HEAD_HANDOFF", "1") != "0"
+
+
+def satnerf_mlp_bwd(feat, tau, n_points, bwd_stream, acts, albedo, sigma, sun_v, beta, g_albedo, g_sigma, g_sun_v, g_beta, want_dt=True, fmt=16,
+                    dpre=None, heads_ready=False):
+    dev = acts.device
+    if dpre is None:
+        if heads_ready:
+            raise ValueError("heads_ready needs the dpre workspace the training forward wrote")
+        dpre = dpre_workspace(n_points, feat, dev, fmt)
+    elif _chk(dpre, "dpre", torch.int16).numel() < _lib.lib().sr_dpre_workspace_elems(n_points, feat, int(fmt)):
+        raise ValueError("dpre workspace too small (ops.dpre_workspace)")
     d_t = torch.empty(n_points, tau, dtype=torch.float32, device=dev) if want_dt else None
     opt = lambda t, nm: _p(_chk(t, nm, allow_none=True))
     ev = kernel_timer.span("mlp_bwd") if kernel_timer is not None else None
     if ev:
         ev[0].record()
-    _lib.call("sr_satnerf_mlp_bwd", feat, tau, n_points, _p(bwd_stream), _p(acts), _p(_chk(albedo, "albedo")), _p(_chk(sigma, "sigma")),
-              _p(_chk(sun_v, "sun_v")), _p(_chk(beta, "beta")), opt(g_albedo, "g_albedo"), opt(g_sigma, "g_sigma"), opt(g_sun_v, "g_sun_v"),
-              opt(g_beta, "g_beta"), _p(dpre), _p(d_t), int(fmt), _stream())
+    if heads_ready:
+        _lib.call("sr_satnerf_mlp_bwd_handoff", feat, tau, n_points, _p(bwd_stream), _p(acts), _p(dpre), _p(d_t), int(fmt), _stream())
+    else:
+        _lib.call("sr_satnerf_mlp_bwd", feat, tau, n_points, _p(bwd_stream), _p(acts), _p(_chk(albedo, "albedo")), _p(_chk(sigma, "sigma")),
+                  _p(_chk(sun_v, "sun_v")), _p(_chk(beta, "beta")), opt(g_albedo, "g_albedo"), opt(g_sigma, "g_sigma"), opt(g_sun_v, "g_sun_v"),
+                  opt(g_beta, "g_beta"), _p(dpre), _p(d_t), int(fmt), _stream())
     if ev:
         ev[1].record()
     return dpre, d_t
diff --git a/satnerf_amd/packing.py b/satnerf_amd/packing.py
--- a/satnerf_amd/packing.py
+++ b/satnerf_amd/packing.py
@@ -420,6 +420,21 @@
     return fmt8_geometry(feat)["D8_UNITS"]
 
 
+def head_row_slots(points, feat=256, fmt=8):
+    p = np.asarray(points, dtype=np.int64)
+    g8 = fmt8_geometry(feat)
+    if fmt == 8:
+        dk, head_unit, sigma_unit = g8["D8_UNITS"], g8["D8_HEAD"], g8["D8_SIGMA"]
+    elif fmt == 16:
+        dk, head_unit, sigma_unit = g8["DP_HEAD"] + 1, g8["DP_HEAD"], g8["DP_SIGMA"]
+    else:
+        raise ValueError(f"workspace format must be 16 or 8 (got {fmt})")
+    tile, slot = p >> 5, p & 31
+    base = tile * dk * 64 + slot
+    return dict(tile=tile, slot=slot, units_per_tile=dk, head_unit=head_unit, sigma_unit=sigma_unit, head=base + head_unit * 64,
+                beta=base + head_unit * 64 + 32, sigma=base + sigma_unit * 64, sigma_pad=base + sigma_unit * 64 + 32)
+
+
 def dpre8_source(f, feat=256):
     g8 = fmt8_geometry(feat)
     if f == g8["DP_SIGMA"]:
diff --git a/satnerf_amd/train.py b/satnerf_amd/train.py
--- a/satnerf_amd/train.py
+++ b/satnerf_amd/train.py
@@ -217,13 +217,16 @@
         gather, self._gather_in_fwd = self._gather_in_fwd, None
         if pit and not fused:
             raise RuntimeError("pack-in-tail steps need the one-launch training forward (it ticks the step counter)")
+        handoff = fused and self.direct and ops.head_handoff_enabled()
+        dpre_ws = ops.dpre_workspace(n * s, feat, rays.device, fmt) if handoff else None
         if fused:
             src = (gather["bank"].rays, gather["bank"].ts, gather["bank"].rgbs) if gather is not None else (rays, ts, rgbs)
             r = ops.render_train(src[0], src[1], emb.weight.data, s, feat, tau, mode, hi, lo, l0, sk[0].weight.data, sk[0].bias.data, sk[2].weight.data,
                                  sk[2].bias.data, src[2], acts, u=u, noise=nz, noise_std=noise_std, seed=self._seed, step_counter=self.adam_state,
                                  sched=self.sched, want_z=sc_on, tick=2 if pit else 0,
                                  gather=None if gather is None else dict(idx=gather["idx"], cursor=gather["cursor"], batches=gather["batches"],
-                                                                         out=(rays, rgbs, ts)))
+                                                                         out=(rays, rgbs, ts)),
+                                 dpre=dpre_ws, dpre_fmt=fmt, skip_point_grads=handoff)
             z, sky, loss, self.last_rgb = r["z"], r["sky"], r["loss"], r["rgb"]
             albedo, sigma, sun_v, beta = r["albedo"].view(-1, 3), r["sigma"].view(-1), r["sun_v"].view(-1), r["beta"].view(-1)
             d_sigma, d_albedo, d_sun, g_beta, d_sky = r["d_sigma"], r["d_albedo"], r["d_sun"], r["g_beta"], r["d_sky"]
@@ -245,7 +248,11 @@
                 d_sigma, d_albedo, d_sun, d_sky = ops.composite_bwd(z, sigma.view(n, s), nz, noise_std, albedo.view(n, s, 3), sun_v.view(n, s), sky,
                                                                    weights, transp, g_rgb, None, g_w, None)
                 self.last_rgb = rgb
-        dpre, d_t = ops.satnerf_mlp_bwd(feat, tau, n * s, bstream, acts, albedo, sigma, sun_v, beta, d_albedo, d_sigma, d_sun, g_beta.view(-1), fmt=fmt)
+        if handoff:
+            dpre, d_t = ops.satnerf_mlp_bwd(feat, tau, n * s, bstream, acts, None, None, None, None, None, None, None, None, fmt=fmt, dpre=dpre_ws,
+                                            heads_ready=True)
+        else:
+            dpre, d_t = ops.satnerf_mlp_bwd(feat, tau, n * s, bstream, acts, albedo, sigma, sun_v, beta, d_albedo, d_sigma, d_sun, g_beta.view(-1), fmt=fmt)
         partial, plan = ops.wgrad_partials(feat, tau, n * s, dpre, acts, maps["blocks"], fmt, maps["loads8"])
         if sc_on:
             loss = torch.cat([loss.view(-1), self._sc_pass(rays, ts, z, noise_std).view(-1)])
```

After: 2.737 million rays/s. -1.7%, worse.
